# AriAaltoGit/deeplearning4j

Hardware: AMD Instinct MI355X
Metric: images/sec (whole node) ResNet-50 training at 1/2/4/8 MI355X (higher is better)
Workload: dtype bf16; 1 GPU; model=ResNet-50 (DL4J zoo ResNet50 graph), variant=dl4j, global_batch=1024, per_gpu_batch=1024, image_size=224, parallelism=dp1, comm=torch, updater=RmsProp(0.1,0.96,1e-3) + l1 1e-7 + l2 5e-5 (fused HIP updater), hip_graph=False, kernel_db=deeplearning4j_amd/ops/tunedb/gfx950.json

## Files before the change

### csrc/batchnorm.hip

```cpp
#include "common.h"
#include <cstdlib>

template <typename T>
__global__ __launch_bounds__(256) void bn_stats_partial(const T* __restrict__ x, long long M, int C,
                                                        long long rows_per_blk, float* __restrict__ part_s1,
                                                        float* __restrict__ part_s2) {
  const int T8 = C >> 3;
  const int R = 256 / T8;
  const int cg = threadIdx.x % T8, r0 = threadIdx.x / T8;
  float s1[8], s2[8], sh[8];
  Vec8<T>::load(x + cg * 8, sh);
#pragma unroll
  for (int i = 0; i < 8; ++i) { s1[i] = 0.f; s2[i] = 0.f; }
  const long long rbeg = (long long)blockIdx.x * rows_per_blk;
  long long rend = rbeg + rows_per_blk;
  if (rend > M) rend = M;
  if (r0 < R) {
    long long r = rbeg + r0;
    for (; r + 3 * R < rend; r += 4 * R) {
      float v[4][8];
#pragma unroll
      for (int u = 0; u < 4; ++u) Vec8<T>::load(x + (r + u * R) * C + cg * 8, v[u]);
#pragma unroll
      for (int u = 0; u < 4; ++u)
#pragma unroll
        for (int i = 0; i < 8; ++i) { const float d = v[u][i] - sh[i]; s1[i] += d; s2[i] += d * d; }
    }
    for (; r < rend; r += R) {
      float v[8];
      Vec8<T>::load(x + r * C + cg * 8, v);
#pragma unroll
      for (int i = 0; i < 8; ++i) { const float d = v[i] - sh[i]; s1[i] += d; s2[i] += d * d; }
    }
  }
  __shared__ float red1[256 * 9];
  __shared__ float red2[256 * 9];
#pragma unroll
  for (int i = 0; i < 8; ++i) {
    red1[threadIdx.x * 9 + i] = (r0 < R) ? s1[i] : 0.f;
    red2[threadIdx.x * 9 + i] = (r0 < R) ? s2[i] : 0.f;
  }
  __syncthreads();
  for (int c = threadIdx.x; c < C; c += 256) {
    const int g = c >> 3, k = c & 7;
    float a = 0.f, b = 0.f;
    for (int rr = 0; rr < R; ++rr) { a += red1[(rr * T8 + g) * 9 + k]; b += red2[(rr * T8 + g) * 9 + k]; }
    part_s1[(long long)blockIdx.x * C + c] = a;
    part_s2[(long long)blockIdx.x * C + c] = b;
  }
}

__global__ __launch_bounds__(256) void bn_reduce_rows(const float* __restrict__ p1, const float* __restrict__ p2,
                                                      int nblk, int C, float* __restrict__ q1, float* __restrict__ q2) {
  const int c = blockIdx.x * 64 + (threadIdx.x & 63);
  const int grp = threadIdx.x >> 6;
  const int r0 = blockIdx.y * 32 + grp * 8;
  float a[8], b[8];
#pragma unroll
  for (int u = 0; u < 8; ++u) {
    const int r = r0 + u;
    const bool ok = c < C && r < nblk;
    a[u] = ok ? p1[(long long)r * C + c] : 0.f;
    b[u] = ok ? p2[(long long)r * C + c] : 0.f;
  }
  float sa = 0.f, sb = 0.f;
#pragma unroll
  for (int u = 0; u < 8; ++u) { sa += a[u]; sb += b[u]; }
  __shared__ float ra[256], rb[256];
  ra[threadIdx.x] = sa; rb[threadIdx.x] = sb;
  __syncthreads();
  if (grp == 0 && c < C) {
    q1[(long long)blockIdx.y * C + c] = ra[threadIdx.x] + ra[threadIdx.x + 64] + ra[threadIdx.x + 128] + ra[threadIdx.x + 192];
    q2[(long long)blockIdx.y * C + c] = rb[threadIdx.x] + rb[threadIdx.x + 64] + rb[threadIdx.x + 128] + rb[threadIdx.x + 192];
  }
}

template <typename T>
__global__ __launch_bounds__(256) void bn_tiles_reduce(const float* __restrict__ ts, long long P, int C, long long M,
                                                       const T* __restrict__ x, float* __restrict__ q1,
                                                       float* __restrict__ q2, int rpp) {
  const int c = blockIdx.x * 64 + (threadIdx.x & 63);
  const int grp = threadIdx.x >> 6;
  const long long p0 = (long long)blockIdx.y * 32 + grp * 8;
  float sa = 0.f, sb = 0.f;
  if (c < C) {
    const float x0 = ld1<T>(x + c);
#pragma unroll
    for (int u = 0; u < 8; ++u) {
      const long long p = p0 + u;
      if (p >= P) break;
      const long long nrow = M - (long long)rpp * p;
      const float n = (float)(nrow < rpp ? (nrow < 0 ? 0 : nrow) : rpp);
      const float s1 = ts[p * C + c], s2 = ts[(P + p) * C + c], d = ts[(2 * P + p) * C + c] - x0;
      sa += s1 + n * d;
      sb += s2 + 2.f * d * s1 + n * d * d;
    }
  }
  __shared__ float ra[256], rb[256];
  ra[threadIdx.x] = sa;
  rb[threadIdx.x] = sb;
  __syncthreads();
  if (grp == 0 && c < C) {
    q1[(long long)blockIdx.y * C + c] = ra[threadIdx.x] + ra[threadIdx.x + 64] + ra[threadIdx.x + 128] + ra[threadIdx.x + 192];
    q2[(long long)blockIdx.y * C + c] = rb[threadIdx.x] + rb[threadIdx.x + 64] + rb[threadIdx.x + 128] + rb[threadIdx.x + 192];
  }
}

__device__ __forceinline__ void reduce_partials(const float* __restrict__ p1, const float* __restrict__ p2, int nblk,
                                                int C, int c, double& a, double& b) {
  const int grp = threadIdx.x >> 6;
  a = 0.0; b = 0.0;
  if (c < C)
    for (int i = grp; i < nblk; i += 4) { a += p1[(long long)i * C + c]; b += p2[(long long)i * C + c]; }
  __shared__ double ra[256], rb[256];
  ra[threadIdx.x] = a; rb[threadIdx.x] = b;
  __syncthreads();
  if (grp == 0) {
    a = ra[threadIdx.x] + ra[threadIdx.x + 64] + ra[threadIdx.x + 128] + ra[threadIdx.x + 192];
    b = rb[threadIdx.x] + rb[threadIdx.x + 64] + rb[threadIdx.x + 128] + rb[threadIdx.x + 192];
  }
}

template <typename T>
__global__ __launch_bounds__(256) void bn_finalize(const float* __restrict__ part_s1, const float* __restrict__ part_s2,
                                                   int nblk, int C, long long M, const T* __restrict__ x,
                                                   const float* __restrict__ gamma, const float* __restrict__ beta,
                                                   float gconst, float bconst, float* __restrict__ run_mean,
                                                   float* __restrict__ run_var, float decay, float eps, int training,
                                                   float* __restrict__ ctx) {
  const int c = blockIdx.x * 64 + (threadIdx.x & 63);
  double a = 0.0, b = 0.0;
  if (training) reduce_partials(part_s1, part_s2, nblk, C, c, a, b);
  if ((threadIdx.x >> 6) != 0 || c >= C) return;
  float mean, var;
  if (training) {
    const double m1 = a / (double)M;
    mean = (float)((double)ld1<T>(x + c) + m1);
    double v = b / (double)M - m1 * m1;
    if (v < 0) v = 0;
    var = (float)v + eps;
    run_mean[c] = decay * run_mean[c] + (1.f - decay) * mean;
    run_var[c] = decay * run_var[c] + (1.f - decay) * var;
  } else {
    mean = run_mean[c];
    var = run_var[c];
  }
  const float inv = rsqrtf(var);
  const float g = gamma ? gamma[c] : gconst;
  const float bb = beta ? beta[c] : bconst;
  ctx[c] = mean;
  ctx[C + c] = inv;
  ctx[2 * C + c] = g * inv;
  ctx[3 * C + c] = bb - mean * g * inv;
}

template <typename T, bool RELU, bool RES, bool RBN = false>
__global__ __launch_bounds__(256) void bn_apply(const T* __restrict__ x, const T* __restrict__ res, T* __restrict__ y,
                                                long long M, int C, const float* __restrict__ ctx,
                                                unsigned char* __restrict__ mask, const float* __restrict__ rctx) {
  const long long nvec = M * (C >> 3);
  const int T8 = C >> 3;
  const float* scale = ctx + 2 * C;
  const float* shift = ctx + 3 * C;
  const long long stride = (long long)gridDim.x * blockDim.x;
  const long long v0 = (long long)blockIdx.x * blockDim.x + threadIdx.x;
  if (stride % T8 == 0) {
    const int c0 = idx_mod(v0, T8) * 8;
    float sc[8], sf[8], rsc[8], rsf[8];
#pragma unroll
    for (int i = 0; i < 8; ++i) {
      sc[i] = scale[c0 + i]; sf[i] = shift[c0 + i];
      rsc[i] = RBN ? rctx[2 * C + c0 + i] : 1.f;
      rsf[i] = RBN ? rctx[3 * C + c0 + i] : 0.f;
    }
    long long v = v0;
    for (; v + stride < nvec; v += 2 * stride) {
      float a[2][8], r[2][8];
#pragma unroll
      for (int u = 0; u < 2; ++u) {
        Vec8<T>::load(x + (v + u * stride) * 8, a[u]);
        if (RES) Vec8<T>::load(res + (v + u * stride) * 8, r[u]);
      }
#pragma unroll
      for (int u = 0; u < 2; ++u) {
        unsigned bits = 0;
#pragma unroll
        for (int i = 0; i < 8; ++i) {
          float t = a[u][i] * sc[i] + sf[i];
          if (RES) t += RBN ? fmaf(r[u][i], rsc[i], rsf[i]) : r[u][i];
          bits |= (t > 0.f ? 1u : 0u) << i;
          a[u][i] = RELU ? fmaxf(t, 0.f) : t;
        }
        Vec8<T>::store(y + (v + u * stride) * 8, a[u]);
        if (RES && mask) mask[v + u * stride] = (unsigned char)bits;
      }
    }
    if (v < nvec) {
      float a[8], r[8];
      Vec8<T>::load(x + v * 8, a);
      if (RES) Vec8<T>::load(res + v * 8, r);
      unsigned bits = 0;
#pragma unroll
      for (int i = 0; i < 8; ++i) {
        float t = a[i] * sc[i] + sf[i];
        if (RES) t += RBN ? fmaf(r[i], rsc[i], rsf[i]) : r[i];
        bits |= (t > 0.f ? 1u : 0u) << i;
        a[i] = RELU ? fmaxf(t, 0.f) : t;
      }
      Vec8<T>::store(y + v * 8, a);
      if (RES && mask) mask[v] = (unsigned char)bits;
    }
    return;
  }
  for (long long v = v0; v < nvec; v += stride) {
    const int c0 = idx_mod(v, T8) * 8;
    float a[8], r[8];
    Vec8<T>::load(x + v * 8, a);
    if (RES) Vec8<T>::load(res + v * 8, r);
    unsigned bits = 0;
#pragma unroll
    for (int i = 0; i < 8; ++i) {
      float t = a[i] * scale[c0 + i] + shift[c0 + i];
      if (RES) t += RBN ? fmaf(r[i], rctx[2 * C + c0 + i], rctx[3 * C + c0 + i]) : r[i];
      bits |= (t > 0.f ? 1u : 0u) << i;
      a[i] = RELU ? fmaxf(t, 0.f) : t;
    }
    Vec8<T>::store(y + v * 8, a);
    if (RES && mask) mask[v] = (unsigned char)bits;
  }
}

template <typename T, bool RELU, bool RES, bool RBN = false>
__global__ __launch_bounds__(256) void bn_bwd_partial(const T* __restrict__ x, const T* __restrict__ res,
                                                      const T* __restrict__ dy, long long M, int C,
                                                      long long rows_per_blk, const float* __restrict__ ctx,
                                                      float* __restrict__ part_db, float* __restrict__ part_dg,
                                                      const unsigned char* __restrict__ mask,
                                                      const float* __restrict__ rctx, float* __restrict__ part_dg2) {
  const int T8 = C >> 3;
  const int R = 256 / T8;
  const int cg = threadIdx.x % T8, r0 = threadIdx.x / T8;
  float db[8], dg[8], mu[8], is[8], sc[8], sf[8], dg2[8], mu2[8], is2[8];
#pragma unroll
  for (int i = 0; i < 8; ++i) {
    db[i] = 0.f; dg[i] = 0.f; dg2[i] = 0.f;
    mu[i] = ctx[cg * 8 + i]; is[i] = ctx[C + cg * 8 + i];
    sc[i] = ctx[2 * C + cg * 8 + i]; sf[i] = ctx[3 * C + cg * 8 + i];
    mu2[i] = RBN ? rctx[cg * 8 + i] : 0.f;
    is2[i] = RBN ? rctx[C + cg * 8 + i] : 0.f;
  }
  const long long rbeg = (long long)blockIdx.x * rows_per_blk;
  long long rend = rbeg + rows_per_blk;
  if (rend > M) rend = M;
  if (r0 < R) {
    constexpr int U = 4;
    struct Batch { RawVec8<T> xv[U], gv[U], rv[RES ? U : 1]; unsigned mb[U]; };
    auto load = [&](long long r, Batch& b) {
#pragma unroll
      for (int u = 0; u < U; ++u) {
        const long long ru = r + u * R;
        const long long rr = ru < rend ? ru : rbeg + r0;
        const long long o = rr * C + cg * 8;
        b.xv[u].load(x + o);
        b.gv[u].load(dy + o);
        if (RES) {
          if (mask) b.mb[u] = mask[rr * T8 + cg];
          if (!mask || RBN) b.rv[RES ? u : 0].load(res + o);
        }
      }
    };
    auto consume = [&](long long r, const Batch& b) {
#pragma unroll
      for (int u = 0; u < U; ++u) {
        if (r + u * R >= rend) continue;
#pragma unroll
        for (int i = 0; i < 8; ++i) {
          const float xf = b.xv[u].get(i);
          float d = b.gv[u].get(i);
          if (RES && mask) {
            d = (b.mb[u] >> i) & 1u ? d : 0.f;
          } else if (RELU) {
            float t = xf * sc[i] + sf[i];
            if (RES) t += RBN ? fmaf(b.rv[RES ? u : 0].get(i), rctx[2 * C + cg * 8 + i], rctx[3 * C + cg * 8 + i])
                              : b.rv[RES ? u : 0].get(i);
            d = t > 0.f ? d : 0.f;
          }
          db[i] += d;
          dg[i] += d * (xf - mu[i]) * is[i];
          if (RBN) dg2[i] += d * (b.rv[RES ? u : 0].get(i) - mu2[i]) * is2[i];
        }
      }
    };
    long long r = rbeg + r0;
    Batch b0, b1;
    if (r < rend) load(r, b0);
    while (r < rend) {
      const long long r1 = r + U * R;
      if (r1 < rend) load(r1, b1);
      consume(r, b0);
      if (r1 >= rend) break;
      const long long r2 = r1 + U * R;
      if (r2 < rend) load(r2, b0);
      consume(r1, b1);
// ... 566 lines not shown
  float* cdb2 = cdg + C;
  float* cdg2 = cdb2 + C;
  hipLaunchKernelGGL((bn_bwd_partial<T, true, true, true>), dim3(nblk), dim3(256), 0, s, x, res, dy, M, C, rpb, ctx, p1,
                     p2, mask, rctx, p3);
  BnFin f{M, nullptr, nullptr, nullptr, 0.f, 0.f, nullptr, nullptr, 0.f, 0.f, nullptr, dbeta, dgamma, cdb, cdg,
          nullptr, 0};
  int rc = bn_fold_launch<T, 0, 1>(p1, p2, nblk, C, q, f, s);
  if (rc) return rc;
  BnFin f2{M, nullptr, nullptr, nullptr, 0.f, 0.f, nullptr, nullptr, 0.f, 0.f, nullptr, dbeta2, dgamma2, cdb2, cdg2,
           nullptr, 0};
  rc = bn_fold_launch<T, 0, 1>(p1, p3, nblk, C, q2, f2, s);
  if (rc) return rc;
  hipLaunchKernelGGL((bn_bwd_apply<T, true, true, true>), dim3(apply_grid(M, C)), dim3(256), 0, s, x, res, dy, dx, dres,
                     M, C, ctx, cdb, cdg, mask, rctx, cdg2);
  return (int)hipGetLastError();
}

DL4J_API int dl4j_bn_bwd_rbn(int dtype, const void* x, const void* res, const void* dy, void* dx, void* dres,
                             long long M, int C, const float* ctx, float* dgamma, float* dbeta, const float* rctx,
                             float* dgamma2, float* dbeta2, float* ws, const unsigned char* mask, hipStream_t s) {
  if (C % 8 != 0 || C / 8 > 256 || !res || !dres || !rctx || (dtype != 1 && dtype != 2)) return -1;
  if (dtype == 2)
    return bn_bwd_rbn_impl<f16>((const f16*)x, (const f16*)res, (const f16*)dy, (f16*)dx, (f16*)dres, M, C, ctx, dgamma,
                                dbeta, rctx, dgamma2, dbeta2, ws, mask, s);
  return bn_bwd_rbn_impl<bf16>((const bf16*)x, (const bf16*)res, (const bf16*)dy, (bf16*)dx, (bf16*)dres, M, C, ctx,
                               dgamma, dbeta, rctx, dgamma2, dbeta2, ws, mask, s);
}

DL4J_API int dl4j_bn_fwd_rbn(int dtype, const void* x, const void* res, const float* rctx, void* y, long long M, int C,
                             const float* gamma, const float* beta, float gconst, float bconst, float* run_mean,
                             float* run_var, float decay, float eps, float* ws, float* ctx_out, unsigned char* mask,
                             const float* tstats, long long P, int rpp, hipStream_t s) {
  if (C % 8 != 0 || C / 8 > 256 || !res || !rctx || !y || (dtype != 1 && dtype != 2)) return -1;
  if (tstats) {
    if (rpp < 1) return -1;
    if (dtype == 2)
      return bn_fwd_tiles_impl<f16>((const f16*)x, (const f16*)res, (f16*)y, M, C, tstats, P, rpp, gamma, beta,
                                    gconst, bconst, run_mean, run_var, decay, eps, 1, ws, ctx_out, mask, s, rctx);
    return bn_fwd_tiles_impl<bf16>((const bf16*)x, (const bf16*)res, (bf16*)y, M, C, tstats, P, rpp, gamma, beta,
                                   gconst, bconst, run_mean, run_var, decay, eps, 1, ws, ctx_out, mask, s, rctx);
  }
  if (dtype == 2)
    return bn_fwd_impl<f16>((const f16*)x, (const f16*)res, (f16*)y, M, C, gamma, beta, gconst, bconst, run_mean,
                            run_var, decay, eps, 1, 1, ws, ctx_out, mask, s, rctx);
  return bn_fwd_impl<bf16>((const bf16*)x, (const bf16*)res, (bf16*)y, M, C, gamma, beta, gconst, bconst, run_mean,
                           run_var, decay, eps, 1, 1, ws, ctx_out, mask, s, rctx);
}

DL4J_API int dl4j_bn_bwd(int dtype, const void* x, const void* res, const void* dy, void* dx, void* dres, long long M,
                         int C, const float* ctx, float* dgamma, float* dbeta, int relu, float* ws,
                         const unsigned char* mask, hipStream_t s) {
  if (C % 8 != 0 || C / 8 > 256) return -1;
  if (res) relu = 1;
  else mask = nullptr;
#define BNB(T) return bn_bwd_impl<T>((const T*)x, (const T*)res, (const T*)dy, (T*)dx, (T*)dres, M, C, ctx, dgamma, \
                                     dbeta, relu, ws, mask, s)
  if (dtype == 1) BNB(bf16);
  if (dtype == 2) BNB(f16);
  BNB(float);
#undef BNB
}

DL4J_API long long dl4j_bn_bwd_planes_workspace_floats(long long P, int C) {
  return 2 * ((P + 31) / 32) * (long long)C + 4LL * C;
}

template <typename T>
static int bn_bwd_planes_impl(const T* x, const T* dy, T* dx, T* dres, const unsigned char* mask, long long M, int C,
                              const float* ctx, float* dgamma, float* dbeta, int relu, const float* planes,
                              long long P, float* ws, hipStream_t s) {
  float* q = ws;
  float* cdb = q + 2 * ((P + 31) / 32) * (long long)C;
  float* cdg = cdb + C;
  BnFin f{M, nullptr, nullptr, nullptr, 0.f, 0.f, nullptr, nullptr, 0.f, 0.f, nullptr, dbeta, dgamma, cdb, cdg,
          nullptr, 0};
  const int rc = bn_fold_launch<T, 0, 1>(planes, planes + P * C, P, C, q, f, s);
  if (rc) return rc;
  if (dres)
    hipLaunchKernelGGL((bn_bwd_apply<T, true, true>), dim3(apply_grid(M, C)), dim3(256), 0, s, x, nullptr, dy, dx,
                       dres, M, C, ctx, cdb, cdg, mask, nullptr, nullptr);
  else if (relu)
    hipLaunchKernelGGL((bn_bwd_apply<T, true, false>), dim3(apply_grid(M, C)), dim3(256), 0, s, x, nullptr, dy, dx,
                       nullptr, M, C, ctx, cdb, cdg, nullptr, nullptr, nullptr);
  else
    hipLaunchKernelGGL((bn_bwd_apply<T, false, false>), dim3(apply_grid(M, C)), dim3(256), 0, s, x, nullptr, dy, dx,
                       nullptr, M, C, ctx, cdb, cdg, nullptr, nullptr, nullptr);
  return (int)hipGetLastError();
}

DL4J_API int dl4j_bn_bwd_planes(int dtype, const void* x, const void* dy, void* dx, void* dres,
                                const unsigned char* mask, long long M, int C, const float* ctx, float* dgamma,
                                float* dbeta, int relu, const float* planes, long long P, float* ws, hipStream_t s) {
  if (C % 8 != 0 || C / 8 > 256 || P < 1 || P != (M + 63) / 64 || ((dres == nullptr) != (mask == nullptr))) return -1;
  if (dtype == 1)
    return bn_bwd_planes_impl<bf16>((const bf16*)x, (const bf16*)dy, (bf16*)dx, (bf16*)dres, mask, M, C, ctx, dgamma,
                                    dbeta, relu, planes, P, ws, s);
  if (dtype == 2)
    return bn_bwd_planes_impl<f16>((const f16*)x, (const f16*)dy, (f16*)dx, (f16*)dres, mask, M, C, ctx, dgamma,
                                   dbeta, relu, planes, P, ws, s);
  return -1;
}

template <typename T>
__global__ __launch_bounds__(256) void bnpool_fwd(const T* __restrict__ x, T* __restrict__ y,
                                                  unsigned char* __restrict__ am, T* __restrict__ xh,
                                                  const float* __restrict__ ctx, int N, int H, int W, int C, int OH,
                                                  int OW, int kh, int kw, int sh, int sw, int pt, int pl) {
  const int CG = C >> 3;
  const long long total = (long long)N * OH * OW * CG;
  for (long long t = (long long)blockIdx.x * blockDim.x + threadIdx.x; t < total;
       t += (long long)gridDim.x * blockDim.x) {
    int cg, ow, oh, n;
    idx_decomp4(t, CG, OW, OH, cg, ow, oh, n);
    float sc[8], sf[8], best[8], bx[8];
    unsigned char idx[8];
#pragma unroll
    for (int i = 0; i < 8; ++i) {
      sc[i] = ctx[2 * C + cg * 8 + i];
      sf[i] = ctx[3 * C + cg * 8 + i];
      best[i] = -INFINITY;
      bx[i] = 0.f;
      idx[i] = 0;
    }
    for (int i = 0; i < kh; ++i) {
      const int ih = oh * sh - pt + i;
      if (ih < 0 || ih >= H) continue;
      for (int j = 0; j < kw; ++j) {
        const int iw = ow * sw - pl + j;
        if (iw < 0 || iw >= W) continue;
        float v[8];
        Vec8<T>::load(x + (((long long)n * H + ih) * W + iw) * C + cg * 8, v);
#pragma unroll
        for (int c = 0; c < 8; ++c) {
          const float a = fmaxf(v[c] * sc[c] + sf[c], 0.f);
          if (a > best[c]) {
            best[c] = a;
            bx[c] = v[c];
            idx[c] = (unsigned char)(i * kw + j);
          }
        }
      }
    }
    Vec8<T>::store(y + t * 8, best);
    if (am) {
      unsigned long long pk = 0;
#pragma unroll
      for (int c = 0; c < 8; ++c)
        pk |= ((unsigned long long)(idx[c] | (best[c] > 0.f ? 0x80 : 0))) << (8 * c);
      *reinterpret_cast<unsigned long long*>(am + t * 8) = pk;
    }
    if (xh) {
#pragma unroll
      for (int c = 0; c < 8; ++c) bx[c] = (bx[c] - ctx[cg * 8 + c]) * ctx[C + cg * 8 + c];
      Vec8<T>::store(xh + t * 8, bx);
    }
  }
}

template <typename T, int KH, int KW>
__global__ __launch_bounds__(256) void bnpool_fwd_k(const T* __restrict__ x, T* __restrict__ y,
                                                    unsigned char* __restrict__ am, T* __restrict__ xh,
                                                    const float* __restrict__ ctx, int N, int H, int W, int C, int OH,
                                                    int OW, int sh, int sw, int pt, int pl) {
  const int CG = C >> 3;
  const long long total = (long long)N * OH * OW * CG;
  for (long long t = (long long)blockIdx.x * blockDim.x + threadIdx.x; t < total;
       t += (long long)gridDim.x * blockDim.x) {
    int cg, ow, oh, n;
    idx_decomp4(t, CG, OW, OH, cg, ow, oh, n);
    float v[KH * KW][8];
    bool ok[KH * KW];
#pragma unroll
    for (int i = 0; i < KH; ++i)
#pragma unroll
      for (int j = 0; j < KW; ++j) {
        const int ih = oh * sh - pt + i, iw = ow * sw - pl + j;
        ok[i * KW + j] = ih >= 0 && ih < H && iw >= 0 && iw < W;
        const int ihc = min(max(ih, 0), H - 1), iwc = min(max(iw, 0), W - 1);
        Vec8<T>::load(x + (((long long)n * H + ihc) * W + iwc) * C + cg * 8, v[i * KW + j]);
      }
    float sc[8], sf[8], best[8], bx[8];
    unsigned char idx[8];
#pragma unroll
    for (int c = 0; c < 8; ++c) {
      sc[c] = ctx[2 * C + cg * 8 + c];
      sf[c] = ctx[3 * C + cg * 8 + c];
      best[c] = -INFINITY;
      bx[c] = 0.f;
      idx[c] = 0;
    }
#pragma unroll
    for (int q = 0; q < KH * KW; ++q) {
      if (!ok[q]) continue;
#pragma unroll
      for (int c = 0; c < 8; ++c) {
        const float a = fmaxf(v[q][c] * sc[c] + sf[c], 0.f);
        if (a > best[c]) {
          best[c] = a;
          bx[c] = v[q][c];
          idx[c] = (unsigned char)q;
        }
      }
    }
    Vec8<T>::store(y + t * 8, best);
    if (am) {
      unsigned long long pk = 0;
#pragma unroll
      for (int c = 0; c < 8; ++c)
        pk |= ((unsigned long long)(idx[c] | (best[c] > 0.f ? 0x80 : 0))) << (8 * c);
      *reinterpret_cast<unsigned long long*>(am + t * 8) = pk;
    }
    if (xh) {
#pragma unroll
      for (int c = 0; c < 8; ++c) bx[c] = (bx[c] - ctx[cg * 8 + c]) * ctx[C + cg * 8 + c];
      Vec8<T>::store(xh + t * 8, bx);
    }
  }
}

template <typename T>
__global__ __launch_bounds__(256) void bnpool_bwd_dx2(const T* __restrict__ x, const T* __restrict__ dy,
                                                      const unsigned char* __restrict__ am, T* __restrict__ dx,
                                                      const float* __restrict__ ctx, const float* __restrict__ cdb,
                                                      const float* __restrict__ cdg, int N, int H, int W, int C,
                                                      int OH, int OW, int kh, int kw, int sh, int sw, int pt, int pl) {
  const int CG = C >> 3;
  const long long total = (long long)N * H * W * CG;
  for (long long t = (long long)blockIdx.x * blockDim.x + threadIdx.x; t < total;
       t += (long long)gridDim.x * blockDim.x) {
    int cg, iw, ih, n;
    idx_decomp4(t, CG, W, H, cg, iw, ih, n);
    const int hp = ih + pt, wp = iw + pl;
    int oh0 = hp - kh + 1;
    oh0 = oh0 <= 0 ? 0 : (oh0 + sh - 1) / sh;
    int ow0 = wp - kw + 1;
    ow0 = ow0 <= 0 ? 0 : (ow0 + sw - 1) / sw;
    const int oh1 = min(hp / sh, OH - 1), ow1 = min(wp / sw, OW - 1);
    float g[4][8], xv[8];
    unsigned long long pk[4];
    unsigned me[4];
#pragma unroll
    for (int a = 0; a < 2; ++a)
#pragma unroll
      for (int b = 0; b < 2; ++b) {
        const int oh = oh0 + a, ow = ow0 + b, q = a * 2 + b;
        const bool ok = oh <= oh1 && ow <= ow1;
        const long long o = (((long long)n * OH + min(oh, OH - 1)) * OW + min(ow, OW - 1)) * C + cg * 8;
        Vec8<T>::load(dy + o, g[q]);
        pk[q] = *reinterpret_cast<const unsigned long long*>(am + o);
        me[q] = ok ? (0x80u | (unsigned)((hp - oh * sh) * kw + (wp - ow * sw))) : 0x100u;
      }
    Vec8<T>::load(x + t * 8, xv);
#pragma unroll
    for (int i = 0; i < 8; ++i) {
      float acc = 0.f;
#pragma unroll
      for (int q = 0; q < 4; ++q)
        if (((pk[q] >> (8 * i)) & 0xff) == me[q]) acc += g[q][i];
      const int c = cg * 8 + i;
      const float xhat = (xv[i] - ctx[c]) * ctx[C + c];
      xv[i] = ctx[2 * C + c] * (acc - cdb[c] - xhat * cdg[c]);
    }
    Vec8<T>::store(dx + t * 8, xv);
  }
}

template <typename T>
__global__ __launch_bounds__(256) void bnpool_bwd_dx_lds(const T* __restrict__ x, const T* __restrict__ dy,
                                                         const unsigned char* __restrict__ am, T* __restrict__ dx,
                                                         const float* __restrict__ ctx, const float* __restrict__ cdb,
                                                         const float* __restrict__ cdg, int N, int H, int W, int C,
                                                         int OH, int OW, int kh, int kw, int sh, int sw, int pt,
                                                         int pl, int maxrows) {
  extern __shared__ __attribute__((aligned(16))) unsigned char smem[];
  const int CG = C >> 3, RB = 2;
  const int rows_per_img = (H + RB - 1) / RB;
  const int n = blockIdx.x / rows_per_img, ih0 = (blockIdx.x - n * rows_per_img) * RB;
  int oh_lo = ih0 + pt - kh + 1;
  oh_lo = oh_lo <= 0 ? 0 : (oh_lo + sh - 1) / sh;
  const int oh_hi = min((min(ih0 + RB, H) - 1 + pt) / sh, OH - 1);
  const int nrows = oh_hi - oh_lo + 1;
  T* sdy = reinterpret_cast<T*>(smem);
  unsigned char* sam = smem + (size_t)maxrows * OW * C * sizeof(T);
  const int row_elems = OW * C;
  if (nrows > 0) {
    const long long g0 = ((long long)n * OH + oh_lo) * row_elems;
    const int nv = nrows * row_elems / 8;
    for (int i = threadIdx.x; i < nv; i += 256) {
      if (sizeof(T) == 2)
        reinterpret_cast<uint4*>(sdy)[i] = reinterpret_cast<const uint4*>(dy + g0)[i];
      else {
        reinterpret_cast<uint4*>(sdy)[2 * i] = reinterpret_cast<const uint4*>(dy + g0)[2 * i];
        reinterpret_cast<uint4*>(sdy)[2 * i + 1] = reinterpret_cast<const uint4*>(dy + g0)[2 * i + 1];
      }
      reinterpret_cast<uint2*>(sam)[i] = reinterpret_cast<const uint2*>(am + g0)[i];
    }
  }
  __syncthreads();
  const int items = min(RB, H - ih0) * W * CG;
  const bool fixed = (256 % CG) == 0;
  float A[8], B[8], Cq[8];
  if (fixed) {
#pragma unroll
    for (int i = 0; i < 8; ++i) {
      const int c = (threadIdx.x % CG) * 8 + i;
      A[i] = ctx[2 * C + c];
      B[i] = ctx[2 * C + c] * ctx[C + c] * cdg[c];
      Cq[i] = ctx[2 * C + c] * (cdb[c] - ctx[c] * ctx[C + c] * cdg[c]);
    }
  }
  for (int it = threadIdx.x; it < items; it += 256) {
    const int cg = it % CG, q1 = it / CG, iw = q1 % W, ih = ih0 + q1 / W;
    const int hp = ih + pt, wp = iw + pl;
    int oh0 = hp - kh + 1;
    oh0 = oh0 <= 0 ? 0 : (oh0 + sh - 1) / sh;
    int ow0 = wp - kw + 1;
    ow0 = ow0 <= 0 ? 0 : (ow0 + sw - 1) / sw;
    const int oh1 = min(hp / sh, OH - 1), ow1 = min(wp / sw, OW - 1);
    const long long t = (((long long)n * H + ih) * W + iw) * CG + cg;
    float xv[8], acc[8];
    Vec8<T>::load(x + t * 8, xv);
#pragma unroll
    for (int i = 0; i < 8; ++i) acc[i] = 0.f;
#pragma unroll
    for (int a = 0; a < 2; ++a)
#pragma unroll
      for (int b = 0; b < 2; ++b) {
        const int oh = oh0 + a, ow = ow0 + b;
        if (oh > oh1 || ow > ow1) continue;
        const int o = ((oh - oh_lo) * OW + ow) * C + cg * 8;
        float g[8];
        Vec8<T>::load(sdy + o, g);
        const unsigned long long pk = *reinterpret_cast<const unsigned long long*>(sam + o);
        const unsigned me = 0x80u | (unsigned)((hp - oh * sh) * kw + (wp - ow * sw));
#pragma unroll
        for (int i = 0; i < 8; ++i)
          if (((pk >> (8 * i)) & 0xff) == me) acc[i] += g[i];
      }
    if (fixed) {
#pragma unroll
      for (int i = 0; i < 8; ++i) xv[i] = A[i] * acc[i] - B[i] * xv[i] - Cq[i];
    } else {
#pragma unroll
      for (int i = 0; i < 8; ++i) {
        const int c = cg * 8 + i;
        const float xhat = (xv[i] - ctx[c]) * ctx[C + c];
        xv[i] = ctx[2 * C + c] * (acc[i] - cdb[c] - xhat * cdg[c]);
      }
    }
    Vec8<T>::store(dx + t * 8, xv);
  }
}

template <typename T>
__global__ __launch_bounds__(256) void bnpool_bwd_partial(const T* __restrict__ dy, const unsigned char* __restrict__ am,
                                                          const T* __restrict__ xh, long long M, int C,
                                                          long long rows_per_blk, float* __restrict__ part_db,
                                                          float* __restrict__ part_dg) {
  const int T8 = C >> 3;
  const int R = 256 / T8;
  const int cg = threadIdx.x % T8, r0 = threadIdx.x / T8;
  float db[8], dg[8];
#pragma unroll
  for (int i = 0; i < 8; ++i) {
    db[i] = 0.f;
    dg[i] = 0.f;
  }
  const long long rbeg = (long long)blockIdx.x * rows_per_blk;
  long long rend = rbeg + rows_per_blk;
  if (rend > M) rend = M;
  if (r0 < R) {
    for (long long r = rbeg + r0; r < rend; r += R) {
      const long long o = r * C + cg * 8;
      float gv[8], hv[8];
      Vec8<T>::load(dy + o, gv);
      Vec8<T>::load(xh + o, hv);
      const unsigned long long pk = *reinterpret_cast<const unsigned long long*>(am + o);
#pragma unroll
      for (int i = 0; i < 8; ++i) {
        const float d = ((pk >> (8 * i)) & 0x80) ? gv[i] : 0.f;
        db[i] += d;
        dg[i] += d * hv[i];
      }
    }
  }
  __shared__ float red1[256 * 9];
  __shared__ float red2[256 * 9];
#pragma unroll
  for (int i = 0; i < 8; ++i) {
    red1[threadIdx.x * 9 + i] = (r0 < R) ? db[i] : 0.f;
    red2[threadIdx.x * 9 + i] = (r0 < R) ? dg[i] : 0.f;
  }
  __syncthreads();
  for (int c = threadIdx.x; c < C; c += 256) {
    const int g = c >> 3, k = c & 7;
    float a = 0.f, b = 0.f;
    for (int rr = 0; rr < R; ++rr) {
      a += red1[(rr * T8 + g) * 9 + k];
      b += red2[(rr * T8 + g) * 9 + k];
    }
    part_db[(long long)blockIdx.x * C + c] = a;
    part_dg[(long long)blockIdx.x * C + c] = b;
  }
}

template <typename T>
__global__ __launch_bounds__(256) void bnpool_bwd_dx(const T* __restrict__ x, const T* __restrict__ dy,
                                                     const unsigned char* __restrict__ am, T* __restrict__ dx,
                                                     const float* __restrict__ ctx, const float* __restrict__ cdb,
                                                     const float* __restrict__ cdg, int N, int H, int W, int C, int OH,
                                                     int OW, int kh, int kw, int sh, int sw, int pt, int pl) {
  const int CG = C >> 3;
  const long long total = (long long)N * H * W * CG;
  for (long long t = (long long)blockIdx.x * blockDim.x + threadIdx.x; t < total;
       t += (long long)gridDim.x * blockDim.x) {
    int cg, iw, ih, n;
    idx_decomp4(t, CG, W, H, cg, iw, ih, n);
    float acc[8];
#pragma unroll
    for (int c = 0; c < 8; ++c) acc[c] = 0.f;
    const int hp = ih + pt, wp = iw + pl;
    int oh0 = hp - kh + 1;
    oh0 = oh0 <= 0 ? 0 : (oh0 + sh - 1) / sh;
    int ow0 = wp - kw + 1;
    ow0 = ow0 <= 0 ? 0 : (ow0 + sw - 1) / sw;
    const int oh1 = min(hp / sh, OH - 1), ow1 = min(wp / sw, OW - 1);
    for (int oh = oh0; oh <= oh1; ++oh) {
      for (int ow = ow0; ow <= ow1; ++ow) {
        const long long o = (((long long)n * OH + oh) * OW + ow) * C + cg * 8;
        float g[8];
        Vec8<T>::load(dy + o, g);
        const unsigned long long pk = *reinterpret_cast<const unsigned long long*>(am + o);
        const unsigned me = 0x80u | (unsigned)((hp - oh * sh) * kw + (wp - ow * sw));
#pragma unroll
        for (int c = 0; c < 8; ++c)
          if (((pk >> (8 * c)) & 0xff) == me) acc[c] += g[c];
      }
    }
    float xv[8];
    Vec8<T>::load(x + t * 8, xv);
#pragma unroll
    for (int i = 0; i < 8; ++i) {
      const int c = cg * 8 + i;
      const float xhat = (xv[i] - ctx[c]) * ctx[C + c];
      xv[i] = ctx[2 * C + c] * (acc[i] - cdb[c] - xhat * cdg[c]);
    }
    Vec8<T>::store(dx + t * 8, xv);
  }
}

static inline int ew_grid(long long total) {
  long long g = (total + 255) / 256;
  if (g > 256 * 32) g = 256 * 32;
  return (int)(g < 1 ? 1 : g);
}

template <typename T>
static void bnpool_fwd_launch(const T* x, T* y, unsigned char* am, T* xh, const float* ctx, int N, int H, int W, int C,
                              int OH, int OW, int kh, int kw, int sh, int sw, int pt, int pl, int pg, hipStream_t s) {
  if (kh == 3 && kw == 3)
    hipLaunchKernelGGL((bnpool_fwd_k<T, 3, 3>), dim3(pg), dim3(256), 0, s, x, y, am, xh, ctx, N, H, W, C, OH, OW, sh,
                       sw, pt, pl);
  else if (kh == 2 && kw == 2)
    hipLaunchKernelGGL((bnpool_fwd_k<T, 2, 2>), dim3(pg), dim3(256), 0, s, x, y, am, xh, ctx, N, H, W, C, OH, OW, sh,
                       sw, pt, pl);
  else
    hipLaunchKernelGGL(bnpool_fwd<T>, dim3(pg), dim3(256), 0, s, x, y, am, xh, ctx, N, H, W, C, OH, OW, kh, kw, sh, sw,
                       pt, pl);
}

template <typename T>
static int bn_pool_fwd_impl(const T* xb, T* y, unsigned char* am, T* xh, int N, int H, int W, int C, int OH, int OW,
                            int kh, int kw, int sh, int sw, int pt, int pl, const float* gamma, const float* beta,
                            float gconst, float bconst, float* run_mean, float* run_var, float decay, float eps,
                            int training, const float* tstats, long long P, int rpp, float* ws, float* ctx_out,
                            hipStream_t s) {
  const long long M = (long long)N * H * W;
  int nblk;
  long long rpb;
  bn_grid(M, C, &nblk, &rpb);
  float* p1 = ws;
  float* p2 = ws + (long long)nblk * C;
  float* q = p2 + (long long)nblk * C;
  const dim3 fg((C + 63) / 64);
  const int pg = ew_grid((long long)N * OH * OW * (C / 8));
  if (training && tstats && sizeof(T) == 2) {
    nblk = (int)((P + 31) / 32);
    p2 = ws + (long long)nblk * C;
    q = p2 + (long long)nblk * C;
    hipLaunchKernelGGL(bn_tiles_reduce<T>, dim3((C + 63) / 64, nblk), dim3(256), 0, s, tstats, P, C, M, xb, p1, p2,
                       rpp);
    bn_reduce_stage(p1, p2, nblk, C, q, s);
    hipLaunchKernelGGL(bn_finalize<T>, fg, dim3(256), 0, s, p1, p2, nblk, C, M, xb, gamma, beta, gconst, bconst,
                       run_mean, run_var, decay, eps, 1, ctx_out);
  } else {
    if (training) hipLaunchKernelGGL(bn_stats_partial<T>, dim3(nblk), dim3(256), 0, s, xb, M, C, rpb, p1, p2);
    if (training) bn_reduce_stage(p1, p2, nblk, C, q, s);
    hipLaunchKernelGGL(bn_finalize<T>, fg, dim3(256), 0, s, p1, p2, nblk, C, M, xb, gamma, beta, gconst, bconst,
                       run_mean, run_var, decay, eps, training, ctx_out);
  }
  bnpool_fwd_launch<T>(xb, y, am, xh, ctx_out, N, H, W, C, OH, OW, kh, kw, sh, sw, pt, pl, pg, s);
  return (int)hipGetLastError();
}

DL4J_API int dl4j_bn_pool_fwd(int dtype, const void* x, void* y, unsigned char* am, void* xh, int N, int H, int W,
                              int C, int OH, int OW, int kh, int kw, int sh, int sw, int pt, int pl,
                              const float* gamma, const float* beta, float gconst, float bconst, float* run_mean,
                              float* run_var, float decay, float eps, int training, const float* tstats,
                              long long P, int rpp, float* ws, float* ctx_out, hipStream_t s) {
  if (C % 8 != 0 || C / 8 > 256 || kh * kw > 127 || kh < 1 || kw < 1) return -1;
#define BPF(T) return bn_pool_fwd_impl<T>((const T*)x, (T*)y, am, (T*)xh, N, H, W, C, OH, OW, kh, kw, sh, sw, pt, pl, \
                                          gamma, beta, gconst, bconst, run_mean, run_var, decay, eps, training,    \
                                          tstats, P, rpp, ws, ctx_out, s)
  if (dtype == 1) BPF(bf16);
  if (dtype == 2) BPF(f16);
  BPF(float);
#undef BPF
}

template <typename T>
static int bn_pool_bwd_impl(const T* x, const T* dy, const unsigned char* am, const T* xh, T* dx, int N, int H, int W,
                            int C, int OH, int OW, int kh, int kw, int sh, int sw, int pt, int pl, const float* ctx,
                            float* dgamma, float* dbeta, float* ws, hipStream_t s) {
  const long long Mp = (long long)N * OH * OW, M = (long long)N * H * W;
  int nblk;
  long long rpb;
  bn_grid(Mp, C, &nblk, &rpb);
  float* p1 = ws;
  float* p2 = ws + (long long)nblk * C;
  float* q = p2 + (long long)nblk * C;
  float* cdb = q + 2LL * ((nblk + 31) / 32) * C;
  float* cdg = cdb + C;
  const int g = ew_grid(M * (C / 8));
  hipLaunchKernelGGL(bnpool_bwd_partial<T>, dim3(nblk), dim3(256), 0, s, dy, am, xh, Mp, C, rpb, p1, p2);
  bn_reduce_stage(p1, p2, nblk, C, q, s);
  hipLaunchKernelGGL(bn_bwd_finalize, dim3((C + 63) / 64), dim3(256), 0, s, p1, p2, nblk, C, M, dbeta, dgamma, cdb,
                     cdg);
  const bool two = kh <= 2 * sh && kw <= 2 * sw;
  const int maxrows = (2 - 1 + kh - 1) / sh + 1;
  const size_t lds = (size_t)maxrows * OW * C * (sizeof(T) + 1);
  if (two && lds <= 64 * 1024) {
    const int nb = N * ((H + 1) / 2);
    hipLaunchKernelGGL(bnpool_bwd_dx_lds<T>, dim3(nb), dim3(256), lds, s, x, dy, am, dx, ctx, cdb, cdg, N, H, W, C, OH,
                       OW, kh, kw, sh, sw, pt, pl, maxrows);
    return (int)hipGetLastError();
  }
  if (two)
    hipLaunchKernelGGL(bnpool_bwd_dx2<T>, dim3(g), dim3(256), 0, s, x, dy, am, dx, ctx, cdb, cdg, N, H, W, C, OH, OW,
                       kh, kw, sh, sw, pt, pl);
  else
    hipLaunchKernelGGL(bnpool_bwd_dx<T>, dim3(g), dim3(256), 0, s, x, dy, am, dx, ctx, cdb, cdg, N, H, W, C, OH, OW,
                       kh, kw, sh, sw, pt, pl);
  return (int)hipGetLastError();
}

DL4J_API int dl4j_bn_pool_bwd(int dtype, const void* x, const void* dy, const unsigned char* am, const void* xh,
                              void* dx, int N, int H, int W, int C, int OH, int OW, int kh, int kw, int sh, int sw,
                              int pt, int pl, const float* ctx, float* dgamma, float* dbeta, float* ws, hipStream_t s) {
  if (C % 8 != 0 || C / 8 > 256 || kh * kw > 127) return -1;
#define BPB(T) return bn_pool_bwd_impl<T>((const T*)x, (const T*)dy, am, (const T*)xh, (T*)dx, N, H, W, C, OH, OW, kh, \
                                          kw, sh, sw, pt, pl, ctx, dgamma, dbeta, ws, s)
  if (dtype == 1) BPB(bf16);
  if (dtype == 2) BPB(f16);
  BPB(float);
#undef BPB
}
```

### csrc/conv_stem.hip

```cpp
#include "common.h"

typedef __attribute__((ext_vector_type(4))) float f4s_t;
typedef __attribute__((ext_vector_type(8))) __bf16 bf16x8s_t;

namespace {
constexpr int KS = 6;
constexpr int ROWS_PER_WG = 4;
constexpr int IN_ROWS = 2 * ROWS_PER_WG + 6;
constexpr int OUT_LD = 64 + 8;
constexpr int STAGE_SLOTS = 12;
}

__global__ void __launch_bounds__(256, 2) stem_conv_fwd(const u16* __restrict__ x, const bf16x8s_t* __restrict__ wpk,
                                                     u16* __restrict__ y, float* __restrict__ tstats, int N, int H,
                                                     int W, int OH, int OW, int RS, long long P) {
  extern __shared__ __attribute__((aligned(16))) unsigned char smem[];
  u16* xin = reinterpret_cast<u16*>(smem);
  u16* ot = xin + 2 * IN_ROWS * RS;
  const int lane = threadIdx.x & 63, wave = threadIdx.x >> 6, col = lane & 15, hg = lane >> 4;
  const int blocks_per_img = OH / ROWS_PER_WG, nblocks = N * blocks_per_img;
  bf16x8s_t b[4][KS];
#pragma unroll
  for (int nt = 0; nt < 4; ++nt)
#pragma unroll
    for (int ks = 0; ks < KS; ++ks) b[nt][ks] = wpk[(nt * KS + ks) * 64 + lane];
  const int row_elems = 3 * W, row_u2 = row_elems / 4;
  const int nchunks = (IN_ROWS - 1) * row_u2;
  {
    const int tail = RS - 12 - row_elems, per_row = 6 + tail / 2;
    for (int i = threadIdx.x; i < 2 * IN_ROWS * per_row; i += 256) {
      const int rb = i / per_row, j = i - rb * per_row;
      const int e = j < 6 ? 2 * j : 12 + row_elems + 2 * (j - 6);
      *reinterpret_cast<unsigned*>(xin + rb * RS + e) = 0u;
    }
    for (int i = threadIdx.x; i < 2 * row_u2; i += 256) {
      const int b2 = i / row_u2, j = i - b2 * row_u2;
      *reinterpret_cast<uint2*>(xin + (b2 * IN_ROWS + IN_ROWS - 1) * RS + 12 + 4 * j) = make_uint2(0u, 0u);
    }
  }
  uint2 pre[STAGE_SLOTS];
  int buf = 0;
  for (int blk = blockIdx.x; blk < nblocks; blk += gridDim.x, buf ^= 1) {
    const int n = blk / blocks_per_img, oh0 = (blk - n * blocks_per_img) * ROWS_PER_WG;
    u16* xb = xin + buf * IN_ROWS * RS;
#pragma unroll
    for (int q = 0; q < STAGE_SLOTS; ++q) {
      const int i = threadIdx.x + q * 256;
      const int rr = i / row_u2, j = i - rr * row_u2;
      const int ih = 2 * oh0 - 3 + rr;
      pre[q] = make_uint2(0u, 0u);
      if (i < nchunks && ih >= 0 && ih < H)
        pre[q] = *reinterpret_cast<const uint2*>(x + ((long long)n * H + ih) * row_elems + 4 * j);
    }
#pragma unroll
    for (int q = 0; q < STAGE_SLOTS; ++q) {
      const int i = threadIdx.x + q * 256;
      const int rr = i / row_u2, j = i - rr * row_u2;
      if (i < nchunks) *reinterpret_cast<uint2*>(xb + rr * RS + 12 + 4 * j) = pre[q];
    }
    __syncthreads();
    const int oh = oh0 + wave;
    const long long mrow = ((long long)n * OH + oh) * OW;
    u16* otw = ot + wave * 16 * OUT_LD;
    float s1[4], s2[4], shv[4];
#pragma unroll
    for (int nt = 0; nt < 4; ++nt) s1[nt] = s2[nt] = 0.f;
    for (int mt = 0; mt < OW / 16; ++mt) {
      const int ow = mt * 16 + col;
      const unsigned* abase = reinterpret_cast<const unsigned*>(xb + (2 * wave) * RS + 6 * ow + 2);
      f4s_t acc[4];
#pragma unroll
      for (int nt = 0; nt < 4; ++nt) acc[nt] = f4s_t{0.f, 0.f, 0.f, 0.f};
#pragma unroll
      for (int ks = 0; ks < KS; ++ks) {
        const int k0 = ks * 32 + hg * 8, r = k0 / 24, q0 = k0 - r * 24;
        const unsigned* ap = abase + (r * RS + q0) / 2;
        unsigned d[5];
#pragma unroll
        for (int jj = 0; jj < 5; ++jj) d[jj] = ap[jj];
        union {
          unsigned u[4];
          bf16x8s_t v;
        } a;
#pragma unroll
        for (int jj = 0; jj < 4; ++jj) a.u[jj] = __builtin_amdgcn_alignbit(d[jj + 1], d[jj], 16);
#pragma unroll
        for (int nt = 0; nt < 4; ++nt)
          acc[nt] = __builtin_amdgcn_mfma_f32_16x16x32_bf16(a.v, b[nt][ks], acc[nt], 0, 0, 0);
      }
#pragma unroll
      for (int nt = 0; nt < 4; ++nt) {
        u16 hv[4];
#pragma unroll
        for (int j = 0; j < 4; ++j) hv[j] = f2bf(acc[nt][j]);
        if (mt == 0) shv[nt] = __shfl(bf2f(hv[0]), col, 64);
#pragma unroll
        for (int j = 0; j < 4; ++j) {
          const float dd = bf2f(hv[j]) - shv[nt];
          s1[nt] += dd;
          s2[nt] += dd * dd;
          otw[(hg * 4 + j) * OUT_LD + nt * 16 + col] = hv[j];
        }
      }
#pragma unroll
      for (int j = 0; j < 2; ++j) {
        const int id = lane + 64 * j, row = id >> 3, c8 = id & 7;
        *reinterpret_cast<bf16x8*>(y + (mrow + mt * 16 + row) * 64 + c8 * 8) =
            *reinterpret_cast<const bf16x8*>(otw + row * OUT_LD + c8 * 8);
      }
    }
    if (tstats) {
#pragma unroll
      for (int nt = 0; nt < 4; ++nt) {
        s1[nt] += __shfl_xor(s1[nt], 16, 64);
        s1[nt] += __shfl_xor(s1[nt], 32, 64);
        s2[nt] += __shfl_xor(s2[nt], 16, 64);
        s2[nt] += __shfl_xor(s2[nt], 32, 64);
      }
      if (hg == 0) {
        const long long p = (long long)n * OH + oh;
#pragma unroll
        for (int nt = 0; nt < 4; ++nt) {
          tstats[p * 64 + nt * 16 + col] = s1[nt];
          tstats[(P + p) * 64 + nt * 16 + col] = s2[nt];
          tstats[(2 * P + p) * 64 + nt * 16 + col] = shv[nt];
        }
      }
    }
  }
}

DL4J_API int dl4j_stem_conv_fwd(const void* x, const void* wpk, void* y, float* tstats, int N, int H, int W,
                                      int OH, int OW, hipStream_t s) {
  if (N < 1 || OH % ROWS_PER_WG != 0 || OW % 16 != 0 || OH != (H - 1) / 2 + 1 ||
      OW != (W - 1) / 2 + 1 || (3 * W) % 4 != 0)
    return -1;
  int RS = 12 + 3 * W;
  const int need = 6 * (OW - 1) + 3 + 24 + 2;
  if (RS < need) RS = need;
  RS = (RS + 15) & ~15;
  const size_t lds = (size_t)2 * IN_ROWS * RS * 2 + 64 * OUT_LD * 2;
  if (lds > 64 * 1024 || (IN_ROWS - 1) * (3 * W / 4) > STAGE_SLOTS * 256) return -1;
  const long long P = (long long)N * OH;
  int dev = 0, ncu = 256;
  (void)hipGetDevice(&dev);
  (void)hipDeviceGetAttribute(&ncu, hipDeviceAttributeMultiprocessorCount, dev);
  int per = 1;
  if (hipOccupancyMaxActiveBlocksPerMultiprocessor(&per, stem_conv_fwd, 256, lds) != hipSuccess || per < 1) per = 1;
  const int nblocks = N * (OH / ROWS_PER_WG);
  const int grid = nblocks < per * ncu ? nblocks : per * ncu;
  hipLaunchKernelGGL(stem_conv_fwd, dim3(grid), dim3(256), lds, s, (const u16*)x,
                     (const bf16x8s_t*)wpk, (u16*)y, tstats, N, H, W, OH, OW, RS, P);
  return (int)hipGetLastError();
}

constexpr int kWrwWgPerCu = 3;
__global__ void __launch_bounds__(256, kWrwWgPerCu) stem_conv_wrw(const u16* __restrict__ x, const u16* __restrict__ dy,
                                                        float* __restrict__ part, float* __restrict__ part_db, int N,
                                                        int H, int W, int OH, int OW, int RS) {
  extern __shared__ __attribute__((aligned(16))) unsigned char smem[];
  u16* xin = reinterpret_cast<u16*>(smem);
  u16* dyt = xin + IN_ROWS * RS;
  float* dbs = reinterpret_cast<float*>(dyt + 2 * 64 * OUT_LD);
  const int lane = threadIdx.x & 63, wave = threadIdx.x >> 6, col = lane & 15, hg = lane >> 4;
  const int blocks_per_img = OH / ROWS_PER_WG, nblocks = N * blocks_per_img;
  const int row_elems = 3 * W, row_u2 = row_elems / 4;
  const int nchunks = (IN_ROWS - 1) * row_u2;
  const int rounds = ROWS_PER_WG * OW / 64;
  {
    const int tail = RS - 12 - row_elems, per_row = 6 + tail / 2;
    for (int i = threadIdx.x; i < IN_ROWS * per_row; i += 256) {
      const int rb = i / per_row, j = i - rb * per_row;
      const int e = j < 6 ? 2 * j : 12 + row_elems + 2 * (j - 6);
      *reinterpret_cast<unsigned*>(xin + rb * RS + e) = 0u;
    }
    for (int i = threadIdx.x; i < row_u2; i += 256)
      *reinterpret_cast<uint2*>(xin + (IN_ROWS - 1) * RS + 12 + 4 * i) = make_uint2(0u, 0u);
  }
  int koff[3];
#pragma unroll
  for (int t3 = 0; t3 < 3; ++t3) {
    const int k = (wave * 3 + t3) * 16 + col, r = k / 24, q = k - r * 24;
    koff[t3] = r * RS + q;
  }
  f4s_t acc[4][3];
#pragma unroll
  for (int ct = 0; ct < 4; ++ct)
#pragma unroll
    for (int t3 = 0; t3 < 3; ++t3) acc[ct][t3] = f4s_t{0.f, 0.f, 0.f, 0.f};
  float dbacc[8];
#pragma unroll
  for (int i = 0; i < 8; ++i) dbacc[i] = 0.f;
  uint2 pre[STAGE_SLOTS];
  for (int blk = blockIdx.x; blk < nblocks; blk += gridDim.x) {
    const int n = blk / blocks_per_img, oh0 = (blk - n * blocks_per_img) * ROWS_PER_WG;
    __syncthreads();
#pragma unroll
    for (int q = 0; q < STAGE_SLOTS; ++q) {
      const int i = threadIdx.x + q * 256;
      const int rr = i / row_u2, j = i - rr * row_u2;
      const int ih = 2 * oh0 - 3 + rr;
      pre[q] = make_uint2(0u, 0u);
      if (i < nchunks && ih >= 0 && ih < H)
        pre[q] = *reinterpret_cast<const uint2*>(x + ((long long)n * H + ih) * row_elems + 4 * j);
    }
#pragma unroll
    for (int q = 0; q < STAGE_SLOTS; ++q) {
      const int i = threadIdx.x + q * 256;
      const int rr = i / row_u2, j = i - rr * row_u2;
      if (i < nchunks) *reinterpret_cast<uint2*>(xin + rr * RS + 12 + 4 * j) = pre[q];
    }
    const long long m_base = ((long long)n * OH + oh0) * OW;
    auto load_dy = [&](int rnd, uint4* dst) {
#pragma unroll
      for (int j = 0; j < 2; ++j)
        dst[j] = *reinterpret_cast<const uint4*>(dy + (m_base + rnd * 64 + (threadIdx.x >> 3) + 32 * j) * 64 +
                                                 (threadIdx.x & 7) * 8);
    };
    auto round = [&](int rnd, uint4* gr) {
      u16* dt = dyt + (rnd & 1) * 64 * OUT_LD;
#pragma unroll
      for (int j = 0; j < 2; ++j) {
        const int px = (threadIdx.x >> 3) + 32 * j, c8 = threadIdx.x & 7;
        const u16* hv = reinterpret_cast<const u16*>(&gr[j]);
#pragma unroll
        for (int i = 0; i < 8; ++i) {
          dt[(c8 * 8 + i) * OUT_LD + (((px >> 3) ^ c8) << 3) + (px & 7)] = hv[i];
          dbacc[i] += bf2f(hv[i]);
        }
      }
      if (rnd + 2 < rounds) load_dy(rnd + 2, gr);
      __syncthreads();
#pragma unroll
      for (int ch = 0; ch < 2; ++ch) {
        const int p0 = rnd * 64 + ch * 32 + 8 * hg;
        const int ohl = p0 / OW, ow0 = p0 - ohl * OW;
        const u16* wb = xin + 2 * ohl * RS + (2 * ow0 + 1) * 3;
        bf16x8s_t bfr[3];
#pragma unroll
        for (int t3 = 0; t3 < 3; ++t3) {
          union {
            u16 h[8];
            bf16x8s_t v;
          } bb;
#pragma unroll
          for (int j = 0; j < 8; ++j) bb.h[j] = wb[koff[t3] + 6 * j];
          bfr[t3] = bb.v;
        }
#pragma unroll
        for (int ct = 0; ct < 4; ++ct) {
          const int row = ct * 16 + col;
          const bf16x8s_t a =
              *reinterpret_cast<const bf16x8s_t*>(dt + row * OUT_LD + (((ch * 4 + hg) ^ (row >> 3)) << 3));
#pragma unroll
          for (int t3 = 0; t3 < 3; ++t3)
            acc[ct][t3] = __builtin_amdgcn_mfma_f32_16x16x32_bf16(a, bfr[t3], acc[ct][t3], 0, 0, 0);
        }
      }
    };
    uint4 gA[2], gB[2];
    load_dy(0, gA);
    if (rounds > 1) load_dy(1, gB);
    for (int rnd = 0; rnd < rounds; rnd += 2) {
      round(rnd, gA);
      if (rnd + 1 < rounds) round(rnd + 1, gB);
    }
  }
  float* pw = part + (long long)blockIdx.x * 64 * 192;
#pragma unroll
  for (int ct = 0; ct < 4; ++ct)
#pragma unroll
    for (int t3 = 0; t3 < 3; ++t3)
#pragma unroll
      for (int j = 0; j < 4; ++j) pw[(ct * 16 + 4 * hg + j) * 192 + (3 * wave + t3) * 16 + col] = acc[ct][t3][j];
  __syncthreads();
#pragma unroll
  for (int i = 0; i < 8; ++i) dbs[threadIdx.x * 8 + i] = dbacc[i];
  __syncthreads();
  if (threadIdx.x < 64) {
    const int c8 = threadIdx.x >> 3, i = threadIdx.x & 7;
    float sum = 0.f;
    for (int t = c8; t < 256; t += 8) sum += dbs[t * 8 + i];
    part_db[(long long)blockIdx.x * 64 + c8 * 8 + i] = sum;
  }
}

__global__ void __launch_bounds__(256) stem_wrw_reduce(const float* __restrict__ part, const float* __restrict__ part_db,
                                                       int G, float* __restrict__ dW, float* __restrict__ db) {
  __shared__ float red[16][17];
  const int ol = threadIdx.x & 15, sl = threadIdx.x >> 4;
  const int o = blockIdx.x * 16 + ol;
  float a0 = 0.f, a1 = 0.f, a2 = 0.f, a3 = 0.f;
  if (o < 64 * 147) {
    const int co = o / 147, rem = o - co * 147, c = rem / 49, rs = rem - c * 49, r = rs / 7, s = rs - r * 7;
    const float* src = part + co * 192 + r * 24 + s * 3 + c;
    int g = sl;
    for (; g + 48 < G; g += 64) {
      a0 += src[(long long)g * 12288];
      a1 += src[(long long)(g + 16) * 12288];
      a2 += src[(long long)(g + 32) * 12288];
      a3 += src[(long long)(g + 48) * 12288];
    }
    for (; g < G; g += 16) a0 += src[(long long)g * 12288];
  } else if (db && o < 64 * 147 + 64) {
    const int co = o - 64 * 147;
    for (int g = sl; g < G; g += 16) a0 += part_db[(long long)g * 64 + co];
  }
  red[ol][sl] = (a0 + a1) + (a2 + a3);
  __syncthreads();
  if (sl == 0) {
    float t = 0.f;
#pragma unroll
    for (int i = 0; i < 16; ++i) t += red[ol][i];
    if (o < 64 * 147) dW[o] = t;
    else if (db && o < 64 * 147 + 64) db[o - 64 * 147] = t;
  }
}

DL4J_API long long dl4j_stem_wrw_workspace_floats(int N, int OH) {
  int dev = 0, ncu = 256;
  (void)hipGetDevice(&dev);
  (void)hipDeviceGetAttribute(&ncu, hipDeviceAttributeMultiprocessorCount, dev);
  const long long G = (long long)kWrwWgPerCu * ncu;
  return G * (64 * 192 + 64);
}

DL4J_API int dl4j_stem_conv_wrw(const void* x, const void* dy, float* dW, float* db, float* ws, int N, int H, int W,
                                int OH, int OW, hipStream_t s) {
  if (N < 1 || OH % ROWS_PER_WG != 0 || OW % 16 != 0 || OH != (H - 1) / 2 + 1 || OW != (W - 1) / 2 + 1 ||
      (3 * W) % 4 != 0 || (ROWS_PER_WG * OW) % 64 != 0)
    return -1;
  int RS = 12 + 3 * W;
  const int need = 6 * (OW - 1) + 3 + 24 + 2;
  if (RS < need) RS = need;
  RS = (RS + 15) & ~15;
  const size_t lds = (size_t)IN_ROWS * RS * 2 + 2 * 64 * OUT_LD * 2 + 256 * 8 * 4;
  if (lds > 64 * 1024 || (IN_ROWS - 1) * (3 * W / 4) > STAGE_SLOTS * 256) return -1;
  int dev = 0, ncu = 256;
  (void)hipGetDevice(&dev);
  (void)hipDeviceGetAttribute(&ncu, hipDeviceAttributeMultiprocessorCount, dev);
  const int nblocks = N * (OH / ROWS_PER_WG);
  const int G = nblocks < kWrwWgPerCu * ncu ? nblocks : kWrwWgPerCu * ncu;
  float* part = ws;
  float* part_db = ws + (long long)G * 64 * 192;
  hipLaunchKernelGGL(stem_conv_wrw, dim3(G), dim3(256), lds, s, (const u16*)x, (const u16*)dy, part, part_db, N, H, W,
                     OH, OW, RS);
  hipLaunchKernelGGL(stem_wrw_reduce, dim3((64 * 147 + 64 + 15) / 16), dim3(256), 0, s, part, part_db, G, dW, db);
  return (int)hipGetLastError();
}

__global__ __launch_bounds__(256) void stem_pack_weights(const u16* __restrict__ w, u16* __restrict__ pk,
                                                         long long sk, long long sc, long long sr, long long ss) {
  const int e = blockIdx.x * blockDim.x + threadIdx.x;
  if (e >= 4 * 6 * 64 * 8) return;
  const int n = e & 7, m = (e >> 3) & 63, j = (e >> 9) % 6, i = e / (6 * 512);
  const int row = j * 32 + (m >> 4) * 8 + n, k = i * 16 + (m & 15);
  const int r = row / 24, rem = row - r * 24;
  u16 v = 0;
  if (r < 7 && rem < 21) {
    const int s_ = rem / 3, c = rem - s_ * 3;
    v = w[k * sk + c * sc + r * sr + s_ * ss];
  }
  pk[e] = v;
}

DL4J_API int dl4j_stem_pack_weights(const void* w, void* pk, long long sk, long long sc, long long sr, long long ss,
                                    hipStream_t s) {
  hipLaunchKernelGGL(stem_pack_weights, dim3((4 * 6 * 64 * 8 + 255) / 256), dim3(256), 0, s, (const u16*)w, (u16*)pk,
                     sk, sc, sr, ss);
  return (int)hipGetLastError();
}
```

### csrc/include/dl4j_amd.h

```cpp
#ifndef DL4J_AMD_H
#define DL4J_AMD_H

#include <stddef.h>
#include <stdint.h>

#ifdef __cplusplus
extern "C" {
#endif

#define DL4J_AMD_ABI_VERSION 1

typedef struct ihipStream_t* hipStream_t;

enum dl4j_dtype { DL4J_F32 = 0, DL4J_BF16 = 1, DL4J_F16 = 2, DL4J_I32 = 3 };

enum dl4j_status {
  DL4J_OK = 0,
  DL4J_ERR_ARG = 1001,
  DL4J_ERR_SHAPE = 1002,
  DL4J_ERR_DTYPE = 1003,
  DL4J_ERR_LAYOUT = 1004,
  DL4J_ERR_LAUNCH = 1005,
  DL4J_ERR_COMM = 1006,
  DL4J_ERR_ABI = 1007
};

enum dl4j_updater {
  DL4J_UPD_NOOP = 0, DL4J_UPD_SGD = 1, DL4J_UPD_NESTEROVS = 2, DL4J_UPD_ADAM = 3, DL4J_UPD_ADAMAX = 4,
  DL4J_UPD_NADAM = 5, DL4J_UPD_ADAGRAD = 6, DL4J_UPD_ADADELTA = 7, DL4J_UPD_RMSPROP = 8
};

enum dl4j_reduce_op { DL4J_SUM = 0, DL4J_AVG = 1, DL4J_MAX = 2 };

typedef struct dl4j_tensor {
  void* data;
  int dtype;
  int ndim;
  long long shape[8];
  long long strides[8];
  int device;
} dl4j_tensor_t;

typedef struct dl4j_comm_s* dl4j_comm_t;

typedef struct Dl4jDevProps {
  char name[128];
  char arch[64];
  int cus, xcds, warp, max_threads, lds_per_block, clock_khz, mem_clock_khz, bus_width, pci_bus;
  long long total_mem, l2_bytes, lds_per_cu;
} Dl4jDevProps;

int dl4j_abi_version(void);
int dl4j_matmul(const dl4j_tensor_t* A, const dl4j_tensor_t* B, dl4j_tensor_t* C, float alpha, float beta, hipStream_t s);
int dl4j_update_flat(int op, float* params, float* grad, float* state, long long n, const float* hp, float l1, float l2, float inv_batch, int write_update, hipStream_t s);
int dl4j_comm_unique_id(void* id_out);
int dl4j_comm_id_bytes(void);
int dl4j_comm_init_rank(dl4j_comm_t* comm, int nranks, const void* id, int rank);
int dl4j_comm_init_all(dl4j_comm_t* comms, int ndev, const int* devices);
int dl4j_comm_all_reduce(dl4j_comm_t comm, const void* send, void* recv, long long count, int dtype, int op, hipStream_t s);
int dl4j_comm_broadcast(dl4j_comm_t comm, const void* send, void* recv, long long count, int dtype, int root, hipStream_t s);
int dl4j_comm_all_gather(dl4j_comm_t comm, const void* send, void* recv, long long count_per_rank, int dtype, hipStream_t s);
int dl4j_comm_reduce_scatter(dl4j_comm_t comm, const void* send, void* recv, long long count_per_rank, int dtype, int op, hipStream_t s);
int dl4j_comm_group_start(void);
int dl4j_comm_group_end(void);
int dl4j_comm_abort(dl4j_comm_t comm);
int dl4j_comm_destroy(dl4j_comm_t comm);

int dl4j_gelu(int dtype, const void* z, const void* dy, void* out, long long n, hipStream_t s);

int dl4j_attn_fwd_dt(int dt, const void* qkv, const float* mask, void* out, float* lse, int B, int T, int H, int D, float scale, int causal, hipStream_t s);
int dl4j_attn_bwd_dt(int dt, const void* qkv, const void* out, const void* dout, const float* mask, const float* lse, float* dq_dot, void* dqkv, int B, int T, int H, int D, float scale, int causal, hipStream_t s);
int dl4j_attn_fwd_drop_dt(int dt, const void* qkv, const float* mask, void* out, float* lse, int B, int T, int H, int D, float scale, int causal, float drop, unsigned long long seed, const long long* offset, hipStream_t s);
int dl4j_attn_bwd_drop_dt(int dt, const void* qkv, const void* out, const void* dout, const float* mask, const float* lse, float* dq_dot, void* dqkv, int B, int T, int H, int D, float scale, int causal, float drop, unsigned long long seed, const long long* offset, hipStream_t s);
int dl4j_attn_drop_mask(unsigned char* keep, int BH, int T, float drop, unsigned long long seed, const long long* offset, hipStream_t s);
int dl4j_attn_fwd(const void* qkv, const float* mask, void* out, float* lse, int B, int T, int H, int D, float scale, int causal, hipStream_t s);
int dl4j_attn_bwd(const void* qkv, const void* out, const void* dout, const float* mask, const float* lse, float* dq_dot, void* dqkv, int B, int T, int H, int D, float scale, int causal, hipStream_t s);

int dl4j_bn_workspace_floats(long long M, int C);
int dl4j_bn_fwd(int dtype, const void* x, const void* res, void* y, long long M, int C, const float* gamma, const float* beta, float gconst, float bconst, float* run_mean, float* run_var, float decay, float eps, int training, int relu, float* ws, float* ctx_out, unsigned char* mask, hipStream_t s);
long long dl4j_bn_tiles_workspace_floats(long long P, int C);
int dl4j_bn_fwd_tiles(int dtype, const void* x, const void* res, void* y, long long M, int C, const float* tstats, long long P, int rpp, const float* gamma, const float* beta, float gconst, float bconst, float* run_mean, float* run_var, float decay, float eps, int relu, float* ws, float* ctx_out, unsigned char* mask, hipStream_t s);
long long dl4j_bn_bwd_rbn_workspace_floats(long long M, int C);
int dl4j_bn_bwd_rbn(int dtype, const void* x, const void* res, const void* dy, void* dx, void* dres, long long M, int C, const float* ctx, float* dgamma, float* dbeta, const float* rctx, float* dgamma2, float* dbeta2, float* ws, const unsigned char* mask, hipStream_t s);
int dl4j_bn_fwd_rbn(int dtype, const void* x, const void* res, const float* rctx, void* y, long long M, int C, const float* gamma, const float* beta, float gconst, float bconst, float* run_mean, float* run_var, float decay, float eps, float* ws, float* ctx_out, unsigned char* mask, const float* tstats, long long P, int rpp, hipStream_t s);
int dl4j_bn_bwd(int dtype, const void* x, const void* res, const void* dy, void* dx, void* dres, long long M, int C, const float* ctx, float* dgamma, float* dbeta, int relu, float* ws, const unsigned char* mask, hipStream_t s);
long long dl4j_bn_bwd_planes_workspace_floats(long long P, int C);
int dl4j_bn_bwd_planes(int dtype, const void* x, const void* dy, void* dx, void* dres, const unsigned char* mask, long long M, int C, const float* ctx, float* dgamma, float* dbeta, int relu, const float* planes, long long P, float* ws, hipStream_t s);
int dl4j_bn_pool_fwd(int dtype, const void* x, void* y, unsigned char* am, void* xh, int N, int H, int W, int C, int OH, int OW, int kh, int kw, int sh, int sw, int pt, int pl, const float* gamma, const float* beta, float gconst, float bconst, float* run_mean, float* run_var, float decay, float eps, int training, const float* tstats, long long P, int rpp, float* ws, float* ctx_out, hipStream_t s);
int dl4j_bn_pool_bwd(int dtype, const void* x, const void* dy, const unsigned char* am, const void* xh, void* dx, int N, int H, int W, int C, int OH, int OW, int kh, int kw, int sh, int sw, int pt, int pl, const float* ctx, float* dgamma, float* dbeta, float* ws, hipStream_t s);

int dl4j_nonfinite_count(const void* segs, int nseg, void* seg_dev, unsigned long long* counts, long long max_n, hipStream_t s);

int dl4j_conv_v3_num_variants(void);
int dl4j_conv_v3_default_variant(long long M, int Nout);
int dl4j_conv_fwd_v3(int dt, const void* X, const void* Wkrsc, const float* bias, void* Y, int N, int H, int W, int C, int K, int R, int S, int sh, int sw, int ph, int pw, int dh, int dw, int OH, int OW, float beta, float* tstats, int variant, hipStream_t s);
int dl4j_conv_wrw_v3_num_variants(void);
long long dl4j_conv_wrw_v3_ws_floats(int N, int C, int K, int R, int S, int OH, int OW, int variant, int splits, int* splits_out);
int dl4j_conv_wrw_v3(int dt, const void* X, const void* dY, float* dW, float* db, float* ws, int N, int H, int W, int C, int K, int R, int S, int sh, int sw, int ph, int pw, int dh, int dw, int OH, int OW, int variant, int splits, hipStream_t s);

long long dl4j_conv_halo_plan(int N, int H, int W, int C, int K, int R, int S, int sh, int sw, int ph, int pw, int dh, int dw, int OH, int OW, int* pixels_per_chunk);
int dl4j_conv_halo(int dt, const void* X, const void* Wkrsc, const float* bias, void* Y, int N, int H, int W, int C, int K, int R, int S, int sh, int sw, int ph, int pw, int dh, int dw, int OH, int OW, float beta, float* tstats, hipStream_t s);

void dl4j_conv_set_variant(int v);
void dl4j_conv_set_wrw_variant(int v);
void dl4j_conv_set_wrw_remap(int v);
int dl4j_conv_w_relayout_batched(const void* jobs, int njobs, long long total_blocks, hipStream_t s);
int dl4j_conv_relayout_job_bytes(void);
int dl4j_conv_relayout_per_block(void);
int dl4j_conv_w_relayout_tiled(const void* jobs, int njobs, long long total_blocks, hipStream_t s);
int dl4j_conv_relayout_tile_job_bytes(void);
int dl4j_conv_relayout_tile_max_rs(void);
int dl4j_conv_w_relayout(const void* W, void* krsc, void* flip, int K, int C, int R, int S, hipStream_t s);
int dl4j_conv_fwd(const void* X, const void* Wkrsc, const float* bias, void* Y, int N, int H, int W, int C, int K, int R, int S, int sh, int sw, int ph, int pw, int dh, int dw, int OH, int OW, float* tstats, hipStream_t s);
int dl4j_conv_bwd_data_s1(const void* dY, const void* Wflip, void* dX, int N, int H, int W, int C, int K, int R, int S, int ph, int pw, int OH, int OW, int accum, hipStream_t s);
int dl4j_conv_bwd_data_1x1(const void* dY, const void* Wflip, void* dX, int N, int H, int W, int C, int K, int stride, int OH, int OW, int accum, hipStream_t s);
int dl4j_conv_wrw_permute(float* ws, float* dW, int K, int C, int R, int S, int rezero, hipStream_t s);
int dl4j_conv_wrw(const void* X, const void* dY, float* dW, float* db, int N, int H, int W, int C, int K, int R, int S, int sh, int sw, int ph, int pw, int dh, int dw, int OH, int OW, int splits, hipStream_t s);
long long dl4j_conv_wrw_det_floats(int N, int C, int K, int R, int S, int OH, int OW, int splits);
int dl4j_conv_wrw_det(const void* X, const void* dY, float* dW, float* db, float* part, int N, int H, int W, int C, int K, int R, int S, int sh, int sw, int ph, int pw, int dh, int dw, int OH, int OW, int splits, hipStream_t s);

int dl4j_stem_conv_fwd(const void* x, const void* wpk, void* y, float* tstats, int N, int H, int W, int OH, int OW, hipStream_t s);
long long dl4j_stem_wrw_workspace_floats(int N, int OH);
int dl4j_stem_conv_wrw(const void* x, const void* dy, float* dW, float* db, float* ws, int N, int H, int W, int OH, int OW, hipStream_t s);
int dl4j_stem_pack_weights(const void* w, void* pk, long long sk, long long sc, long long sr, long long ss, hipStream_t s);

int dl4j_conv_wrw_set_tree(int fan);
long long dl4j_conv_wrw_halo_ws_floats(int N, int H, int W, int C, int K, int R, int S, int sh, int sw, int ph, int pw, int dh, int dw, int OH, int OW, int variant, int splits, int* splits_out);
int dl4j_conv_wrw_halo(int dt, const void* X, const void* dY, float* dW, float* db, float* ws, int N, int H, int W, int C, int K, int R, int S, int sh, int sw, int ph, int pw, int dh, int dw, int OH, int OW, int variant, int splits, hipStream_t s);

int dl4j_w2v_sg(const int32_t* item_in, const int32_t* item_tgt, const float* alpha, long long n, float* syn0, float* syn1, float* syn1neg, int D, const uint8_t* codes, const int32_t* points, const int32_t* codelen, int maxc, const int32_t* table, long long tsize, int negative, int flags, unsigned long long seed, long long item_base, float* loss_out, int max_blocks, hipStream_t stream);
int dl4j_w2v_cbow(const int32_t* item_tgt, const float* alpha, const int32_t* ctx_off, const int32_t* ctx, long long n, float* syn0, float* syn1, float* syn1neg, int D, const uint8_t* codes, const int32_t* points, const int32_t* codelen, int maxc, const int32_t* table, long long tsize, int negative, int flags, unsigned long long seed, long long item_base, const float* extra_in, int n_extra, float* extra_grad, float* loss_out, int max_blocks, hipStream_t stream);
int dl4j_glove(const int32_t* ei, const int32_t* ej, const float* ex, long long n, float* W, float* b, float* hW, float* hb, int D, float lr, float xmax, float alpha, float* cost_out, int max_blocks, hipStream_t stream);

int dl4j_rt_device_count(void);
int dl4j_rt_device_props(int dev, Dl4jDevProps* p);
int dl4j_rt_set_device(int dev);
int dl4j_rt_get_device(void);
int dl4j_rt_device_sync(int dev);
int dl4j_rt_mem_info(int dev, long long* free_b, long long* total_b);
int dl4j_rt_stream_create(int dev, int high_priority, void** out);
int dl4j_rt_stream_create_cumask(int dev, int ncu, void** out);
int dl4j_rt_stream_cu_count(void* s);
int dl4j_rt_stream_destroy(void* s);
int dl4j_rt_stream_sync(void* s);
int dl4j_rt_stream_query(void* s);
int dl4j_rt_stream_wait_event(void* s, void* ev);
int dl4j_rt_event_create(int timing, void** out);
int dl4j_rt_event_destroy(void* e);
int dl4j_rt_event_record(void* e, void* s);
int dl4j_rt_event_sync(void* e);
int dl4j_rt_event_query(void* e);
int dl4j_rt_event_elapsed(void* a, void* b, float* ms);
int dl4j_rt_capture_begin(void* s, int dev, int mode);
int dl4j_rt_capture_end(void* s, int dev, void** out);
int dl4j_rt_graph_launch(void* h, void* s);
long long dl4j_rt_graph_node_count(void* h);
int dl4j_rt_free_pool(int dev, int pool);
int dl4j_rt_graph_destroy(void* hp);
int dl4j_rt_malloc(int dev, long long nbytes, void* stream, void** out);
int dl4j_rt_record_stream(int dev, void* ptr, void* s);
int dl4j_rt_free(int dev, void* ptr);
int dl4j_rt_free_pool(int dev, int pool);
long long dl4j_rt_empty_cache(int dev);
int dl4j_rt_alloc_stats(int dev, long long* stats);
int dl4j_rt_reset_peak(int dev);
void* dl4j_rt_dlpack_empty(int dev, int ndim, const long long* shape, int code, int bits, void* stream, int* err);
int dl4j_rt_op_count(void);
int dl4j_rt_op_info(int i, const char** name, const char** sig, const char** what, void** fn);

int dl4j_gemm_stream(int in_dt, const void* A, long long lda, const void* B, long long ldb, void* C, long long ldc, int M, int N, int K, float alpha, const float* bias, int bias_mode, int act, int out_dt, float* tstats, int stats_P, int store_nt, hipStream_t s);
int dl4j_gemm_set_splitk_fixup(int on);
long long dl4j_gemm_plan(int M, int N, int K, int batch, int* cfg, int* splits);
void dl4j_bnb_arm(const void* x, const float* ctx, const unsigned char* mask, int mode);
int dl4j_gemm(int in_dt, int out_dt, int M, int N, int K, int batch, const void* A, long long lda, int akc, long long sA, const void* B, long long ldb, int bkc, long long sB, void* C, long long ldc, long long sC, float alpha, float beta, const float* bias, int bias_mode, int act, void* Z, int cfg, int splits, float* ws, float* tstats, int stats_P, hipStream_t s);
long long dl4j_gemm_f32_plan(int M, int N, int K, int batch, int* tile, int* splits);
int dl4j_gemm_f32(int in_dt, int out_dt, int M, int N, int K, int batch, const void* A, long long sam, long long sak, long long sA, const void* B, long long sbk, long long sbn, long long sB, void* C, long long ldc, long long sC, float alpha, float beta, const float* bias, int bias_mode, int act, void* Z, int tile, int splits, float* ws, hipStream_t s);
int dl4j_gemm_simple(int in_dt, int out_dt, int M, int N, int K, int batch, const void* A, long long sam, long long sak, long long sA, const void* B, long long sbk, long long sbn, long long sB, void* C, long long ldc, long long sC, float alpha, float beta, const float* bias, int bias_mode, int act, void* Z, hipStream_t s);

int dl4j_conv_stream(int dt, const void* X, const void* Wkrsc, const float* bias, void* Y, int N, int H, int W, int C, int K, int R, int S, int sh, int sw, int ph, int pw, int dh, int dw, int OH, int OW, float beta, float* tstats, hipStream_t s);

void dl4j_ln_set_config(int block_cap, int fold);
long long dl4j_ln_partial_rows(long long M);
int dl4j_ln_fwd(int dtype, const void* x, const void* r, const float* gamma, const float* beta, void* y, float* mean, float* rstd, long long M, int N, float eps, hipStream_t s);
int dl4j_ln_fwd_drop(int dtype, void* x, const void* r, const float* gamma, const float* beta, void* y, float* mean, float* rstd, long long M, int N, float eps, float keep, unsigned long long seed, const long long* offset, hipStream_t s);
int dl4j_ln_bwd(int dtype, const void* dy, const void* x, const void* r, const float* gamma, const float* mean, const float* rstd, void* dx, float* part, float* dgamma, float* dbeta, float* dsum, long long M, int N, hipStream_t s);

int dl4j_lstm_fwd(int dtype, const void* zx, const void* rwt, const float* peep, const float* h0, const float* c0, const float* mask, float* out, void* out16, float* gates, float* call, float* hT, float* cT, int Tn, int mb, int H, hipStream_t s);
int dl4j_lstm_bwd(int dtype, const void* eps, int eps_dt, const float* gates, const float* call, const float* c0, const void* rw, const float* peep, const float* mask, const float* dh_last, const float* dc_last, float* dz, float* dh0, float* dc0, int Tn, int mb, int H, int t_end, hipStream_t s);

void dl4j_lstm_coop_launch_mode(int mode);
unsigned* dl4j_lstm_step_guard(void);
int dl4j_lstm_step_guard_reset(hipStream_t s);
long long dl4j_lstm_coop_bwd_exch_bytes(int mb, int H);
int dl4j_lstm_bwd_coop(const void* eps, int eps_dt, const float* gates, const float* call, const float* c0, const void* rw, const float* peep, const float* mask, const float* dh_last, const float* dc_last, float* dz, float* dh0, float* dc0, unsigned long long* exch, unsigned* err, int Tn, int mb, int H, int t_end, unsigned tag_base, int reset, hipStream_t s);
long long dl4j_lstm_coop_exch_bytes(int mb, int H);
int dl4j_lstm_fwd_coop(const void* zx, const void* rwt, const float* peep, const float* h0, const float* c0, const float* mask, float* out, void* out16, float* gates, float* call, float* hT, float* cT, unsigned long long* exch, unsigned* err, int Tn, int mb, int H, unsigned tag_base, int reset, hipStream_t s);
long long dl4j_lstm_stack2_exch_bytes(int mb, int H, int Tn, int bwd);
int dl4j_lstm_stack2_max_t(void);
int dl4j_lstm_fwd_stack2(const void* p, int H, int reset, hipStream_t s);
int dl4j_lstm_bwd_stack2(const void* p, int H, int reset, hipStream_t s);
int dl4j_lstm_stack2_struct_bytes(int bwd);

int dl4j_lstm_bwd_prep(int dt, const float* dz, const float* out, const float* h0, const float* call, const float* c0, void* dzb, void* hpb, float* db, float* dpeep, int R, int mb, int H, int peephole, hipStream_t s);
int dl4j_lstm_pack_rw(int dt, const void* rw, long long s0, long long s1, int H, void* fwd, void* bwd, float* peep, hipStream_t s);

int dl4j_transform(int dt, int op, const void* x, void* y, long long n, float a0, float a1, hipStream_t s);
int dl4j_transform_bp(int dt, int op, const void* z, const void* eps, void* out, long long n, float a0, hipStream_t s);
int dl4j_binary(int dt, int op, const void* a, const void* b, void* out, int rank, const long long* shape, const long long* sa, const long long* sb, int flat, hipStream_t s);
int dl4j_reduce_segments(long long O, long long R, long long I);
long long dl4j_reduce_ws_bytes(long long O, long long R, long long I);
int dl4j_reduce(int dt, int op, const void* x, float* out, long long* iout, long long O, long long R, long long I, int bias_corrected, void* ws, hipStream_t s);
int dl4j_strided_copy2(int sdt, int ddt, const void* x, void* y, int rank, const long long* shape, const long long* st, const long long* off, const long long* lim, long long base, hipStream_t s);
int dl4j_strided_copy(int dt, const void* x, void* y, int rank, const long long* shape, const long long* st, const long long* off, const long long* lim, long long base, hipStream_t s);
int dl4j_strided_copy2(int sdt, int ddt, const void* x, void* y, int rank, const long long* shape, const long long* st, const long long* off, const long long* lim, long long base, hipStream_t s);
int dl4j_mergemax(int dt, const void* const* inputs, int nin, void* y, unsigned char* am, long long n, hipStream_t s);
int dl4j_mergemax_bp(int dt, const void* eps, const unsigned char* am, void* const* outs, int nout, long long n, hipStream_t s);
int dl4j_col2im(int dt, const void* cols, void* x, int N, int C, int Hp, int Wp, int R, int S, int sh, int sw, int dh, int dw, int OH, int OW, hipStream_t s);
int dl4j_im2col_rows(int dt, const void* x, void* cols, int N, int C, const long long* st, const int* g, hipStream_t s);
int dl4j_col2im_rows(int dt, const void* cols, void* dx, int N, int C, const int* g, hipStream_t s);
int dl4j_fill(void* out, long long nbytes, unsigned pattern, hipStream_t s);
int dl4j_axpy(int dt, const void* x, float* y, long long n, float alpha, hipStream_t s);

int dl4j_lrn_fwd(int dt, const void* x, void* y, float* unit, long long total, int C, int P, long long sn, long long sc, long long sp, int half, float k, float alpha, float beta, int cfast, hipStream_t s);
int dl4j_lrn_bwd(int dt, const void* x, const void* g, const float* unit, void* dx, long long total, int C, int P, long long sn, long long sc, long long sp, int half, float alpha, float beta, int cfast, hipStream_t s);
int dl4j_dropout(int dt, const void* x, void* y, long long n, unsigned long long seed, const long long* offset, int mode, int bwd, float p, float a, float b, float alpha_p, float sd, hipStream_t s);
int dl4j_emb_gather(int dt, const void* W, const long long* idx, void* out, int rows, int D, long long swr, long long swc, int V, hipStream_t s);
int dl4j_emb_scatter_add(int dt, const void* g, const long long* idx, float* dW, int rows, int D, long long sdr, long long sdc, int V, hipStream_t s);
int dl4j_bert_embed_fwd(int dt, const void* Ww, const void* Wp, const void* Wt, const long long* idx, void* out, int rows, int Tn, int E, long long sw, long long sp, int V, hipStream_t s);
int dl4j_bert_embed_bwd_pt(int dt, const void* de, float* gpos, float* gtype, int B, int Tn, int Tmax, int E, long long sgr, long long sgc, int ntype, long long str, long long stc, hipStream_t s);
int dl4j_dwconv_fwd(int dt, const void* x, const float* wr, const float* bias, void* y, const int* gi, hipStream_t s);
int dl4j_dwconv_bwd_data(int dt, const void* dy, const float* wr, void* dx, const int* gi, hipStream_t s);
int dl4j_dwconv_bwd_weight(int dt, const void* x, const void* dy, float* dwr, const int* gi, hipStream_t s);

int dl4j_pool_fwd(int dtype, int mode, const void* x, void* y, unsigned char* argmax, int N, int H, int W, int C, int OH, int OW, int kh, int kw, int sh, int sw, int pt, int pl, hipStream_t s);
int dl4j_pool_bwd(int dtype, int mode, const void* dy, const unsigned char* argmax, void* dx, int N, int H, int W, int C, int OH, int OW, int kh, int kw, int sh, int sw, int pt, int pl, hipStream_t s);

int dl4j_softmax_xent_strided(int dtype, const void* z, int ldz, const float* y, long long ys_b, long long ys_t, long long ys_j, int mb, int B, int V, void* grad, int ldg, float* score, float clip_eps, hipStream_t s);
int dl4j_softmax_xent(int dtype, const void* z, const float* y, int B, int V, void* grad, float* score, float* prob, float clip_eps, hipStream_t s);
int dl4j_softmax_xent_masked(int dtype, const void* z, const float* y, int B, int V, void* grad, float* score, const float* rmask, float clip_eps, hipStream_t s);
int dl4j_score_reduce(const float* s, long long n, float add, float scale, const float* reg, float reg_scale, float* out, hipStream_t st);

int dl4j_segment_stats(int dtype, const void* x, const long long* off, int nseg, long long maxlen, float* ws, float* out, int bins, unsigned* hist, hipStream_t stream);
long long dl4j_channel_sum_ws_floats(long long M, int C);
int dl4j_channel_sum(int dtype, const void* x, long long M, int C, float* out, float* ws, hipStream_t stream);

long long dl4j_threshold_ws_ints(long long n);
int dl4j_threshold_encode(float* residual, long long n, float thr, int* out, int capacity, int* ws, hipStream_t s);
int dl4j_threshold_count(const float* residual, long long n, float thr, int* ws, int* hdr4, hipStream_t s);
int dl4j_threshold_decode(const int* enc, float* target, int max_count, float scale, hipStream_t s);
int dl4j_bitmap_encode(float* residual, long long n, float thr, int* out, int* counter, hipStream_t s);
int dl4j_decode_any(const int* enc, long long n, int max_payload, float* target, float scale, hipStream_t s);
int dl4j_bitmap_decode(const int* enc, long long n, float* target, float scale, hipStream_t s);

int dl4j_fused_update(const void* segs, const void* btab, int nblocks, float* p, float* g, float* st, void* shadow, int shadow_kind, float inv_div, int write_update, float* reg_out, float* gn_partial, hipStream_t stream);
int dl4j_fused_update_regpart(const void* segs, const void* btab, int nblocks, float* p, float* g, float* st, void* shadow, int shadow_kind, float inv_div, int write_update, float* reg_part, float* gn_partial, hipStream_t stream);
int dl4j_update_chunk(void);
int dl4j_segdesc_size(void);


void* rt_cooc_new(const char* dir, int64_t max_entries);
int rt_cooc_add(void* h, const int32_t* tokens, const int64_t* offs, int64_t nseq, int window, int symmetric);
int64_t rt_cooc_spills(void* h);
int64_t rt_cooc_finish(void* h, const char* out_path);
void rt_cooc_free(void* h);

int64_t rt_w2v_batch(const int32_t* tokens, const int64_t* offs, int64_t nseq, const int32_t* labels, const int64_t* label_offs, const float* keep_prob, int window, int mode, uint64_t* seed_io, float alpha0, float alpha_min, int64_t words_before, int64_t total_words, int32_t* item_in, int32_t* item_tgt, float* item_alpha, int32_t* ctx_off, int32_t* ctx, int64_t cap_items, int64_t cap_ctx, int64_t* words_out);
double rt_w2v_sg_apply(const int32_t* item_in, const int32_t* item_tgt, const float* item_alpha, int64_t n, float* syn0, float* syn1, float* syn1neg, int D, const uint8_t* codes, const int32_t* points, const int32_t* codelen, int maxc, const int32_t* table, int64_t tsize, int negative, int flags, uint64_t seed, int64_t item_base, int nthreads);
double rt_w2v_cbow_apply(const int32_t* item_tgt, const float* item_alpha, const int32_t* ctx_off, const int32_t* ctx, int64_t n, float* syn0, float* syn1, float* syn1neg, int D, const uint8_t* codes, const int32_t* points, const int32_t* codelen, int maxc, const int32_t* table, int64_t tsize, int negative, int flags, uint64_t seed, int64_t item_base, int nthreads, const float* extra_in, int n_extra, float* extra_grad);
void* rt_glove_cooccur_new(const int32_t* tokens, const int64_t* offs, int64_t nseq, int window, int symmetric);
int64_t rt_glove_cooccur_size(void* h);
int64_t rt_glove_cooccur_fetch(void* h, int32_t* out_i, int32_t* out_j, float* out_x, int64_t cap);
void rt_glove_cooccur_free(void* h);
double rt_glove_apply(const int32_t* ei, const int32_t* ej, const float* ex, int64_t n, float* W, float* b, float* hW, float* hb, int D, float lr, float xmax, float alpha, int nthreads);

int64_t rt_random_walks(const int64_t* offs, const int32_t* nbr, const float* weight, const int32_t* starts, int64_t nstarts, int walk_length, uint64_t seed, int no_edge, int32_t* out, int nthreads);

long long rt_threshold_count(const float* r, long long n, float thr);
int rt_threshold_encode(float* r, long long n, float thr, int32_t* out, int capacity);
void rt_threshold_decode(const int32_t* enc, float* target, float scale);
int rt_bitmap_encode(float* r, long long n, float thr, int32_t* out);
void rt_bitmap_decode(const int32_t* enc, float* target, float scale);

void* rt_vptree_build(const float* data, int n, int d, int metric_id, int invert, uint64_t seed);
void rt_vptree_free(void* h);
void rt_vptree_knn(void* h, const float* queries, int nq, int k, int32_t* out_idx, float* out_dist, int nthreads);
void* rt_sptree_build(const double* Y, int n, int D);
void rt_sptree_free(void* h);
int rt_sptree_depth(void* h);
int rt_sptree_cum(void* h);
void rt_sptree_com(void* h, double* out);
double rt_sptree_nonedge(void* h, int i, double theta, double* negF);
double rt_bhtsne_gradient(const double* Y, int n, int D, const int64_t* rowP, const int32_t* colP, const double* valP, double theta, double* dY, int nthreads);
void rt_tsne_row_probs(const float* dist, int n, int K, double perplexity, double tol, float* out, int nthreads);

long long rt_ws_create(long long initial_bytes, long long max_bytes, long long alignment, double overalloc, int learning, int reset_policy, int cycles_before_init);
void rt_ws_destroy(long long h);
int rt_ws_alloc(long long h, long long bytes, long long* off, long long* generation);
long long rt_ws_cycle_end(long long h);
int rt_ws_set_capacity(long long h, long long bytes);
long long rt_ws_generation(long long h);
int rt_ws_stats(long long h, long long* out);

#ifdef __cplusplus
}
#endif

#endif
```

### deeplearning4j_amd/nn/graph/computation_graph.py

```python
import os

import torch

from ...datasets.dataset import DataSet, MultiDataSet
from ..conf.enums import BackpropType
from ..conf.graph import LayerVertex
from ..conf.layers import ActivationLayer, BatchNormalization
from ..conf.validation import check_layer_input, validate_network_conf
from ...exceptions import DL4JInvalidInputException
from ..layers.output import BaseOutputLayerImpl
from ..network_base import BaseNetwork
from ... import profiling as _prof


def _shares_storage(a, b):
    if a is None or b is None or not torch.is_tensor(a) or not torch.is_tensor(b) or a.device != b.device:
        return False
    if a.numel() == 0 or b.numel() == 0:
        return False

    def span(t):
        n = 1 + sum((s - 1) * abs(st) for s, st in zip(t.shape, t.stride()))
        return t.data_ptr(), t.data_ptr() + n * t.element_size()
    a0, a1 = span(a)
    b0, b1 = span(b)
    return a0 < b1 and b0 < a1



def _out_dtype(t):
    return t.float() if t.dtype in (torch.bfloat16, torch.float16) else t

class ComputationGraph(BaseNetwork):
    _key_by_name = True

    def __init__(self, conf, params=None):
        super().__init__(conf)
        self._init_params = params
        self.inputs = None
        self.labels = None
        self.inputMaskArrays = None
        self.labelMaskArrays = None

    def init(self, parameters=None, cloneParametersArray=False, device=None):
        if self.initCalled and parameters is None:
            return
        parameters = parameters if parameters is not None else self._init_params
        conf = self.conf
        if conf.inputTypes is not None and not hasattr(conf, "_types"):
            conf.addPreProcessorsAndInferNIn()
        self.topo = [n for n in conf.topologicalOrder() if n not in conf.networkInputs]
        validate_network_conf({n: conf.vertices[n].layerConf for n in self.topo
                               if isinstance(conf.vertices[n], LayerVertex)})
        self.vertex_inputs = conf.vertexInputs
        self.consumers = {n: [] for n in list(conf.networkInputs) + self.topo}
        for v in self.topo:
            for i in self.vertex_inputs[v]:
                self.consumers[i].append(v)
        self.layers_by_name = {}
        layer_list = []
        for idx, name in enumerate(self.topo):
            v = conf.vertices[name]
            if isinstance(v, LayerVertex):
                impl = v.layerConf.instantiate(index=idx, net=self)
                self.layers_by_name[name] = impl
                layer_list.append((idx, name, impl))
        self._setup_flat(layer_list, parameters, cloneParametersArray, device)
        self.outputs = list(conf.networkOutputs)
        self._plan_fusions()
        for l in self.layers_by_name.values():
            if hasattr(l, "bind"):
                l.bind()

    def _plan_fusions(self):
        from ..conf.activations import ActivationReLU
        from ..conf.graph import ElementWiseVertex
        self._passthrough = {}
        self._residual_of = {}
        pos = {n: i for i, n in enumerate(self.topo)}
        for n in self.conf.networkInputs:
            pos[n] = -1

        def is_relu_layer(n):
            vv = self.conf.vertices.get(n)
            return isinstance(vv, LayerVertex) and isinstance(vv.layerConf, ActivationLayer) and \
                isinstance(vv.layerConf.activation, ActivationReLU) and vv.preProcessor is None and \
                vv.layerConf.idropout is None and len(self.vertex_inputs[n]) == 1

        def is_max_pool(n):
            from ..conf.layers import SubsamplingLayer
            vv = self.conf.vertices.get(n)
            if not (isinstance(vv, LayerVertex) and type(vv.layerConf) is SubsamplingLayer) or \
                    vv.preProcessor is not None or vv.layerConf.idropout is not None or \
                    len(self.vertex_inputs[n]) != 1:
                return False
            lc = vv.layerConf
            return lc.poolingType.value == "MAX" and tuple(lc.dilation) == (1, 1)

        for name in self.topo:
            v = self.conf.vertices[name]
            if not (isinstance(v, LayerVertex) and isinstance(v.layerConf, BatchNormalization)):
                continue
            if v.layerConf.idropout is not None:
                continue
            cons = self.consumers[name]
            if len(cons) != 1 or name in self.outputs:
                continue
            nxt_name = cons[0]
            nxt = self.conf.vertices[nxt_name]
            if isinstance(nxt, ElementWiseVertex) and nxt.op == "Add" and len(self.vertex_inputs[nxt_name]) == 2 \
                    and nxt_name not in self.outputs and len(self.consumers[nxt_name]) == 1 \
                    and is_relu_layer(self.consumers[nxt_name][0]) and os.environ.get("DL4J_AMD_FUSE_RES", "1") == "1":
                ins = self.vertex_inputs[nxt_name]
                other = ins[1] if ins[0] == name else ins[0]
                relu_name = self.consumers[nxt_name][0]
                if other != name and pos[other] < pos[name] and relu_name not in self.outputs:
                    self.layers_by_name[name].fuse_relu = True
                    self._residual_of[name] = other
                    self._passthrough[nxt_name] = name
                    self._passthrough[relu_name] = nxt_name
                    ov = self.conf.vertices.get(other)
                    if isinstance(ov, LayerVertex) and isinstance(ov.layerConf, BatchNormalization) and \
                            ov.layerConf.idropout is None and ov.preProcessor is None and \
                            self.consumers.get(other) == [nxt_name] and other not in self.outputs and \
                            not getattr(ov.layerConf, "useLogStd", False) and \
                            os.environ.get("DL4J_AMD_FUSE_RES_BN", "1") == "1":
                        self.layers_by_name[name].residual_bn = self.layers_by_name[other]
                        self.layers_by_name[other].defer_apply = True
                    continue
            if is_relu_layer(nxt_name) and nxt_name not in self.outputs:
                self.layers_by_name[name].fuse_relu = True
                self._passthrough[nxt_name] = name
                pc = self.consumers[nxt_name]
                if len(pc) == 1 and pc[0] not in self.outputs and is_max_pool(pc[0]) and \
                        os.environ.get("DL4J_AMD_FUSE_POOL", "1") == "1":
                    self.layers_by_name[name].fuse_pool = self.layers_by_name[pc[0]]
                    self._passthrough[pc[0]] = nxt_name
        from ..conf.layers import ConvolutionLayer, ZeroPaddingLayer
        from ..conf.enums import ConvolutionMode
        for name in self.topo:
            v = self.conf.vertices[name]
            if not (isinstance(v, LayerVertex) and isinstance(v.layerConf, ZeroPaddingLayer)) or \
                    name in self.outputs or len(self.consumers[name]) != 1 or \
                    os.environ.get("DL4J_AMD_FOLD_PAD", "1") != "1":
                continue
            cn = self.consumers[name][0]
            cv = self.conf.vertices[cn]
            if not (isinstance(cv, LayerVertex) and type(cv.layerConf) is ConvolutionLayer) or \
                    cv.preProcessor is not None or cv.layerConf.convolutionMode != ConvolutionMode.Truncate or \
                    len(self.vertex_inputs[cn]) != 1 or len(self.vertex_inputs[name]) != 1:
                continue
            p = list(v.layerConf.padding)
            self.layers_by_name[cn].extra_pad4 = (p[0], p[1], p[2], p[3])
            self._passthrough[name] = self.vertex_inputs[name][0]
        for name in self.topo:
            v = self.conf.vertices[name]
            if not (isinstance(v, LayerVertex) and type(v.layerConf) is ConvolutionLayer) or name in self.outputs \
                    or len(self.consumers[name]) != 1 or os.environ.get("DL4J_AMD_DEFER_BIAS", "1") != "1":
                continue
            impl = self.layers_by_name[name]
            if "b" not in impl.params or type(v.layerConf.activation).__name__ != "ActivationIdentity":
                continue
            if v.layerConf.nIn % 8 == 0 and v.layerConf.nOut % 4 == 0 and \
                    os.environ.get("DL4J_AMD_DEFER_BIAS", "1") != "all":
                continue
            bn_name = self.consumers[name][0]
            bv = self.conf.vertices[bn_name]
            if not (isinstance(bv, LayerVertex) and isinstance(bv.layerConf, BatchNormalization)) or \
                    bv.preProcessor is not None or len(self.vertex_inputs[bn_name]) != 1:
                continue
            impl.defer_bias = True
            self.layers_by_name[bn_name].deferred_bias = impl
        for name in self.topo:
            v = self.conf.vertices[name]
            if not (isinstance(v, LayerVertex) and type(v.layerConf) is ConvolutionLayer) or name in self.outputs \
                    or len(self.consumers[name]) != 1 or os.environ.get("DL4J_AMD_CONV_BN_STATS", "1") != "1":
                continue
            if type(v.layerConf.activation).__name__ != "ActivationIdentity" or v.layerConf.idropout is not None:
                continue
            bv = self.conf.vertices[self.consumers[name][0]]
            if isinstance(bv, LayerVertex) and isinstance(bv.layerConf, BatchNormalization) and \
                    bv.preProcessor is None and bv.layerConf.idropout is None and \
                    not getattr(bv.layerConf, "useLogStd", False):
                self.layers_by_name[name].emit_bn_stats = True
        flows = {n: False for n in self.conf.networkInputs}
        self._need_input_grad = {}
        for name in self.topo:
            ins = self.vertex_inputs[name]
            need = any(flows.get(i, False) for i in ins)
            self._need_input_grad[name] = need
            layer = self.layers_by_name.get(name)
            own = layer is not None and layer.conf.numParams() > 0
            flows[name] = need or own
        for name, layer in self.layers_by_name.items():
            layer.need_input_grad = self._need_input_grad[name]

    def getLayers(self):
        return list(self.layers_by_name.values())

    def getLayer(self, name):
        if isinstance(name, int):
            return self.getLayers()[name]
        return self.layers_by_name[name]

    def getVertex(self, name):
        return _RuntimeVertex(self, name)

    def getVertices(self):
        return [_RuntimeVertex(self, n) for n in list(self.conf.networkInputs) + list(self.conf.vertices)]

    def _replace_impl(self, idx, name, old, new):
        self.layers_by_name[name] = new

    def _summary_types(self, inputTypes):
        import copy
        c = copy.deepcopy(self.conf)
        c.inputTypes = list(inputTypes)
        types = c.addPreProcessorsAndInferNIn()
        out = {}
        for name in self.layers_by_name:
            ins = [types[i] for i in c.vertexInputs[name]]
            out[name] = (ins[0] if len(ins) == 1 else ins, types[name])
        return out

    def getNumLayers(self):
        return len(self.layers_by_name)

    def getOutputLayer(self, i):
        return self.layers_by_name[self.outputs[i]]

    def getConfiguration(self):
        return self.conf

    def _prep_inputs(self, inputs):
        if torch.is_tensor(inputs) or not isinstance(inputs, (list, tuple)):
            inputs = [inputs]
        out = []
        for x in inputs:
            if not torch.is_tensor(x):
                import numpy as np
                x = torch.from_numpy(np.asarray(x))
            x = x.toTensor() if hasattr(x, "toTensor") else x
            out.append(self._to_dev(x, self._feat_dtype()) if x.is_floating_point() else self._to_dev(x))
        return out

    def feedForward(self, inputs=None, train=False, masks=None, stored_state=False, store_last_for_tbptt=False,
                    layerTillIndex=None):
        if isinstance(inputs, bool):
            inputs, train = None, inputs
        inputs = self._prep_inputs(self.inputs if inputs is None else inputs)
        if len(inputs) != len(self.conf.networkInputs):
            raise DL4JInvalidInputException(f"ComputationGraph has {len(self.conf.networkInputs)} inputs "
                                            f"{list(self.conf.networkInputs)}, got {len(inputs)} arrays")
        chk = self._input_check(inputs)
        idx = self._index_checked()
        if masks is None:
            masks = self.inputMaskArrays
        acts = {}
        amask = {}
        active = {}
        mb = inputs[0].shape[0]
        self._prep_mb = mb
        for i, n in enumerate(self.conf.networkInputs):
            acts[n] = inputs[i]
            amask[n] = masks[i] if masks is not None and i < len(masks) else None
            active[n] = True
        self._ctx = {}
        for name in self.topo:
            v = self.conf.vertices[name]
            ins = [acts[i] for i in self.vertex_inputs[name]]
            ms = [amask.get(i) for i in self.vertex_inputs[name]]
            active[name] = any(active.get(i, True) for i in self.vertex_inputs[name])
            if isinstance(v, LayerVertex):
                x = ins[0] if len(ins) == 1 else torch.cat(ins, dim=1)
                if len(ins) > 1:
                    self._ctx[name] = ("merge", [t.shape[1] for t in ins])
                mask = ms[0] if ms else None
                if v.preProcessor is not None:
                    x = v.preProcessor.preProcess(x, mb, train)
                    if mask is not None:
                        mask, _ = v.preProcessor.feedForwardMaskArray(mask, None, mb)
                if chk is not None or name in idx:
                    check_layer_input(v.layerConf, x, name)
                if name in self._passthrough:
                    acts[name] = acts[self._passthrough[name]]
                    amask[name] = mask
                    continue
                layer = self.layers_by_name[name]
                layer.iteration, layer.epoch = self.conf.iterationCount, self.conf.epochCount
                if name in self._residual_of:
                    layer.residual = acts[self._residual_of[name]]
                tok = _prof.layer_begin("fwd", name, layer) if _prof.ACTIVE else None
                if not active[name] and hasattr(layer, "setLabels"):
                    mask = None
                if stored_state and hasattr(layer, "tBpttStateMap"):
                    out = layer.activate(x, train, mask, stored_state=True, store_last_for_tbptt=store_last_for_tbptt)
                else:
                    out = layer.activate(x, train, mask)
                if tok is not None:
                    _prof.layer_end(tok, "fwd", name, layer, out)
                acts[name] = out
                amask[name], _ = layer.feedForwardMaskArray(mask, None, mb)
                if getattr(layer, "MASK_PASSTHROUGH", False):
                    active[name] = False
            elif name in self._passthrough:
                acts[name] = acts[self._passthrough[name]]
                amask[name] = ms[0] if ms else None
            else:
                from ..conf.graph import DuplicateToTimeSeriesVertex
                if isinstance(v, DuplicateToTimeSeriesVertex):
                    v._T = acts[v.inputName].shape[2]
                out, ctx = v.forward(ins, train, ms)
                self._ctx[name] = ("vertex", ctx)
                acts[name] = out
                amask[name] = v.feedForwardMask(ms)
        if chk is not None:
            self._validated = chk
        self._acts_masks = amask
        return acts

    def setLayerMaskArrays(self, featureMaskArrays, labelMaskArrays):
        self.inputMaskArrays = list(featureMaskArrays) if featureMaskArrays is not None else None
        self.labelMaskArrays = list(labelMaskArrays) if labelMaskArrays is not None else None

    def clearLayerMaskArrays(self):
        self.inputMaskArrays = self.labelMaskArrays = None

    def output(self, *inputs, train=False, masks=None):
        if inputs and isinstance(inputs[0], bool):
            train, inputs = inputs[0], inputs[1:]
        if len(inputs) == 1 and isinstance(inputs[0], (list, tuple)):
            inputs = inputs[0]
        with torch.no_grad():
            acts = self.feedForward(list(inputs), train, masks)
        outs = [_out_dtype(acts[o]) for o in self.outputs]
        lm = self.labelMaskArrays
        if lm is not None:
            from ..network_base import _apply_output_mask
            outs = [_apply_output_mask(t, lm[i]) if i < len(lm) and hasattr(self.layers_by_name.get(o), "setLabels")
                    else t for i, (o, t) in enumerate(zip(self.outputs, outs))]
        return outs

    def outputSingle(self, *inputs, train=False):
        if inputs and isinstance(inputs[0], bool):
            train, inputs = inputs[0], inputs[1:]
        return self.output(*inputs, train=train)[0]

    def _backprop(self, tbptt_back=None):
        eps_acc = {}

        def add(name, e):
            if e is None:
                return
            if name in eps_acc:
                if eps_acc[name] is e:
                    return
                eps_acc[name] = eps_acc[name] + e
            else:
                eps_acc[name] = e

        self._begin_backward()
        for name in reversed(self.topo):
            v = self.conf.vertices[name]
            if name in self._passthrough:
                add(self._passthrough[name], eps_acc.pop(name, None))
                continue
            if isinstance(v, LayerVertex):
                layer = self.layers_by_name.get(name)
                if name in self.outputs and (isinstance(layer, BaseOutputLayerImpl) or hasattr(layer, "computeScore")):
                    tok = _prof.layer_begin("bwd", name, layer) if _prof.ACTIVE else None
                    _, e = layer.backpropGradient(None)
                    if tok is not None:
                        _prof.layer_end(tok, "bwd", name, layer, e)
                    self._grad_ready(name)
                else:
                    e_in = eps_acc.pop(name, None)
                    if e_in is None:
                        continue
                    if not self._need_input_grad[name] and layer.conf.numParams() == 0:
                        continue
                    tok = _prof.layer_begin("bwd", name, layer) if _prof.ACTIVE else None
                    ins0 = self.vertex_inputs[name]
                    if len(ins0) == 1 and v.preProcessor is None and ins0[0] in eps_acc and \
                            hasattr(layer, "dx_accum") and \
                            not any(_shares_storage(eps_acc[ins0[0]], t) for t in
                                    [e_in] + [t for k, t in eps_acc.items() if k != ins0[0]]):
                        layer.dx_accum = eps_acc[ins0[0]]
                    if tbptt_back is not None and hasattr(layer, "tBpttStateMap"):
                        _, e = layer.backpropGradient(e_in, tbptt_back=tbptt_back)
                    else:
                        _, e = layer.backpropGradient(e_in)
                    if tok is not None:
                        _prof.layer_end(tok, "bwd", name, layer, e)
                    self._grad_ready(name)
                    if name in self._residual_of:
                        add(self._residual_of[name], layer.dresidual)
                        layer.dresidual = None
                if e is None or not self._need_input_grad[name]:
                    continue
                if v.preProcessor is not None:
                    e = v.preProcessor.backprop(e, self._mb)
                ins = self.vertex_inputs[name]
                if len(ins) > 1:
                    parts = torch.split(e, self._ctx[name][1], dim=1)
                    for i, p in zip(ins, parts):
                        add(i, p)
                else:
                    add(ins[0], e)
            else:
                e_in = eps_acc.pop(name, None)
                if e_in is None or not self._need_input_grad[name]:
                    continue
                es = v.backward(e_in, self._ctx[name][1])
                for i, ei in zip(self.vertex_inputs[name], es):
                    add(i, ei)
        self._end_backward()
        for l in self.listeners:
            if hasattr(l, "onBackwardPass"):
                l.onBackwardPass(self)
        self._input_eps = [eps_acc.get(n) for n in self.conf.networkInputs]
        return self._input_eps

    def computeGradientAndScore(self, inputs=None, labels=None, fmasks=None, lmasks=None, stored_state=False,
                                store_last_for_tbptt=False, tbptt_back=None, defer_reg=False):
        if inputs is None:
            fmasks = getattr(self, "inputMaskArrays", None) if fmasks is None else fmasks
            lmasks = getattr(self, "labelMaskArrays", None) if lmasks is None else lmasks
        inputs = self._prep_inputs(self.inputs if inputs is None else inputs)
        labels = self.labels if labels is None else labels
        if torch.is_tensor(labels):
            labels = [labels]
        self._mb = inputs[0].shape[0]
        self._prepare_conv_weights()
        fm = [self._to_dev(m) for m in fmasks] if fmasks else None
        skip = not any(hasattr(l, "onForwardPass") for l in self.listeners)
        outs = [self.layers_by_name.get(o) for o in self.outputs]
        for o, l in zip(self.outputs, outs):
            if l is not None and skip and not self.consumers.get(o):
                l._skip_train_output = True
        try:
            acts = self.feedForward(inputs, True, fm, stored_state, store_last_for_tbptt)
        finally:
            for l in outs:
                if l is not None:
                    l._skip_train_output = False
        for l in self.listeners:
            if hasattr(l, "onForwardPass"):
                l.onForwardPass(self, acts)
        mb_in = self._prep_mb if getattr(self, "_prep_mb", None) else None
        for i, o in enumerate(self.outputs):
            layer = self.layers_by_name.get(o)
            if layer is None or not hasattr(layer, "setLabels"):
                from ...exceptions import DL4JException
                kind = type(layer.conf).__name__ if layer is not None else type(self.conf.vertices[o]).__name__
                raise DL4JException(f"Cannot calculate gradient and score: network output \"{o}\" is not an output "
                                    f"layer ({kind}); end the graph in an OutputLayer / RnnOutputLayer / LossLayer")
            layer.setLabels(self._to_dev(labels[i], self.master_dtype))
            layer.inputMiniBatchSize = mb_in
            lm = lmasks[i] if lmasks is not None and i < len(lmasks) else None
            if lm is not None:
                layer.maskArray = self._to_dev(lm)
        self._backprop(tbptt_back)
        l1, l2 = (0.0, 0.0) if defer_reg else self._regularization_terms()
        score = None
        for i, o in enumerate(self.outputs):
            layer = self.layers_by_name[o]
            s = layer.computeScore(l1 if i == 0 else 0.0, l2 if i == 0 else 0.0, True)
            score = s if score is None else score + s
        self._loss_part = score
        self._score_t = score
        self._score_val = None
        return score

    def _fit_batch_sgd(self, inputs, labels, fmasks=None, lmasks=None):
        x0 = inputs[0] if isinstance(inputs, (list, tuple)) else inputs
        if self.conf.backpropType == BackpropType.TruncatedBPTT and x0.dim() == 3:
            return self._fit_tbptt(inputs, labels, fmasks, lmasks)
        self.computeGradientAndScore(inputs, labels, fmasks, lmasks, defer_reg=True)
        self._apply_update(x0.shape[0])
        self._iteration_done()

    def _fit_tbptt(self, inputs, labels, fmasks, lmasks):
        inputs = inputs if isinstance(inputs, (list, tuple)) else [inputs]
        labels = labels if isinstance(labels, (list, tuple)) else [labels]
        T = inputs[0].shape[2]
        fwd, back = self.conf.tbpttFwdLength, self.conf.tbpttBackLength
        self.rnnClearPreviousState()
        for s in range((T + fwd - 1) // fwd):
            t0, t1 = s * fwd, min(T, (s + 1) * fwd)
            xs = [x[:, :, t0:t1] if x.dim() == 3 else x for x in inputs]
            ys = [y[:, :, t0:t1] if y.dim() == 3 else y for y in labels]
            fm = [m[:, t0:t1] if m is not None else None for m in fmasks] if fmasks else None
            lm = [m[:, t0:t1] if m is not None else None for m in lmasks] if lmasks else None
            if self._try_graph_step(xs, ys, fm, lm, tbptt_back=back):
                continue
            from ...memory.arena import tbptt_scope
            with tbptt_scope(self):
                self.computeGradientAndScore(xs, ys, fm, lm, stored_state=True, store_last_for_tbptt=True,
                                             tbptt_back=back, defer_reg=True)
                self._apply_update(inputs[0].shape[0])
            self._iteration_done()
        self.rnnClearPreviousState()

    def fit(self, data, labels=None, numEpochs=None, featureMaskArrays=None, labelMaskArrays=None):
        if not self.initCalled:
            self.init()
        if labels is not None and not isinstance(labels, int):
            self._fit_batch(data, labels, featureMaskArrays, labelMaskArrays)
            return self
        if isinstance(labels, int):
            numEpochs = labels
        if numEpochs is not None:
            for _ in range(numEpochs):
                self.fit(data)
            return self
        if isinstance(data, DataSet):
            self._fit_batch([data.features], [data.labels],
                            None if data.featuresMask is None else [data.featuresMask],
                            None if data.labelsMask is None else [data.labelsMask])
            return self
        if isinstance(data, MultiDataSet):
            self._fit_batch(data.features, data.labels, data.featuresMasks, data.labelsMasks)
            return self
        self._fit_iterator(data)
        return self

    def _fit_iterator(self, it):
        from ...datasets.iterators import AsyncDataSetIterator
        wrap = it
        if getattr(it, "asyncSupported", lambda: False)() and not isinstance(it, AsyncDataSetIterator) and \
                type(it).__name__ not in ("BenchmarkDataSetIterator", "BenchmarkMultiDataSetIterator",
                                          "ListDataSetIterator"):
            wrap = AsyncDataSetIterator(it, 2, self.device)
        for l in self.listeners:
            if hasattr(l, "onEpochStart"):
                l.onEpochStart(self)
        wrap.reset()
        t0 = self._timer()
        while wrap.hasNext():
            ds = wrap.next()
            self.lastEtlTime = (self._timer() - t0) * 1000.0
            if isinstance(ds, MultiDataSet):
                self._fit_batch(ds.features, ds.labels, ds.featuresMasks, ds.labelsMasks)
            else:
                self._fit_batch([ds.features], [ds.labels], None if ds.featuresMask is None else [ds.featuresMask],
                                None if ds.labelsMask is None else [ds.labelsMask])
            t0 = self._timer()
        if wrap is not it and hasattr(wrap, "shutdown"):
            wrap.shutdown()
        for l in self.listeners:
            if hasattr(l, "onEpochEnd"):
                l.onEpochEnd(self)
        self.incrementEpochCount()

    def _score_dataset(self, ds, training=False):
        if isinstance(ds, DataSet):
            ds = MultiDataSet.fromDataSet(ds)
        with torch.no_grad():
            self._mb = ds.features[0].shape[0]
            self.feedForward(ds.features, training)
            l1, l2 = self._regularization_terms()
            score = 0.0
            for i, o in enumerate(self.outputs):
                layer = self.layers_by_name[o]
                layer.setLabels(self._to_dev(ds.labels[i], self.master_dtype))
                layer.inputMiniBatchSize = self._mb
                score += float(layer.computeScore(l1 if i == 0 else 0.0, l2 if i == 0 else 0.0, training))
            return score

    def scoreExamples(self, data, addRegularizationTerms=True):
        ds = data if isinstance(data, (DataSet, MultiDataSet)) else data.next()
        if isinstance(ds, DataSet):
            ds = MultiDataSet.fromDataSet(ds)
        with torch.no_grad():
            self.feedForward(ds.features, False, ds.featuresMasks)
            l1, l2 = self._regularization_terms() if addRegularizationTerms else (0.0, 0.0)
            total = None
            for i, o in enumerate(self.outputs):
                layer = self.layers_by_name[o]
                layer.setLabels(self._to_dev(ds.labels[i], self.master_dtype))
                if ds.labelsMasks and i < len(ds.labelsMasks) and ds.labelsMasks[i] is not None:
                    layer.maskArray = self._to_dev(ds.labelsMasks[i])
                s = layer.computeScoreForExamples(l1 if i == 0 else 0.0, l2 if i == 0 else 0.0)
                total = s if total is None else total + s
            return total

    def evaluate(self, it, labelsList=None, topN=1):
        from ...eval.evaluation import Evaluation
        return self.doEvaluation(it, Evaluation(labelsList, topN=topN))[0]

    def evaluateRegression(self, it):
        from ...eval.regression import RegressionEvaluation
        return self.doEvaluation(it, RegressionEvaluation())[0]

    def evaluateROC(self, it, steps=0):
        from ...eval.roc import ROC
        return self.doEvaluation(it, ROC(steps))[0]

    def doEvaluation(self, it, *evals):
        items = [it] if isinstance(it, (DataSet, MultiDataSet)) else it
        if not isinstance(it, (DataSet, MultiDataSet)):
            it.reset()
        for ds in items:
            if isinstance(ds, MultiDataSet):
                out = self.output(ds.features)[0]
                lab = ds.labels[0]
                lm = ds.labelsMasks[0] if ds.labelsMasks else None
            else:
                out = self.output(ds.features)[0]
                lab, lm = ds.labels, ds.labelsMask
            for e in evals:
                e.eval(lab, out, lm)
        return list(evals)

    def rnnTimeStep(self, *inputs):
        inputs = self._prep_inputs(list(inputs))
        mb = inputs[0].shape[0]
        acts = {n: inputs[i] for i, n in enumerate(self.conf.networkInputs)}
        with torch.no_grad():
            for name in self.topo:
                v = self.conf.vertices[name]
                if name in self._passthrough:
                    acts[name] = acts[self._passthrough[name]]
                    continue
                ins = [acts[i] for i in self.vertex_inputs[name]]
                if isinstance(v, LayerVertex):
                    x = ins[0] if len(ins) == 1 else torch.cat(ins, 1)
                    if v.preProcessor is not None:
                        x = v.preProcessor.preProcess(x, mb, False)
                    layer = self.layers_by_name[name]
                    if name in self._residual_of:
                        layer.residual = acts[self._residual_of[name]]
                    if hasattr(layer, "rnnTimeStep"):
                        acts[name] = layer.rnnTimeStep(x)
                    else:
                        acts[name] = layer.activate(x, False)
                else:
                    acts[name], _ = v.forward(ins, False, None)
        return [_out_dtype(acts[o]) for o in self.outputs]

    def rnnClearPreviousState(self):
        for l in self.layers_by_name.values():
            if hasattr(l, "rnnClearPreviousState"):
                l.rnnClearPreviousState()

    def rnnGetPreviousState(self, layerName):
        layer = self.layers_by_name[layerName] if isinstance(layerName, str) else self.getLayers()[layerName]
        return layer.rnnGetPreviousState() if hasattr(layer, "rnnGetPreviousState") else None

    def rnnSetPreviousState(self, layerName, state):
        layer = self.layers_by_name[layerName] if isinstance(layerName, str) else self.getLayers()[layerName]
        if not hasattr(layer, "rnnSetPreviousState"):
            raise ValueError(f"layer {layerName} is not a recurrent layer")
        layer.rnnSetPreviousState(state)

    def rnnGetPreviousStates(self):
        return {n: l.rnnGetPreviousState() for n, l in self.layers_by_name.items() if hasattr(l, "rnnGetPreviousState")}

    def rnnSetPreviousStates(self, states):
        for n, st in states.items():
            self.rnnSetPreviousState(n, st)

    def pretrainLayer(self, layerName, data, numEpochs=1):
        if not self.initCalled:
# ... 128 lines not shown
```

### deeplearning4j_amd/nn/layers/convolution.py

```python
import torch
import torch.nn.functional as F

from ... import ops
from ..conf.enums import ConvolutionMode
from ..conf.layers import conv_out_size, same_padding
from .base import LayerImpl, copy_grad_
from deeplearning4j_amd.nn.util.dtypes import acc as _acc


def _cl(x):
    if x.is_cuda and x.dim() == 4:
        if x.is_contiguous(memory_format=torch.channels_last):
            return x
        from ...ops import nd4j_kernels as NK
        y = NK.channels_last_copy(x)
        return y if y is not None else x.contiguous(memory_format=torch.channels_last)
    return x


def compute_pad4(conf, h, w, kernel=None, stride=None, dilation=None):
    kernel = kernel or conf.kernelSize
    stride = stride or conf.stride
    dilation = dilation or getattr(conf, "dilation", [1, 1]) or [1, 1]
    if conf.convolutionMode == ConvolutionMode.Same:
        oh = conv_out_size(h, kernel[0], stride[0], 0, dilation[0], ConvolutionMode.Same)
        ow = conv_out_size(w, kernel[1], stride[1], 0, dilation[1], ConvolutionMode.Same)
        pt, pb = same_padding(h, oh, kernel[0], stride[0], dilation[0])
        pl, pr = same_padding(w, ow, kernel[1], stride[1], dilation[1])
        return (pt, pb, pl, pr)
    p = conf.padding
    conv_out_size(h, kernel[0], stride[0], p[0], dilation[0], conf.convolutionMode)
    conv_out_size(w, kernel[1], stride[1], p[1], dilation[1], conf.convolutionMode)
    return (p[0], p[0], p[1], p[1])


def _truncate_input(conf, x, kernel, stride, pad4, dilation):
    if conf.convolutionMode == ConvolutionMode.Same:
        return x
    h, w = x.shape[2], x.shape[3]
    oh = conv_out_size(h, kernel[0], stride[0], pad4[0], dilation[0], ConvolutionMode.Truncate)
    ow = conv_out_size(w, kernel[1], stride[1], pad4[2], dilation[1], ConvolutionMode.Truncate)
    need_h = (oh - 1) * stride[0] + (kernel[0] - 1) * dilation[0] + 1 - 2 * pad4[0]
    need_w = (ow - 1) * stride[1] + (kernel[1] - 1) * dilation[1] + 1 - 2 * pad4[2]
    if need_h < h or need_w < w:
        return x[:, :, :max(need_h, 0) if need_h < h else h, :max(need_w, 0) if need_w < w else w]
    return x


class ConvolutionLayerImpl(LayerImpl):
    def type(self):
        return "CONVOLUTIONAL"

    extra_pad4 = None
    defer_bias = False
    dx_accum = None
    emit_bn_stats = False

    def _geom(self, x):
        c = self.conf
        pad4 = compute_pad4(c, x.shape[2], x.shape[3])
        if self.extra_pad4 is not None:
            pad4 = tuple(a + b for a, b in zip(pad4, self.extra_pad4))
        return list(c.kernelSize), list(c.stride), pad4, list(c.dilation)

    def preOutput(self, x, training=False):
        k, s, pad4, d = self._geom(x)
        W = self.W("W")
        b = self.params["b"].reshape(-1) if "b" in self.params else None
        if self.defer_bias and training:
            b = None
        xt = x
        self._xt = xt
        self._geom_cache = (s, pad4, d)
        return ops.conv2d_forward(_cl(xt.to(W.dtype)), W, b, s, pad4, d,
                                  want_stats=bool(training and self.emit_bn_stats))

    def activate(self, x, training=False, mask=None):
        if x.dim() != 4:
            raise ValueError(f"Got rank {x.dim()} array as input to ConvolutionLayer {self.layerId()}; "
                             "expected rank 4 [minibatch, channels, height, width]")
        if x.shape[1] != self.conf.nIn:
            raise ValueError(f"Cannot do forward pass in Convolution layer {self.layerId()}: input depth "
                             f"{x.shape[1]} does not match nIn {self.conf.nIn}")
        self.training = training
        x = self.applyDropOutIfNecessary(x, training)
        self.input = x
        z = self.preOutput(x, training)
        self._z = z
        return self.conf.activation.getActivation(z, training)

    def backpropGradient(self, eps):
        delta = self.conf.activation.backprop(self._z, eps.to(self._z.dtype))
        s, pad4, d = self._geom_cache
        W = self.W("W")
        xt = _cl(self._xt.to(W.dtype))
        need_dx = getattr(self, "need_input_grad", True)
        acc = getattr(self, "dx_accum", None)
        self.dx_accum = None
        dx, dW, db = ops.conv2d_backward(xt, W, _cl(delta.to(W.dtype)), s, pad4, d, need_dx, True,
                                         "b" in self.grads, gW=self.grads["W"], gb=self.grads.get("b"),
                                         grads_zeroed=getattr(self.net, "_grads_zeroed", False),
                                         dx_accum=acc if need_dx and self.conf.idropout is None else None)
        if dW is not None:
            copy_grad_(self.grads["W"], dW)
        if "b" in self.grads and db is not None:
            copy_grad_(self.grads["b"], db)
        if not need_dx:
            return self.make_gradient(), None
        if dx.shape[2:] != self.input.shape[2:]:
            full = torch.zeros(self.input.shape, dtype=dx.dtype, device=dx.device)
            full[:, :, :dx.shape[2], :dx.shape[3]] = dx
            dx = full
        return self.make_gradient(), self.backpropDropOut(dx)


class Convolution1DLayerImpl(ConvolutionLayerImpl):

    def activate(self, x, training=False, mask=None):
        self._was3d = x.dim() == 3
        x4 = x.unsqueeze(3) if x.dim() == 3 else x
        out = super().activate(x4, training, None)
        out = out.squeeze(3)
        if mask is not None:
            out = out * mask.unsqueeze(1).to(out.dtype)[:, :, :out.shape[2]]
        return out

    def backpropGradient(self, eps):
        g, dx = super().backpropGradient(eps.unsqueeze(3))
        return g, (dx.squeeze(3) if dx is not None else None)


class Deconvolution2DImpl(ConvolutionLayerImpl):

    def _pad(self):
        c = self.conf
        return [0, 0] if c.convolutionMode == ConvolutionMode.Same else list(c.padding)

    def preOutput(self, x, training=False):
        from ...ops.nn_misc import deconv_forward
        c = self.conf
        W = self.W("W")
        b = self.W("b").reshape(-1) if "b" in self.params else None
        self._xt = x
        out = deconv_forward(_cl(x.to(W.dtype)), W, b, list(c.stride), self._pad(), list(c.dilation))
        self._full_hw = out.shape[2:]
        if c.convolutionMode == ConvolutionMode.Same:
            out = out[:, :, :x.shape[2] * c.stride[0], :x.shape[3] * c.stride[1]]
        return out

    def backpropGradient(self, eps):
        from ...ops.nn_misc import deconv_backward
        c = self.conf
        delta = self.conf.activation.backprop(self._z, eps.to(self._z.dtype))
        W = self.W("W")
        if tuple(delta.shape[2:]) != tuple(self._full_hw):
            full = torch.zeros(delta.shape[:2] + tuple(self._full_hw), dtype=delta.dtype, device=delta.device)
            full[:, :, :delta.shape[2], :delta.shape[3]] = delta
            delta = full
        gW = self.grads["W"] if self.grads["W"].dtype == torch.float32 and self.grads["W"].is_contiguous() else None
        dx, dW, db = deconv_backward(self._xt.to(W.dtype), W, delta.to(W.dtype), list(c.stride), self._pad(),
                                     list(c.dilation), "b" in self.grads, gW=gW,
                                     gb=self.grads["b"].reshape(-1) if "b" in self.grads else None)
        if dW is not None and dW is not gW:
            copy_grad_(self.grads["W"], _acc(dW))
        if "b" in self.grads and db is not None:
            copy_grad_(self.grads["b"], _acc(db))
        return self.make_gradient(), self.backpropDropOut(dx)


class DepthwiseConvolution2DImpl(ConvolutionLayerImpl):

    def preOutput(self, x, training=False):
        from ...ops.nn_misc import depthwise_forward
        c = self.conf
        W = self.W("W")
        pad4 = compute_pad4(c, x.shape[2], x.shape[3])
        self._xt = _cl(x.to(W.dtype))
        self._geom_cache = (list(c.stride), pad4, list(c.dilation))
        b = self.params["b"].reshape(-1) if "b" in self.params else None
        return depthwise_forward(self._xt, W, b, *self._geom_cache)

    def backpropGradient(self, eps):
        from ...ops.nn_misc import depthwise_backward
        delta = self.conf.activation.backprop(self._z, eps.to(self._z.dtype))
        W = self.W("W")
        dx, dW, db = depthwise_backward(self._xt, W, _cl(delta.to(W.dtype)), *self._geom_cache,
                                        need_db="b" in self.grads)
        copy_grad_(self.grads["W"], dW)
        if "b" in self.grads:
            copy_grad_(self.grads["b"], db)
        return self.make_gradient(), self.backpropDropOut(dx)


class SeparableConvolution2DImpl(DepthwiseConvolution2DImpl):

    def preOutput(self, x, training=False):
        from ...ops.nn_misc import depthwise_forward
        c = self.conf
        W = self.W("W")
        pad4 = compute_pad4(c, x.shape[2], x.shape[3])
        self._xt = _cl(x.to(W.dtype))
        self._geom_cache = (list(c.stride), pad4, list(c.dilation))
        self._y1 = _cl(depthwise_forward(self._xt, W, None, *self._geom_cache))
        b = self.params["b"].reshape(-1) if "b" in self.params else None
        return ops.conv2d_forward(self._y1, self.W("pW"), b, (1, 1), (0, 0, 0, 0), (1, 1))

    def backpropGradient(self, eps):
        from ...ops.nn_misc import depthwise_backward
        delta = self.conf.activation.backprop(self._z, eps.to(self._z.dtype))
        W, pW = self.W("W"), self.W("pW")
        dy1, dpW, db = ops.conv2d_backward(self._y1, pW, _cl(delta.to(pW.dtype)), (1, 1), (0, 0, 0, 0), (1, 1),
                                           True, True, "b" in self.grads, gW=self.grads["pW"],
                                           gb=self.grads.get("b"))
        if dpW is not None:
            copy_grad_(self.grads["pW"], _acc(dpW))
        if "b" in self.grads and db is not None:
            copy_grad_(self.grads["b"], _acc(db))
        dx, dW, _ = depthwise_backward(self._xt, W, _cl(dy1.to(W.dtype)), *self._geom_cache, need_db=False)
        copy_grad_(self.grads["W"], dW)
        return self.make_gradient(), self.backpropDropOut(dx)


class SubsamplingLayerImpl(LayerImpl):
    def type(self):
        return "SUBSAMPLING"

    def activate(self, x, training=False, mask=None):
        self.training = training
        x = self.applyDropOutIfNecessary(x, training)
        self.input = x
        c = self.conf
        pad4 = compute_pad4(c, x.shape[2], x.shape[3], c.kernelSize, c.stride, c.dilation)
        xt = x
        self._xshape = x.shape
        y, self._ctx = ops.pool2d_forward(_cl(xt), c.poolingType.value, c.kernelSize, c.stride, pad4, c.dilation,
                                          c.pnorm, c.eps)
        return y

    def backpropGradient(self, eps):
        dx = ops.pool2d_backward(_cl(eps), self._ctx)
        if dx.shape[2:] != self._xshape[2:]:
            full = torch.zeros(self._xshape, dtype=dx.dtype, device=dx.device)
            full[:, :, :dx.shape[2], :dx.shape[3]] = dx
            dx = full
        return self.make_gradient(), self.backpropDropOut(dx)


class Subsampling1DLayerImpl(SubsamplingLayerImpl):
    def activate(self, x, training=False, mask=None):
        out = super().activate(x.unsqueeze(3), training, None).squeeze(3)
        if mask is not None:
            from ..util.time_series import reverse_time_series
        return out

    def backpropGradient(self, eps):
        g, dx = super().backpropGradient(eps.unsqueeze(3))
        return g, dx.squeeze(3)


class ZeroPaddingLayerImpl(LayerImpl):
    def activate(self, x, training=False, mask=None):
        t, b, l, r = self.conf.padding
        self._pad = (t, b, l, r)
        return _cl(F.pad(x, (l, r, t, b)))

    def backpropGradient(self, eps):
        t, b, l, r = self._pad
        H, W = eps.shape[2], eps.shape[3]
        return self.make_gradient(), eps[:, :, t:H - b, l:W - r]


class ZeroPadding1DLayerImpl(LayerImpl):
    def activate(self, x, training=False, mask=None):
        l, r = self.conf.padding
        self._pad = (l, r)
        return F.pad(x, (l, r))

    def backpropGradient(self, eps):
        l, r = self._pad
        return self.make_gradient(), eps[:, :, l:eps.shape[2] - r]


class Cropping2DImpl(LayerImpl):
    def activate(self, x, training=False, mask=None):
        t, b, l, r = self.conf.cropping
        self._shape = x.shape
        return x[:, :, t:x.shape[2] - b, l:x.shape[3] - r]

    def backpropGradient(self, eps):
        t, b, l, r = self.conf.cropping
        g = torch.zeros(self._shape, dtype=eps.dtype, device=eps.device)
        g[:, :, t:self._shape[2] - b, l:self._shape[3] - r] = eps
        return self.make_gradient(), g


def _nd4j():
    from ...ops import nd4j_kernels
    return nd4j_kernels


class Upsampling2DImpl(LayerImpl):

    def activate(self, x, training=False, mask=None):
        s = self.conf.size
        if x.is_cuda:
            y = _nd4j().upsample_nearest2d(x, s[0], s[1])
            if y is not None:
                return y
        return x.repeat_interleave(s[0], dim=2).repeat_interleave(s[1], dim=3)

    def backpropGradient(self, eps):
        s = self.conf.size
        n, c, h, w = eps.shape
        if eps.is_cuda:
            g = _nd4j().upsample_nearest2d_bp(eps, s[0], s[1])
            if g is not None:
                return self.make_gradient(), g
        return self.make_gradient(), eps.reshape(n, c, h // s[0], s[0], w // s[1], s[1]).sum(dim=(3, 5))


class Upsampling1DImpl(LayerImpl):
    def activate(self, x, training=False, mask=None):
        return x.repeat_interleave(self.conf.size[0], dim=2)

    def backpropGradient(self, eps):
        s = self.conf.size[0]
        n, c, T = eps.shape
        return self.make_gradient(), eps.reshape(n, c, T // s, s).sum(dim=3)


class SpaceToDepthImpl(LayerImpl):

    def activate(self, x, training=False, mask=None):
        b = self.conf.blockSize
        n, c, H, W = x.shape
        if x.is_cuda:
            y = _nd4j().space_to_depth(x, b)
            if y is not None:
                return y
        y = x.reshape(n, c, H // b, b, W // b, b).permute(0, 3, 5, 1, 2, 4)
        return y.reshape(n, b * b * c, H // b, W // b)

    def backpropGradient(self, eps):
        b = self.conf.blockSize
        if eps.is_cuda:
            g = _nd4j().depth_to_space(eps, b)
            if g is not None:
                return self.make_gradient(), g
        n, cc, h, w = eps.shape
        c = cc // (b * b)
        g = eps.reshape(n, b, b, c, h, w).permute(0, 3, 4, 1, 5, 2)
        return self.make_gradient(), g.reshape(n, c, h * b, w * b)


class SpaceToBatchImpl(LayerImpl):
    def activate(self, x, training=False, mask=None):
        (pt, pb), (pl, pr) = self.conf.padding
        bh, bw = self.conf.blocks
        if x.is_cuda:
            y = _nd4j().space_to_batch(x, (bh, bw), ((pt, pb), (pl, pr)))
            if y is not None:
                self._shape = (x.shape, (x.shape[0], x.shape[1], x.shape[2] + pt + pb, x.shape[3] + pl + pr))
                return y
        xp = F.pad(x, (pl, pr, pt, pb))
        n, c, H, W = xp.shape
        self._shape = (x.shape, xp.shape)
        y = xp.reshape(n, c, H // bh, bh, W // bw, bw).permute(3, 5, 0, 1, 2, 4)
        return y.reshape(bh * bw * n, c, H // bh, W // bw)

    def backpropGradient(self, eps):
        (pt, pb), (pl, pr) = self.conf.padding
        bh, bw = self.conf.blocks
        xs, xps = self._shape
        n, c, H, W = xps
        if eps.is_cuda:
            g = _nd4j().batch_to_space(eps, (bh, bw), ((pt, pb), (pl, pr)))
            if g is not None:
                return self.make_gradient(), g
        g = eps.reshape(bh, bw, n, c, H // bh, W // bw).permute(2, 3, 4, 0, 5, 1).reshape(n, c, H, W)
        return self.make_gradient(), g[:, :, pt:pt + xs[2], pl:pl + xs[3]]
```

### deeplearning4j_amd/nn/layers/normalization.py

```python
import torch

from ... import ops
from .base import LayerImpl, copy_grad_
from deeplearning4j_amd.nn.util.dtypes import acc as _acc


class BatchNormalizationImpl(LayerImpl):
    def __init__(self, conf, index=0, net=None):
        super().__init__(conf, index, net)
        self.fuse_relu = False

    def type(self):
        return "NORMALIZATION"

    def _gb(self):
        c = self.conf
        if c.lockGammaBeta:
            return c.gamma, c.beta
        return self.params["gamma"], self.params["beta"]

    def activate(self, x, training=False, mask=None):
        self.training = training
        x = self.applyDropOutIfNecessary(x, training)
        self.input = x
        if x.dim() not in (2, 4):
            raise ValueError(f"BatchNormalization on activations of rank {x.dim()} not supported {self.layerId()}")
        g, b = self._gb()
        c = self.conf
        pool = getattr(self, "fuse_pool", None)
        if pool is not None and x.dim() == 4:
            from .convolution import compute_pad4
            pc = pool.conf
            pad4 = compute_pad4(pc, x.shape[2], x.shape[3], pc.kernelSize, pc.stride, pc.dilation)
            y, self._ctx = ops.bn_pool_forward(x, g, b, self.params["mean"], self.params["var"], training, c.decay,
                                               c.eps, tuple(pc.kernelSize), tuple(pc.stride), pad4)
            self._pool_fused = True
            self._track_deferred_bias(training)
            return y
        self._pool_fused = False
        self._apply_deferred = False
        if getattr(self, "defer_apply", False) and training:
            r = ops.bn_forward(x, g, b, self.params["mean"], self.params["var"], training, c.decay, c.eps,
                               stats_only=True)
            if r is not None:
                self._apply_deferred = True
                y, self._ctx = r
                self._track_deferred_bias(training)
                return y
        res = getattr(self, "residual", None)
        rbn = getattr(self, "residual_bn", None)
        self._rbn_active = None
        if res is not None and rbn is not None and getattr(rbn, "_apply_deferred", False):
            r = ops.bn_forward(x, g, b, self.params["mean"], self.params["var"], training, c.decay, c.eps,
                               relu=True, residual=res, rctx=rbn._ctx[2])
            if r is None:
                raise RuntimeError(f"{self.layerId()}: fused shortcut BatchNormalization could not run")
            y, self._ctx = r
            self._rbn_active = rbn
        else:
            y, self._ctx = ops.bn_forward(x, g, b, self.params["mean"], self.params["var"], training, c.decay, c.eps,
                                          relu=self.fuse_relu, residual=res)
        self.residual = None
        self._track_deferred_bias(training)
        return y

    def _track_deferred_bias(self, training):
        c = self.conf
        db = getattr(self, "deferred_bias", None)
        if training and db is not None:
            from ...ops.nd4j_kernels import axpy_
            with torch.no_grad():
                axpy_(self.params["mean"], db.params["b"], 1.0 - c.decay)

    def backpropGradient(self, eps):
        gg, gb = self.grads.get("gamma"), self.grads.get("beta")
        if getattr(self, "_apply_deferred", False):
            self._apply_deferred = False
            self._zero_stat_grads()
            return self.make_gradient(), self.backpropDropOut(eps)
        if getattr(self, "_pool_fused", False):
            dx, dgamma, dbeta = ops.bn_pool_backward(eps, self._ctx, gg, gb)
            self.dresidual = None
        elif getattr(self, "_rbn_active", None) is not None:
            rbn = self._rbn_active
            self._rbn_active = None
            dx, dgamma, dbeta, self.dresidual = ops.bn_backward(eps, self._ctx, gg, gb,
                                                                rgrads=(rbn.grads.get("gamma"), rbn.grads.get("beta")))
        else:
            dx, dgamma, dbeta, self.dresidual = ops.bn_backward(eps, self._ctx, gg, gb)
        if gg is not None:
            if dgamma is not gg:
                copy_grad_(gg, dgamma)
            if dbeta is not gb:
                copy_grad_(gb, dbeta)
        self._zero_stat_grads()
        return self.make_gradient(), self.backpropDropOut(dx)

    def _zero_stat_grads(self):
        if not getattr(self, "_stat_grads_zero", False):
            self.grads["mean"].zero_()
            self.grads["var"].zero_()
            self._stat_grads_zero = True


def _is_identity(a):
    from ..conf.activations import ActivationIdentity
    return a is None or isinstance(a, ActivationIdentity)


class LocalResponseNormalizationImpl(LayerImpl):

    def activate(self, x, training=False, mask=None):
        from ...ops.nn_misc import lrn_forward
        self.input = x
        c = self.conf
        y, self._ctx = lrn_forward(x, c.n, c.k, c.alpha, c.beta)
        return y.to(x.dtype)

    def backpropGradient(self, eps):
        from ...ops.nn_misc import lrn_backward
        return self.make_gradient(), lrn_backward(eps, self._ctx).to(eps.dtype)


class LayerNormalizationImpl(LayerImpl):
    def activate(self, x, training=False, mask=None):
        self.input = x
        y, self._ctx = ops.layer_norm_forward(x, self.params["gamma"], self.params["beta"], self.conf.eps)
        self._pre = y
        return self.conf.activation.getActivation(y, training) if not _is_identity(self.conf.activation) else y

    def backpropGradient(self, eps):
        if not _is_identity(self.conf.activation):
            eps = self.conf.activation.backprop(self._pre, eps)
        dx, dg, db = ops.layer_norm_backward(eps, self._ctx)
        copy_grad_(self.grads["gamma"], dg)
        copy_grad_(self.grads["beta"], db)
        return self.make_gradient(), dx
```

### deeplearning4j_amd/ops/conv_stem.py

```python
import torch

from . import native
from .native import _ptr, _stream

_packed = {}


def supported(x, w, b, stride, pad4, dilation):
    if not (x.is_cuda and x.dtype == torch.bfloat16 and w.dtype == torch.bfloat16 and x.dim() == 4):
        return False
    N, C, H, W = x.shape
    if tuple(w.shape) != (64, 3, 7, 7) or C != 3 or b is not None:
        return False
    if tuple(stride) != (2, 2) or tuple(pad4) != (3, 3, 3, 3) or tuple(dilation) != (1, 1):
        return False
    OH, OW = (H - 1) // 2 + 1, (W - 1) // 2 + 1
    return OH % 4 == 0 and (4 * OW) % 64 == 0 and x.is_contiguous(memory_format=torch.channels_last)


def pack_weights(w):
    from .conv_native import WEIGHT_VERSION, is_managed
    key = (w.data_ptr(), str(w.device))
    ent = _packed.get(key)
    if ent is None:
        ent = _packed[key] = {"pk": torch.empty(4, 6, 64, 8, dtype=torch.bfloat16, device=w.device), "v": -1}
    if ent["v"] != WEIGHT_VERSION[0] or not is_managed(w.data_ptr()):
        lib = native.load()
        rc = lib.dl4j_stem_pack_weights(_ptr(w), _ptr(ent["pk"]), *[int(t) for t in w.stride()], _stream())
        native._check(rc, "stem_pack_weights")
        ent["v"] = WEIGHT_VERSION[0]
    return ent["pk"]


def pack_weights_reference(w):
    k = torch.arange(147, device=w.device)
    r, rem = k // 21, k % 21
    full = torch.zeros(192, 64, dtype=w.dtype, device=w.device)
    full.index_copy_(0, r * 24 + rem, w.permute(2, 3, 1, 0).reshape(147, 64))
    return full.view(6, 4, 8, 4, 16).permute(3, 0, 1, 4, 2).reshape(4, 6, 64, 8).contiguous()


def forward(x, w, want_stats=False):
    N, _, H, W = x.shape
    OH, OW = (H - 1) // 2 + 1, (W - 1) // 2 + 1
    lib = native.load()
    y = torch.empty((N, 64, OH, OW), dtype=torch.bfloat16, device=x.device, memory_format=torch.channels_last)
    ts = torch.empty((3, N * OH, 64), dtype=torch.float32, device=x.device) if want_stats else None
    rc = lib.dl4j_stem_conv_fwd(_ptr(x), _ptr(pack_weights(w)), _ptr(y), _ptr(ts), N, H, W, OH, OW,
                                _stream())
    if rc == -1:
        return None
    native._check(rc, "stem_conv_fwd")
    if ts is not None:
        y._bn_tile_stats = (ts, ts.shape[1], OW)
    return y


_ws = {}


def backward_weight(x, dy, gW=None, gb=None, need_db=False):
    N, _, H, W = x.shape
    OH, OW = dy.shape[2], dy.shape[3]
    lib = native.load()
    key = str(x.device)
    nws = lib.dl4j_stem_wrw_workspace_floats(N, OH)
    ws = _ws.get(key)
    if ws is None or ws.numel() < nws:
        ws = _ws[key] = torch.empty(nws, dtype=torch.float32, device=x.device)
    direct = gW is not None and gW.dtype == torch.float32 and gW.is_contiguous() and gW.numel() == 64 * 147
    dW = gW if direct else torch.empty((64, 3, 7, 7), dtype=torch.float32, device=x.device)
    db = None
    if need_db:
        directb = gb is not None and gb.dtype == torch.float32 and gb.is_contiguous() and gb.numel() == 64
        db = gb.reshape(-1) if directb else torch.empty(64, dtype=torch.float32, device=x.device)
    rc = lib.dl4j_stem_conv_wrw(_ptr(x), _ptr(dy), _ptr(dW), _ptr(db), _ptr(ws), N, H, W, OH, OW,
                                _stream())
    if rc == -1:
        return "unsupported"
    native._check(rc, "stem_conv_wrw")
    db_out = None
    if need_db:
        db_out = None if (gb is not None and db.data_ptr() == gb.data_ptr()) else db
    return (None if direct else dW), db_out
```

### deeplearning4j_amd/ops/native.py

```python
import ctypes
import os

import threading

import numpy as np
import torch

from . import abi
from .build import KERNEL_LIB

_lib = None
_load_lock = threading.Lock()
c_void_p, c_int, c_ll, c_float = ctypes.c_void_p, ctypes.c_int, ctypes.c_longlong, ctypes.c_float


def load():
    global _lib
    if _lib is not None:
        return _lib
    with _load_lock:
        if _lib is None:
            if not os.path.exists(KERNEL_LIB):
                if os.environ.get("DL4J_AMD_AUTOBUILD", "1") == "1":
                    from .build import build_kernels
# ... 158 lines not shown
        st = _slot(cache, ("graph", k), len(b), device)
        _write_pinned(st, b)


def refresh_graph_table(plan, slot, iteration, epoch):
    cache = plan.__dict__.get("_native_cache")
    st = cache.slots[("graph", slot)]
    b = seg_table_bytes(plan, iteration, epoch)
    if b != st.bytes:
        _write_pinned(st, b)


def mark_graph_replayed(plan, slot):
    cache = plan.__dict__.get("_native_cache")
    st = cache.slots[("graph", slot)]
    if st.event is None:
        st.event = torch.cuda.Event()
    st.event.record()


def fused_update(plan, params, grad, state, iteration, epoch, div, shadow, write_update, reg_out=None):
    lib = load()
    if lib.dl4j_segdesc_size() != _SEG_DTYPE.itemsize:
        raise RuntimeError("SegDesc layout mismatch between python and HIP")
    segs = plan.segments
    b = seg_table_bytes(plan, iteration, epoch)
    cache = plan.__dict__.setdefault("_native_cache", _SegTableCache())
    gslot = GRAPH_SLOT[0]
    if gslot is None:
        st = _slot(cache, "eager", len(b), params.device)
        if st.bytes != b:
            _write_pinned(st, b)
            st.dev.copy_(st.pinned, non_blocking=True)
            if st.event is None:
                st.event = torch.cuda.Event()
            st.event.record()
    else:
        st = cache.slots.get(("graph", gslot))
        if st is None or st.dev.numel() != len(b):
            raise RuntimeError("graph table slot not prepared before capture (prepare_graph_slots)")
        if st.bytes != b:
            st.pinned.numpy()[:] = np.frombuffer(b, dtype=np.uint8)
            st.bytes = b
        st.dev.copy_(st.pinned, non_blocking=True)
    if cache.btab is None or cache.btab.device != params.device:
        chunk = lib.dl4j_update_chunk()
        rows = [(si, ci) for si, s in enumerate(segs) for ci in range((s.n + chunk - 1) // chunk)]
        cache.btab = torch.tensor(rows if rows else [(0, 0)], dtype=torch.int32).to(params.device)
        cache.nblocks = len(rows)
    sk = 0
    if shadow is not None:
        sk = {torch.bfloat16: 1, torch.float16: 2}.get(shadow.dtype)
        if sk is None:
            return False
    gn_part = None
    if any(getattr(sg, "gn_mode", 0) in (1, 2, 4, 5) for sg in segs):
        gn_part = getattr(cache, "gn_partial", None)
        if gn_part is None or gn_part.numel() < cache.nblocks or gn_part.device != params.device:
            gn_part = cache.gn_partial = torch.empty(max(cache.nblocks, 1), dtype=torch.float32,
                                                     device=params.device)
    reg_part = None
    if reg_out is not None:
        reg_part = getattr(cache, "reg_partial", None)
        if reg_part is None or reg_part.numel() < cache.nblocks or reg_part.device != params.device:
            reg_part = cache.reg_partial = torch.empty(max(cache.nblocks, 1), dtype=torch.float32,
                                                       device=params.device)
        rc = lib.dl4j_fused_update_regpart(_ptr(st.dev), _ptr(cache.btab), cache.nblocks, _ptr(params), _ptr(grad),
                                           _ptr(state), _ptr(shadow), sk, 1.0 / div, 1 if write_update else 0,
                                           _ptr(reg_part), _ptr(gn_part), _stream())
        _check(rc, "fused_update")
        score_reduce(reg_part[:cache.nblocks], 0.0, 1.0, out=reg_out.reshape(-1)[:1])
    else:
        rc = lib.dl4j_fused_update(_ptr(st.dev), _ptr(cache.btab), cache.nblocks, _ptr(params), _ptr(grad),
                                   _ptr(state), _ptr(shadow), sk, 1.0 / div, 1 if write_update else 0, None,
                                   _ptr(gn_part), _stream())
        _check(rc, "fused_update")
    from . import rnn_native
    rnn_native.check_step_guard(params.device)
    return True


def score_reduce(s, add, scale, reg=None, reg_scale=0.0, out=None):
    lib = load()
    if out is None:
        out = torch.empty((), dtype=torch.float32, device=s.device)
    rc = lib.dl4j_score_reduce(_ptr(s), s.numel(), float(add), float(scale), _ptr(reg), float(reg_scale), _ptr(out),
                               _stream())
    _check(rc, "score_reduce")
    return out


def score_reduce_ok(*ts):
    return all(t is None or (torch.is_tensor(t) and t.is_cuda and t.dtype == torch.float32 and t.is_contiguous())
               for t in ts) and load() is not None


def _rows_like(t, ref):
    if t.dim() == 4 and not t.is_contiguous(memory_format=torch.channels_last):
        t = t.contiguous(memory_format=torch.channels_last)
    elif t.dim() == 2 and not t.is_contiguous():
        t = t.contiguous()
    return t.to(ref.dtype)


def bn_fwd(x, gamma, beta, run_mean, run_var, training, decay, eps, relu, residual=None, rctx=None,
           stats_only=False):
    dt = _dt16(x)
    xr = _as_rows_nhwc(x) if dt is not None else None
    if xr is None:
        return None
    M, C = xr.shape
    if C % 8 != 0 or C // 8 > 256 or run_mean.dtype != torch.float32:
        return None
    if (stats_only or rctx is not None) and not (training and dt in (1, 2)):
        return None
    lib = load()
    if rctx is not None:
        return _bn_fwd_rbn(lib, x, xr, dt, M, C, gamma, beta, run_mean, run_var, decay, eps, residual, rctx)
    y = None if stats_only else _like_rows(x)
    ws = _ae((lib.dl4j_bn_workspace_floats(M, C),), torch.float32, x.device)
    ctx = _ae((4 * C,), torch.float32, x.device)
    g = gamma if torch.is_tensor(gamma) else None
    b = beta if torch.is_tensor(beta) else None
    res = _rows_like(residual, x) if residual is not None else None
    mask = _ae((M * C // 8,), torch.uint8, x.device) if res is not None and training else None
    ts = getattr(x, "_bn_tile_stats", None)
    rpp = _tile_rpp(ts, M, C) if training and dt in (1, 2) else None
    if rpp is not None:
        wst = _ae((lib.dl4j_bn_tiles_workspace_floats(ts[1], C),), torch.float32, x.device)
        rc = lib.dl4j_bn_fwd_tiles(dt, _ptr(xr), _ptr(res), _ptr(y), M, C, _ptr(ts[0]), ts[1], rpp, _ptr(g), _ptr(b),
                                   float(gamma) if g is None else 1.0, float(beta) if b is None else 0.0,
                                   _ptr(run_mean), _ptr(run_var), float(decay), float(eps), 1 if relu else 0,
                                   _ptr(wst), _ptr(ctx), _ptr(mask), _stream())
        _check(rc, "bn_fwd_tiles")
        if stats_only:
            return x, ("NATIVE_STATS", x, ctx, False, M, C, None, None)
        _bnb_request(y, xr, ctx, relu, res, mask, training, dt)
        return y, ("NATIVE", x, ctx, relu, M, C, res, mask)
    rc = lib.dl4j_bn_fwd(dt, _ptr(xr), _ptr(res), _ptr(y), M, C, _ptr(g), _ptr(b),
                         float(gamma) if g is None else 1.0, float(beta) if b is None else 0.0, _ptr(run_mean),
                         _ptr(run_var), float(decay), float(eps), 1 if training else 0, 1 if relu else 0, _ptr(ws),
                         _ptr(ctx), _ptr(mask), _stream())
    _check(rc, "bn_fwd")
    if stats_only:
        return x, ("NATIVE_STATS", x, ctx, False, M, C, None, None)
    _bnb_request(y, xr, ctx, relu, res, mask, training, dt)
    return y, ("NATIVE", x, ctx, relu, M, C, res, mask)


def _tile_rpp(ts, M, C):
    if ts is None or ts[0].shape[2] != C:
        return None
    rpp = ts[2] if len(ts) > 2 else 64
    if rpp == 64:
        return 64 if ts[1] == 2 * ((M + 127) // 128) else None
    return rpp if ts[1] == (M + rpp - 1) // rpp else None


def _bn_fwd_rbn(lib, x, xr, dt, M, C, gamma, beta, run_mean, run_var, decay, eps, residual, rctx):
    y = _like_rows(x)
    ctx = _ae((4 * C,), torch.float32, x.device)
    g = gamma if torch.is_tensor(gamma) else None
    b = beta if torch.is_tensor(beta) else None
    res = _rows_like(residual, x)
    mask = _ae((M * C // 8,), torch.uint8, x.device)
    ts = getattr(x, "_bn_tile_stats", None)
    rpp = _tile_rpp(ts, M, C)
    tiles = rpp is not None
    if tiles:
        ws = _ae((lib.dl4j_bn_tiles_workspace_floats(ts[1], C),), torch.float32, x.device)
    else:
        ws = _ae((lib.dl4j_bn_workspace_floats(M, C),), torch.float32, x.device)
    rc = lib.dl4j_bn_fwd_rbn(dt, _ptr(xr), _ptr(res), _ptr(rctx), _ptr(y), M, C, _ptr(g), _ptr(b),
                             float(gamma) if g is None else 1.0, float(beta) if b is None else 0.0, _ptr(run_mean),
                             _ptr(run_var), float(decay), float(eps), _ptr(ws), _ptr(ctx), _ptr(mask),
                             _ptr(ts[0]) if tiles else None, ts[1] if tiles else 0, rpp if tiles else 0, _stream())
    _check(rc, "bn_fwd_rbn")
    return y, ("NATIVE", x, ctx, True, M, C, res, mask, rctx)


BNB_MODE = int(os.environ.get("DL4J_AMD_BN_BWD_EPILOGUE", "0") or 0)
BNB = BNB_MODE > 0


def _bnb_request(y, xr, ctx, relu, res, mask, training, dt):
    if BNB and training and (res is None or (mask is not None and BNB_MODE >= 2)) and dt in (1, 2) and \
            xr.dim() == 2:
        y._bn_bwd_req = (xr, ctx, bool(relu), mask)


class bnb_armed:

    def __init__(self, req):
        self.req = req

    def __enter__(self):
        xr, ctx, relu, mask = self.req
        load().dl4j_bnb_arm(_ptr(xr), _ptr(ctx), _ptr(mask), 3 if mask is not None else (2 if relu else 1))
        return self

    def __exit__(self, *exc):
        load().dl4j_bnb_arm(None, None, None, 0)
        return False


def bnb_tag(dx, planes, req):
    dx._bn_bwd_stats = (planes, req[1], planes.shape[1], dx._version)


def _bnb_planes(dy, c, res, M, C, mask=None):
    st = getattr(dy, "_bn_bwd_stats", None)
    if st is None or (res is not None and mask is None):
        return None
    planes, ctx_t, P, ver = st
    if ctx_t is not c or ver != dy._version or P != (M + 63) // 64 or tuple(planes.shape) != (2, P, C):
        return None
    return planes


def bn_bwd(dy, ctx, dgamma_out=None, dbeta_out=None, rgrads=None):
    _, x, c, relu, M, C, res, mask = ctx[:8]
    rctx = ctx[8] if len(ctx) > 8 else None
    planes = _bnb_planes(dy, c, res, M, C, mask) if rctx is None else None
    dy = _rows_like(dy, x)
    lib = load()
    dx = _like_rows(x)
    dres = _like_rows(x) if res is not None else None
    ok = lambda t: t is not None and t.dtype == torch.float32 and t.is_contiguous() and t.numel() == C
    dgamma = dgamma_out if ok(dgamma_out) else _ae((C,), torch.float32, x.device)
    dbeta = dbeta_out if ok(dbeta_out) else _ae((C,), torch.float32, x.device)
    if rctx is not None:
        rg = rgrads if rgrads is not None else (None, None)
        dg2 = rg[0] if ok(rg[0]) else _ae((C,), torch.float32, x.device)
        db2 = rg[1] if ok(rg[1]) else _ae((C,), torch.float32, x.device)
        ws = _ae((lib.dl4j_bn_bwd_rbn_workspace_floats(M, C),), torch.float32, x.device)
        rc = lib.dl4j_bn_bwd_rbn(_dt16(x), _ptr(x), _ptr(res), _ptr(dy), _ptr(dx), _ptr(dres), M, C, _ptr(c),
                                 _ptr(dgamma), _ptr(dbeta), _ptr(rctx), _ptr(dg2), _ptr(db2), _ptr(ws), _ptr(mask),
                                 _stream())
        _check(rc, "bn_bwd_rbn")
        if rgrads is not None:
            for dst, src in zip(rgrads, (dg2, db2)):
                if dst is not None and dst is not src:
                    dst.copy_(src.reshape(dst.shape))
        return dx, dgamma, dbeta, dres
    if planes is not None:
        P = planes.shape[1]
        ws = _ae((lib.dl4j_bn_bwd_planes_workspace_floats(P, C),), torch.float32, x.device)
        rc = lib.dl4j_bn_bwd_planes(_dt16(x), _ptr(x), _ptr(dy), _ptr(dx), _ptr(dres), _ptr(mask if dres is not None
                                                                                               else None), M, C,
                                    _ptr(c), _ptr(dgamma), _ptr(dbeta), 1 if relu else 0, _ptr(planes), P, _ptr(ws),
                                    _stream())
        _check(rc, "bn_bwd_planes")
        return dx, dgamma, dbeta, dres
    ws = _ae((lib.dl4j_bn_workspace_floats(M, C),), torch.float32, x.device)
    rc = lib.dl4j_bn_bwd(_dt16(x), _ptr(x), _ptr(res), _ptr(dy), _ptr(dx), _ptr(dres), M, C, _ptr(c), _ptr(dgamma),
                         _ptr(dbeta), 1 if relu else 0, _ptr(ws), _ptr(mask), _stream())
    _check(rc, "bn_bwd")
    return dx, dgamma, dbeta, dres


def bn_pool_fwd(x, gamma, beta, run_mean, run_var, training, decay, eps, kernel, stride, pad4):
    dt = _dt16(x)
    if dt is None or x.dim() != 4 or not torch.is_tensor(gamma) or run_mean.dtype != torch.float32:
        return None
    if not x.is_contiguous(memory_format=torch.channels_last):
        return None
    N, C, H, W = x.shape
    if C % 8 != 0 or C // 8 > 256:
        return None
    kh, kw = kernel
    sh, sw = stride
    pt, pb, pl, pr = pad4
    OH = (H + pt + pb - kh) // sh + 1
    OW = (W + pl + pr - kw) // sw + 1
    if OH < 1 or OW < 1 or kh * kw > 127:
        return None
    lib = load()
    y = _ae((N, C, OH, OW), x.dtype, x.device, channels_last=True)
    am = _ae((N * OH * OW * C,), torch.uint8, x.device) if training else None
    xh = _ae((N, C, OH, OW), x.dtype, x.device, channels_last=True) if training else None
    ts = getattr(x, "_bn_tile_stats", None)
    M = N * H * W
    rpp = ts[2] if ts is not None and len(ts) > 2 else 64
    if not (training and ts is not None and dt in (1, 2) and ts[0].shape[2] == C and
            (ts[1] * rpp == M if rpp != 64 else ts[1] == 2 * ((M + 127) // 128))):
        ts = None
    nws = lib.dl4j_bn_workspace_floats(M, C)
    if ts is not None:
        nws = max(nws, lib.dl4j_bn_tiles_workspace_floats(ts[1], C))
    ws = _ae((nws,), torch.float32, x.device)
    ctx = _ae((4 * C,), torch.float32, x.device)
    b = beta if torch.is_tensor(beta) else None
    rc = lib.dl4j_bn_pool_fwd(dt, _ptr(x), _ptr(y), _ptr(am), _ptr(xh), N, H, W, C, OH, OW, kh, kw, sh, sw, pt, pl,
                              _ptr(gamma), _ptr(b), 1.0, float(beta) if b is None else 0.0, _ptr(run_mean),
                              _ptr(run_var), float(decay), float(eps), 1 if training else 0,
                              _ptr(ts[0] if ts is not None else None), int(ts[1]) if ts is not None else 0, int(rpp),
                              _ptr(ws), _ptr(ctx), _stream())
    if rc == -1:
        return None
    _check(rc, "bn_pool_fwd")
    return y, ("NATIVE_POOL", x, ctx, am, xh, (kh, kw, sh, sw, pt, pl), (OH, OW))


def bn_pool_bwd(dy, ctx, dgamma_out=None, dbeta_out=None):
    _, x, c, am, xh, (kh, kw, sh, sw, pt, pl), (OH, OW) = ctx
    N, C, H, W = x.shape
    dy = _rows_like(dy, xh)
    lib = load()
    dx = _ae(x.shape, x.dtype, x.device, channels_last=True)
    ok = lambda t: t is not None and t.dtype == torch.float32 and t.is_contiguous() and t.numel() == C
    dgamma = dgamma_out if ok(dgamma_out) else _ae((C,), torch.float32, x.device)
    dbeta = dbeta_out if ok(dbeta_out) else _ae((C,), torch.float32, x.device)
    ws = _ae((lib.dl4j_bn_workspace_floats(N * OH * OW, C),), torch.float32, x.device)
    rc = lib.dl4j_bn_pool_bwd(_dt16(x), _ptr(x), _ptr(dy), _ptr(am), _ptr(xh), _ptr(dx), N, H, W, C, OH, OW, kh, kw,
                              sh, sw, pt, pl, _ptr(c), _ptr(dgamma), _ptr(dbeta), _ptr(ws), _stream())
    _check(rc, "bn_pool_bwd")
    return dx, dgamma, dbeta


def _dt16(t):
    return {torch.float32: 0, torch.bfloat16: 1, torch.float16: 2}.get(t.dtype)


def softmax_xent(logits, labels, clip_eps, row_mask=None):
    dt = _dt16(logits)
    if dt is None or not logits.is_contiguous():
        return None
    B, V = logits.shape
    lab = labels.contiguous().float()
    grad = _ae(logits.shape, logits.dtype, logits.device)
    score = _ae((B,), torch.float32, logits.device)
    if row_mask is not None:
        m = row_mask.reshape(-1).to(torch.float32).contiguous()
        if m.numel() != B:
            return None
        rc = load().dl4j_softmax_xent_masked(dt, _ptr(logits), _ptr(lab), B, V, _ptr(grad), _ptr(score), _ptr(m),
                                             float(clip_eps or 0.0), _stream())
        _check(rc, "softmax_xent_masked")
        return score, grad, None
    rc = load().dl4j_softmax_xent(dt, _ptr(logits), _ptr(lab), B, V, _ptr(grad), _ptr(score), None,
                                  float(clip_eps or 0.0), _stream())
    _check(rc, "softmax_xent")
    return score, grad, None


def softmax_xent_strided(logits, y, mb, ys, clip_eps):
    dt = _dt16(logits)
    if dt is None or logits.dim() != 2 or logits.stride(1) != 1 or y.dtype != torch.float32 or not y.is_cuda:
        return None
    B, V = logits.shape
    from ..memory import arena
    from .gemm import kz_view
    V8 = (V + 7) // 8 * 8
    buf = arena.empty((B, V8), logits.dtype, logits.device)
    score = arena.empty((B,), torch.float32, logits.device)
    rc = load().dl4j_softmax_xent_strided(dt, _ptr(logits), logits.stride(0) if B > 1 else V, _ptr(y), int(ys[0]),
                                          int(ys[1]), int(ys[2]), int(mb), B, V, _ptr(buf), V8, _ptr(score),
                                          float(clip_eps or 0.0), _stream())
    _check(rc, "softmax_xent_strided")
    return score, (kz_view(buf, V) if V8 != V else buf)


def pool2d_fwd(x, ptype, kernel, stride, pad4):
    dt = _dt16(x)
    if dt is None or x.dim() != 4 or x.shape[1] % 8 != 0:
        return None
    if not x.is_contiguous(memory_format=torch.channels_last):
        x = x.contiguous(memory_format=torch.channels_last)
    N, C, H, W = x.shape
    pt, pb, pl, pr = pad4
    kh, kw = kernel
    sh, sw = stride
    OH = (H + pt + pb - kh) // sh + 1
    OW = (W + pl + pr - kw) // sw + 1
    y = _ae((N, C, OH, OW), x.dtype, x.device, channels_last=True)
    mode = 0 if ptype == "MAX" else 1
    am = _ae((N * OH * OW * C if mode == 0 else 8,), torch.uint8, x.device)
    rc = load().dl4j_pool_fwd(dt, mode, _ptr(x), _ptr(y), _ptr(am), N, H, W, C, OH, OW, kh, kw, sh, sw, pt, pl,
                              _stream())
    _check(rc, "pool_fwd")
    return y, ("NATIVE", mode, am, x.shape, x.dtype, (kh, kw, sh, sw, pt, pl), (OH, OW))


def pool2d_bwd(dy, ctx):
    _, mode, am, xshape, xdt, (kh, kw, sh, sw, pt, pl), (OH, OW) = ctx
    N, C, H, W = xshape
    dy = dy.to(xdt).contiguous(memory_format=torch.channels_last)
    dx = _ae(xshape, xdt, dy.device, channels_last=True)
    rc = load().dl4j_pool_bwd({torch.bfloat16: 1, torch.float16: 2}.get(xdt, 0), mode, _ptr(dy), _ptr(am), _ptr(dx), N, H, W, C, OH,
                              OW, kh, kw, sh, sw, pt, pl, _stream())
    _check(rc, "pool_bwd")
    return dx


def conv2d_fwd(x, w, b, stride, pad4, dilation, want_stats=False):
    from . import conv_native
    return conv_native.conv2d_fwd(x, w, b, stride, pad4, dilation, want_stats)


def conv2d_bwd(x, w, dy, stride, pad4, dilation, need_dx, need_dw, need_db, gW=None, gb=None, grads_zeroed=False,
               dx_accum=None):
    from . import conv_native
    return conv_native.conv2d_bwd(x, w, dy, stride, pad4, dilation, need_dx, need_dw, need_db, gW, gb,
                                  grads_zeroed, dx_accum)


def segment_stats(flat, offsets, bins=0):
    lib = load()
    dt = _dt(flat)
    if dt is None or not flat.is_contiguous():
        raise ValueError("segment_stats needs a contiguous fp32/bf16 tensor")
    nseg = len(offsets) - 1
    if offsets[0] < 0 or offsets[-1] > flat.numel() or any(b < a for a, b in zip(offsets[:-1], offsets[1:])):
        raise IndexError("segment offsets outside the flat array")
    dev = flat.device
    off = torch.tensor(offsets, dtype=torch.int64, device=dev)
    ws = torch.empty(5 * nseg, dtype=torch.float32, device=dev)
    out = torch.empty(nseg, 5, dtype=torch.float32, device=dev)
    hist = torch.empty(nseg, bins, dtype=torch.int32, device=dev) if bins > 0 else None
    maxlen = max(b - a for a, b in zip(offsets[:-1], offsets[1:])) if nseg else 0
    rc = lib.dl4j_segment_stats(dt, _ptr(flat), _ptr(off), nseg, maxlen, _ptr(ws), _ptr(out), bins, _ptr(hist),
                                _stream())
    _check(rc, "segment_stats")
    return out, (hist.to(torch.int64) if hist is not None else None)


def channel_sum(rows, out=None):
    dt = _dt16(rows)
    if dt is None or rows.dim() != 2 or not rows.is_contiguous() or rows.shape[1] == 0:
        return None
    lib = load()
    if out is None or not (out.is_contiguous() and out.dtype == torch.float32 and out.numel() == rows.shape[1]):
        out = torch.empty(rows.shape[1], dtype=torch.float32, device=rows.device)
    ws = _scratch(lib.dl4j_channel_sum_ws_floats(rows.shape[0], rows.shape[1]), rows.device)
    _check(lib.dl4j_channel_sum(dt, _ptr(rows), rows.shape[0], rows.shape[1], _ptr(out), _ptr(ws),
                                _stream()), "channel_sum")
    return out


_scratch_bufs = {}


def _scratch(nfloats, device):
    key = (str(device), torch.cuda.current_stream(device).stream_id if device.type == "cuda" else 0)
    t = _scratch_bufs.get(key)
    if t is None or t.numel() < nfloats:
        t = _scratch_bufs[key] = torch.empty(max(int(nfloats), 1 << 16), dtype=torch.float32, device=device)
    return t
```

### deeplearning4j_amd/ops/norm.py

```python
import torch

from .dispatch import use_native
from deeplearning4j_amd.nn.util.dtypes import acc as _acc


def _dims(x):
    return (0,) if x.dim() == 2 else (0, 2, 3)


def _bshape(x):
    return (1, -1) if x.dim() == 2 else (1, -1, 1, 1)


def bn_forward(x, gamma, beta, run_mean, run_var, training, decay, eps, relu=False, residual=None, rctx=None,
               stats_only=False):
    if residual is not None:
        relu = True
    if stats_only or rctx is not None:
        if not (use_native(x, "bn") and x.dim() in (2, 4) and torch.is_tensor(gamma)):
            return None
        from . import native
        return native.bn_fwd(x, gamma, beta, run_mean, run_var, training, decay, eps, relu, residual, rctx=rctx,
                             stats_only=stats_only)
    if use_native(x, "bn") and x.dim() in (2, 4) and torch.is_tensor(gamma):
        from . import native
        r = native.bn_fwd(x, gamma, beta, run_mean, run_var, training, decay, eps, relu, residual)
        if r is not None:
            return r
    from .fallback import note
    note(x, "bn", f"torch path ({x.dtype}, dim {x.dim()})")
    xf = _acc(x)
    dims = _dims(x)
    bs = _bshape(x)
    if training:
        mean = xf.mean(dim=dims)
        var = xf.var(dim=dims, unbiased=False) + eps
        with torch.no_grad():
            run_mean.mul_(decay).add_(mean.reshape(run_mean.shape).to(run_mean.dtype) * (1 - decay))
            run_var.mul_(decay).add_(var.reshape(run_var.shape).to(run_var.dtype) * (1 - decay))
    else:
        mean = _acc(run_mean.reshape(-1))
        var = _acc(run_var.reshape(-1))
    invstd = torch.rsqrt(var)
    g = _acc(gamma.reshape(-1)) if torch.is_tensor(gamma) else torch.full_like(mean, float(gamma))
    b = _acc(beta.reshape(-1)) if torch.is_tensor(beta) else torch.full_like(mean, float(beta))
    xhat = (xf - mean.reshape(bs)) * invstd.reshape(bs)
    y = xhat * g.reshape(bs) + b.reshape(bs)
    if residual is not None:
        y = y + _acc(residual)
    if relu:
        y = torch.relu(y)
    y = y.to(x.dtype)
    if x.dim() == 4 and x.is_cuda:
        y = y.contiguous(memory_format=torch.channels_last)
    return y, ("REF", x, mean, invstd, g, b, relu, y if relu else None, residual is not None)


def bn_backward(dy, ctx, dgamma_out=None, dbeta_out=None, rgrads=None):
    if ctx[0] == "NATIVE":
        from . import native
        return native.bn_bwd(dy, ctx, dgamma_out, dbeta_out, rgrads=rgrads)
    _, x, mean, invstd, g, b, relu, y, has_res = ctx
    dims = _dims(x)
    bs = _bshape(x)
    dyf = _acc(dy)
    if relu:
        dyf = dyf * (y > 0).to(dyf.dtype)
    xhat = (_acc(x) - mean.reshape(bs)) * invstd.reshape(bs)
    m = x.numel() // x.shape[1]
    dbeta = dyf.sum(dim=dims)
    dgamma = (dyf * xhat).sum(dim=dims)
    dx = (g * invstd).reshape(bs) * (dyf - dbeta.reshape(bs) / m - xhat * (dgamma.reshape(bs) / m))
    dx = dx.to(dy.dtype)
    if x.dim() == 4 and x.is_cuda:
        dx = dx.contiguous(memory_format=torch.channels_last)
    dres = dyf.to(dy.dtype) if has_res else None
    return dx, dgamma, dbeta, dres


def bn_pool_forward(x, gamma, beta, run_mean, run_var, training, decay, eps, kernel, stride, pad4):
    if use_native(x, "bn") and x.dim() == 4 and torch.is_tensor(gamma):
        from . import native
        r = native.bn_pool_fwd(x, gamma, beta, run_mean, run_var, training, decay, eps, kernel, stride, pad4)
        if r is not None:
            return r
    from .pool import pool2d_forward
    y_bn, bctx = bn_forward(x, gamma, beta, run_mean, run_var, training, decay, eps, relu=True)
    y, pctx = pool2d_forward(y_bn, "MAX", kernel, stride, pad4)
    return y, ("COMPOSED", bctx, pctx, tuple(x.shape))


def bn_pool_backward(dy, ctx, dgamma_out=None, dbeta_out=None):
    if ctx[0] == "NATIVE_POOL":
        from . import native
        return native.bn_pool_bwd(dy, ctx, dgamma_out, dbeta_out)
    from .pool import pool2d_backward
    _, bctx, pctx, xshape = ctx
    d = pool2d_backward(dy, pctx)
    if tuple(d.shape[2:]) != tuple(xshape[2:]):
        full = torch.zeros(xshape, dtype=d.dtype, device=d.device)
        full[:, :, :d.shape[2], :d.shape[3]] = d
        d = full
    dx, dgamma, dbeta, _ = bn_backward(d, bctx, dgamma_out, dbeta_out)
    return dx, dgamma, dbeta


def bn_forward_inference_only(x, gamma, beta, run_mean, run_var, relu=False):
    y, _ = bn_forward(x, gamma, beta, run_mean, run_var, False, 0.0, 0.0, relu)
    return y


def layer_norm_forward(x, gamma, beta, eps):
    xf = _acc(x)
    if x.dim() == 3:
        xf = xf.transpose(1, 2)
    mean = xf.mean(dim=-1, keepdim=True)
    var = xf.var(dim=-1, unbiased=False, keepdim=True)
    invstd = torch.rsqrt(var + eps)
    xhat = (xf - mean) * invstd
    y = xhat * _acc(gamma.reshape(-1)) + _acc(beta.reshape(-1))
    if x.dim() == 3:
        y = y.transpose(1, 2)
    return y.to(x.dtype), (xhat, invstd, _acc(gamma.reshape(-1)), x.dim())


def layer_norm_backward(dy, ctx):
    xhat, invstd, g, nd = ctx
    d = _acc(dy)
    if nd == 3:
        d = d.transpose(1, 2)
    n = xhat.shape[-1]
    red = tuple(range(d.dim() - 1))
    dgamma = (d * xhat).sum(dim=red)
    dbeta = d.sum(dim=red)
    dxhat = d * g
    dx = invstd * (dxhat - dxhat.mean(dim=-1, keepdim=True) - xhat * (dxhat * xhat).mean(dim=-1, keepdim=True))
    if nd == 3:
        dx = dx.transpose(1, 2)
    _ = n
    return dx.to(dy.dtype), dgamma, dbeta
```

Before: 41580 images/sec.

## Fuse stem BN+maxpool backward dx into stem conv weight-gradient kernel

```diff
diff --git a/csrc/batchnorm.hip b/csrc/batchnorm.hip
--- a/csrc/batchnorm.hip
+++ b/csrc/batchnorm.hip
@@ -1,4 +1,5 @@
 #include "common.h"
+#include "bnpool_dx.h"
 #include <cstdlib>
 
 template <typename T>
@@ -1171,12 +1172,8 @@
   float A[8], B[8], Cq[8];
   if (fixed) {
 #pragma unroll
-    for (int i = 0; i < 8; ++i) {
-      const int c = (threadIdx.x % CG) * 8 + i;
-      A[i] = ctx[2 * C + c];
-      B[i] = ctx[2 * C + c] * ctx[C + c] * cdg[c];
-      Cq[i] = ctx[2 * C + c] * (cdb[c] - ctx[c] * ctx[C + c] * cdg[c]);
-    }
+    for (int i = 0; i < 8; ++i)
+      bnpool_dx_factors(ctx, cdb, cdg, C, (threadIdx.x % CG) * 8 + i, A[i], B[i], Cq[i]);
   }
   for (int it = threadIdx.x; it < items; it += 256) {
     const int cg = it % CG, q1 = it / CG, iw = q1 % W, ih = ih0 + q1 / W;
@@ -1208,7 +1205,7 @@
       }
     if (fixed) {
 #pragma unroll
-      for (int i = 0; i < 8; ++i) xv[i] = A[i] * acc[i] - B[i] * xv[i] - Cq[i];
+      for (int i = 0; i < 8; ++i) xv[i] = bnpool_dx_elem(A[i], B[i], Cq[i], acc[i], xv[i]);
     } else {
 #pragma unroll
       for (int i = 0; i < 8; ++i) {
@@ -1388,6 +1385,21 @@
 }
 
 template <typename T>
+static void bn_pool_bwd_stats_impl(const T* dy, const unsigned char* am, const T* xh, long long Mp, long long M, int C,
+                                   float* dgamma, float* dbeta, float* cdb, float* cdg, float* ws, hipStream_t s) {
+  int nblk;
+  long long rpb;
+  bn_grid(Mp, C, &nblk, &rpb);
+  float* p1 = ws;
+  float* p2 = ws + (long long)nblk * C;
+  float* q = p2 + (long long)nblk * C;
+  hipLaunchKernelGGL(bnpool_bwd_partial<T>, dim3(nblk), dim3(256), 0, s, dy, am, xh, Mp, C, rpb, p1, p2);
+  bn_reduce_stage(p1, p2, nblk, C, q, s);
+  hipLaunchKernelGGL(bn_bwd_finalize, dim3((C + 63) / 64), dim3(256), 0, s, p1, p2, nblk, C, M, dbeta, dgamma, cdb,
+                     cdg);
+}
+
+template <typename T>
 static int bn_pool_bwd_impl(const T* x, const T* dy, const unsigned char* am, const T* xh, T* dx, int N, int H, int W,
                             int C, int OH, int OW, int kh, int kw, int sh, int sw, int pt, int pl, const float* ctx,
                             float* dgamma, float* dbeta, float* ws, hipStream_t s) {
@@ -1395,16 +1407,10 @@
   int nblk;
   long long rpb;
   bn_grid(Mp, C, &nblk, &rpb);
-  float* p1 = ws;
-  float* p2 = ws + (long long)nblk * C;
-  float* q = p2 + (long long)nblk * C;
-  float* cdb = q + 2LL * ((nblk + 31) / 32) * C;
+  float* cdb = ws + 2LL * nblk * C + 2LL * ((nblk + 31) / 32) * C;
   float* cdg = cdb + C;
   const int g = ew_grid(M * (C / 8));
-  hipLaunchKernelGGL(bnpool_bwd_partial<T>, dim3(nblk), dim3(256), 0, s, dy, am, xh, Mp, C, rpb, p1, p2);
-  bn_reduce_stage(p1, p2, nblk, C, q, s);
-  hipLaunchKernelGGL(bn_bwd_finalize, dim3((C + 63) / 64), dim3(256), 0, s, p1, p2, nblk, C, M, dbeta, dgamma, cdb,
-                     cdg);
+  bn_pool_bwd_stats_impl<T>(dy, am, xh, Mp, M, C, dgamma, dbeta, cdb, cdg, ws, s);
   const bool two = kh <= 2 * sh && kw <= 2 * sw;
   const int maxrows = (2 - 1 + kh - 1) / sh + 1;
   const size_t lds = (size_t)maxrows * OW * C * (sizeof(T) + 1);
@@ -1434,3 +1440,16 @@
   BPB(float);
 #undef BPB
 }
+
+DL4J_API int dl4j_bn_pool_bwd_stats(int dtype, const void* dy, const unsigned char* am, const void* xh, int N, int H,
+                                    int W, int C, int OH, int OW, float* dgamma, float* dbeta, float* cdbg, float* ws,
+                                    hipStream_t s) {
+  if (C % 8 != 0 || C / 8 > 256 || !cdbg) return -1;
+  const long long Mp = (long long)N * OH * OW, M = (long long)N * H * W;
+#define BPS(T) bn_pool_bwd_stats_impl<T>((const T*)dy, am, (const T*)xh, Mp, M, C, dgamma, dbeta, cdbg, cdbg + C, ws, s)
+  if (dtype == 1) BPS(bf16);
+  else if (dtype == 2) BPS(f16);
+  else BPS(float);
+#undef BPS
+  return (int)hipGetLastError();
+}
diff --git a/csrc/bnpool_dx.h b/csrc/bnpool_dx.h
--- /dev/null
+++ b/csrc/bnpool_dx.h
@@ -0,0 +1,19 @@
+#pragma once
+#include "common.h"
+
+__device__ __forceinline__ void bnpool_dx_factors(const float* __restrict__ ctx, const float* __restrict__ cdb,
+                                                  const float* __restrict__ cdg, int C, int c, float& A, float& B,
+                                                  float& Cq) {
+  A = ctx[2 * C + c];
+  B = ctx[2 * C + c] * ctx[C + c] * cdg[c];
+  Cq = ctx[2 * C + c] * (cdb[c] - ctx[c] * ctx[C + c] * cdg[c]);
+}
+
+__device__ __forceinline__ float bnpool_dx_elem(float A, float B, float Cq, float g, float x) {
+  return A * g - B * x - Cq;
+}
+
+__device__ __forceinline__ int bnpool_first_window(int p, int k, int s) {
+  const int o = p - k + 1;
+  return o <= 0 ? 0 : (o + s - 1) / s;
+}
diff --git a/csrc/conv_stem.hip b/csrc/conv_stem.hip
--- a/csrc/conv_stem.hip
+++ b/csrc/conv_stem.hip
@@ -1,4 +1,6 @@
 #include "common.h"
+#include "bnpool_dx.h"
+#include <cstdlib>
 
 typedef __attribute__((ext_vector_type(4))) float f4s_t;
 typedef __attribute__((ext_vector_type(8))) __bf16 bf16x8s_t;
@@ -155,13 +157,31 @@
 }
 
 constexpr int kWrwWgPerCu = 3;
-__global__ void __launch_bounds__(256, kWrwWgPerCu) stem_conv_wrw(const u16* __restrict__ x, const u16* __restrict__ dy,
-                                                        float* __restrict__ part, float* __restrict__ part_db, int N,
-                                                        int H, int W, int OH, int OW, int RS) {
+constexpr int kWrwFusedWgPerCu = 2;
+constexpr int kWrwFusedGridPerCu = 8;
+constexpr int kWrwMaxGridPerCu = 8;
+constexpr int POOL_SLOTS = 6;
+struct StemBnPool {
+  const u16* dyp;
+  const unsigned char* am;
+  const float* ctx;
+  const float* cdbg;
+  int PH, PW, kh, kw, sh, sw, pt, pl, maxrows;
+};
+
+__device__ __forceinline__ int small_div(int a, float inv) { return (int)(((float)a + 0.5f) * inv); }
+
+template <bool FUSE>
+__global__ void __launch_bounds__(256, FUSE ? kWrwFusedWgPerCu : kWrwWgPerCu)
+stem_conv_wrw(const u16* __restrict__ x, const u16* __restrict__ dy, float* __restrict__ part,
+              float* __restrict__ part_db, int N, int H, int W, int OH, int OW, int RS, StemBnPool bp) {
+  constexpr int LA = FUSE ? 3 : 2;
   extern __shared__ __attribute__((aligned(16))) unsigned char smem[];
   u16* xin = reinterpret_cast<u16*>(smem);
   u16* dyt = xin + IN_ROWS * RS;
   float* dbs = reinterpret_cast<float*>(dyt + 2 * 64 * OUT_LD);
+  u16* sdy = reinterpret_cast<u16*>(dbs + 256 * 8);
+  unsigned char* sam = reinterpret_cast<unsigned char*>(sdy + (FUSE ? bp.maxrows * bp.PW * 64 : 0));
   const int lane = threadIdx.x & 63, wave = threadIdx.x >> 6, col = lane & 15, hg = lane >> 4;
   const int blocks_per_img = OH / ROWS_PER_WG, nblocks = N * blocks_per_img;
   const int row_elems = 3 * W, row_u2 = row_elems / 4;
@@ -191,6 +211,20 @@
   float dbacc[8];
 #pragma unroll
   for (int i = 0; i < 8; ++i) dbacc[i] = 0.f;
+  float fA[8], fB[8], fC[8];
+  if constexpr (FUSE) {
+#pragma unroll
+    for (int i = 0; i < 8; ++i)
+      bnpool_dx_factors(bp.ctx, bp.cdbg, bp.cdbg + 64, 64, (threadIdx.x & 7) * 8 + i, fA[i], fB[i], fC[i]);
+  }
+  float inv_ow = 0.f, inv_sh = 0.f, inv_sw = 0.f;
+  int shkw = 0;
+  if constexpr (FUSE) {
+    inv_ow = 1.0f / (float)OW;
+    inv_sh = 1.0f / (float)bp.sh;
+    inv_sw = 1.0f / (float)bp.sw;
+    shkw = bp.sh * bp.kw;
+  }
   uint2 pre[STAGE_SLOTS];
   for (int blk = blockIdx.x; blk < nblocks; blk += gridDim.x) {
     const int n = blk / blocks_per_img, oh0 = (blk - n * blocks_per_img) * ROWS_PER_WG;
@@ -204,6 +238,25 @@
       if (i < nchunks && ih >= 0 && ih < H)
         pre[q] = *reinterpret_cast<const uint2*>(x + ((long long)n * H + ih) * row_elems + 4 * j);
     }
+    int oh_lo = 0, oh_hi = -1;
+    uint4 pdy[POOL_SLOTS];
+    uint2 pam[POOL_SLOTS];
+    if constexpr (FUSE) {
+      oh_lo = bnpool_first_window(oh0 + bp.pt, bp.kh, bp.sh);
+      oh_hi = min((oh0 + ROWS_PER_WG - 1 + bp.pt) / bp.sh, bp.PH - 1);
+      const int nv = (oh_hi - oh_lo + 1) * bp.PW * 8;
+      const long long g0 = ((long long)n * bp.PH + oh_lo) * bp.PW * 64;
+#pragma unroll
+      for (int q = 0; q < POOL_SLOTS; ++q) {
+        const int i = threadIdx.x + q * 256;
+        pdy[q] = make_uint4(0u, 0u, 0u, 0u);
+        pam[q] = make_uint2(0u, 0u);
+        if (i < nv) {
+          pdy[q] = reinterpret_cast<const uint4*>(bp.dyp + g0)[i];
+          pam[q] = reinterpret_cast<const uint2*>(bp.am + g0)[i];
+        }
+      }
+    }
 #pragma unroll
     for (int q = 0; q < STAGE_SLOTS; ++q) {
       const int i = threadIdx.x + q * 256;
@@ -211,25 +264,72 @@
       if (i < nchunks) *reinterpret_cast<uint2*>(xin + rr * RS + 12 + 4 * j) = pre[q];
     }
     const long long m_base = ((long long)n * OH + oh0) * OW;
+    constexpr int PX_MUL = FUSE ? 2 : 1, PX_STEP = FUSE ? 1 : 32;
     auto load_dy = [&](int rnd, uint4* dst) {
 #pragma unroll
       for (int j = 0; j < 2; ++j)
-        dst[j] = *reinterpret_cast<const uint4*>(dy + (m_base + rnd * 64 + (threadIdx.x >> 3) + 32 * j) * 64 +
+        dst[j] = *reinterpret_cast<const uint4*>(dy + (m_base + rnd * 64 + (threadIdx.x >> 3) * PX_MUL + PX_STEP * j) * 64 +
                                                  (threadIdx.x & 7) * 8);
     };
     auto round = [&](int rnd, uint4* gr) {
       u16* dt = dyt + (rnd & 1) * 64 * OUT_LD;
 #pragma unroll
       for (int j = 0; j < 2; ++j) {
-        const int px = (threadIdx.x >> 3) + 32 * j, c8 = threadIdx.x & 7;
-        const u16* hv = reinterpret_cast<const u16*>(&gr[j]);
+        const int px = (threadIdx.x >> 3) * PX_MUL + PX_STEP * j, c8 = threadIdx.x & 7;
+        u16 hv[8];
+        if constexpr (FUSE) {
+          const int p = rnd * 64 + px, ohl = small_div(p, inv_ow), iw = p - ohl * OW;
+          const int hp = oh0 + ohl + bp.pt, wp = iw + bp.pl;
+          const int po0 = hp < bp.kh ? 0 : small_div(hp - bp.kh + bp.sh, inv_sh);
+          const int pw0 = wp < bp.kw ? 0 : small_div(wp - bp.kw + bp.sw, inv_sw);
+          const int po1 = min(small_div(hp, inv_sh), bp.PH - 1), pw1 = min(small_div(wp, inv_sw), bp.PW - 1);
+          const int base = __mul24(po0 - oh_lo, bp.PW) + pw0;
+          const int idx00 = __mul24(hp - __mul24(po0, bp.sh), bp.kw) + (wp - __mul24(pw0, bp.sw));
+          uint4 cg4[4];
+          uint2 ca[4];
+          unsigned me[4];
+#pragma unroll
+          for (int a = 0; a < 2; ++a)
+#pragma unroll
+            for (int b = 0; b < 2; ++b) {
+              const int q = a * 2 + b;
+              const bool ok = po0 + a <= po1 && pw0 + b <= pw1;
+              const int o = ok ? (base + a * bp.PW + b) * 64 + c8 * 8 : c8 * 8;
+              cg4[q] = *reinterpret_cast<const uint4*>(sdy + o);
+              ca[q] = *reinterpret_cast<const uint2*>(sam + o);
+              me[q] = ok ? 0x80u + (unsigned)(idx00 - a * shkw - b * bp.sw) : 0x100u;
+            }
+          float g[8];
+#pragma unroll
+          for (int i = 0; i < 8; ++i) g[i] = 0.f;
+#pragma unroll
+          for (int q = 0; q < 4; ++q) {
+            if (me[q] == 0x100u) continue;
+            const unsigned* gw = reinterpret_cast<const unsigned*>(&cg4[q]);
+#pragma unroll
+            for (int i = 0; i < 8; ++i) {
+              const unsigned ab = ((i < 4 ? ca[q].x : ca[q].y) >> (8 * (i & 3))) & 0xffu;
+              const float gv = __uint_as_float((i & 1) ? (gw[i >> 1] & 0xffff0000u) : (gw[i >> 1] << 16));
+              if (ab == me[q]) g[i] += gv;
+            }
+          }
+          const unsigned* yw = reinterpret_cast<const unsigned*>(&gr[j]);
+#pragma unroll
+          for (int i = 0; i < 8; ++i) {
+            const float yv = __uint_as_float((i & 1) ? (yw[i >> 1] & 0xffff0000u) : (yw[i >> 1] << 16));
+            hv[i] = f2bf(bnpool_dx_elem(fA[i], fB[i], fC[i], g[i], yv));
+          }
+        } else {
+#pragma unroll
+          for (int i = 0; i < 8; ++i) hv[i] = reinterpret_cast<const u16*>(&gr[j])[i];
+        }
 #pragma unroll
         for (int i = 0; i < 8; ++i) {
           dt[(c8 * 8 + i) * OUT_LD + (((px >> 3) ^ c8) << 3) + (px & 7)] = hv[i];
           dbacc[i] += bf2f(hv[i]);
         }
       }
-      if (rnd + 2 < rounds) load_dy(rnd + 2, gr);
+      if (rnd + LA < rounds) load_dy(rnd + LA, gr);
       __syncthreads();
 #pragma unroll
       for (int ch = 0; ch < 2; ++ch) {
@@ -258,12 +358,30 @@
         }
       }
     };
-    uint4 gA[2], gB[2];
+    uint4 gA[2], gB[2], gC[2];
     load_dy(0, gA);
     if (rounds > 1) load_dy(1, gB);
-    for (int rnd = 0; rnd < rounds; rnd += 2) {
-      round(rnd, gA);
-      if (rnd + 1 < rounds) round(rnd + 1, gB);
+    if constexpr (FUSE) {
+      if (rounds > 2) load_dy(2, gC);
+#pragma unroll
+      for (int q = 0; q < POOL_SLOTS; ++q) {
+        const int i = threadIdx.x + q * 256;
+        if (i < (oh_hi - oh_lo + 1) * bp.PW * 8) {
+          reinterpret_cast<uint4*>(sdy)[i] = pdy[q];
+          reinterpret_cast<uint2*>(sam)[i] = pam[q];
+        }
+      }
+      __syncthreads();
+      for (int rnd = 0; rnd < rounds; rnd += 3) {
+        round(rnd, gA);
+        if (rnd + 1 < rounds) round(rnd + 1, gB);
+        if (rnd + 2 < rounds) round(rnd + 2, gC);
+      }
+    } else {
+      for (int rnd = 0; rnd < rounds; rnd += 2) {
+        round(rnd, gA);
+        if (rnd + 1 < rounds) round(rnd + 1, gB);
+      }
     }
   }
   float* pw = part + (long long)blockIdx.x * 64 * 192;
@@ -321,7 +439,7 @@
   int dev = 0, ncu = 256;
   (void)hipGetDevice(&dev);
   (void)hipDeviceGetAttribute(&ncu, hipDeviceAttributeMultiprocessorCount, dev);
-  const long long G = (long long)kWrwWgPerCu * ncu;
+  const long long G = (long long)kWrwMaxGridPerCu * ncu;
   return G * (64 * 192 + 64);
 }
 
@@ -343,8 +461,61 @@
   const int G = nblocks < kWrwWgPerCu * ncu ? nblocks : kWrwWgPerCu * ncu;
   float* part = ws;
   float* part_db = ws + (long long)G * 64 * 192;
-  hipLaunchKernelGGL(stem_conv_wrw, dim3(G), dim3(256), lds, s, (const u16*)x, (const u16*)dy, part, part_db, N, H, W,
-                     OH, OW, RS);
+  hipLaunchKernelGGL(stem_conv_wrw<false>, dim3(G), dim3(256), lds, s, (const u16*)x, (const u16*)dy, part, part_db, N,
+                     H, W, OH, OW, RS, StemBnPool{});
+  hipLaunchKernelGGL(stem_wrw_reduce, dim3((64 * 147 + 64 + 15) / 16), dim3(256), 0, s, part, part_db, G, dW, db);
+  return (int)hipGetLastError();
+}
+
+DL4J_API int dl4j_stem_conv_wrw_bnpool(const void* x, const void* y, const void* dyp, const unsigned char* am,
+                                       const float* ctx, const float* cdbg, float* dW, float* db, float* ws, int N,
+                                       int H, int W, int OH, int OW, int PH, int PW, int kh, int kw, int sh, int sw,
+                                       int pt, int pl, hipStream_t s) {
+  if (N < 1 || OH % ROWS_PER_WG != 0 || OW % 16 != 0 || OH != (H - 1) / 2 + 1 || OW != (W - 1) / 2 + 1 ||
+      (3 * W) % 4 != 0 || (ROWS_PER_WG * OW) % 64 != 0)
+    return -1;
+  if (kh < 1 || kw < 1 || sh < 1 || sw < 1 || kh > 2 * sh || kw > 2 * sw || kh * kw > 127 || pt < 0 || pl < 0 ||
+      PH < 1 || PW < 1 || !y || !dyp || !am || !ctx || !cdbg)
+    return -1;
+  int RS = 12 + 3 * W;
+  const int need = 6 * (OW - 1) + 3 + 24 + 2;
+  if (RS < need) RS = need;
+  RS = (RS + 15) & ~15;
+  const int maxrows = (ROWS_PER_WG - 1 + kh - 1) / sh + 1;
+  if ((long long)maxrows * PW * 8 > POOL_SLOTS * 256) return -1;
+  const size_t lds = (size_t)IN_ROWS * RS * 2 + 2 * 64 * OUT_LD * 2 + 256 * 8 * 4 + (size_t)maxrows * PW * 64 * 3;
+  if (lds > 160 * 1024 / kWrwFusedWgPerCu || (IN_ROWS - 1) * (3 * W / 4) > STAGE_SLOTS * 256) return -1;
+  int dev = 0, ncu = 256;
+  (void)hipGetDevice(&dev);
+  (void)hipDeviceGetAttribute(&ncu, hipDeviceAttributeMultiprocessorCount, dev);
+  static bool lds_opt_in[64] = {};
+  if (dev < 0 || dev >= 64) return -1;
+  if (!lds_opt_in[dev]) {
+    if (hipFuncSetAttribute(reinterpret_cast<const void*>(stem_conv_wrw<true>),
+                            hipFuncAttributeMaxDynamicSharedMemorySize, 160 * 1024 / kWrwFusedWgPerCu) != hipSuccess) {
+      (void)hipGetLastError();
+      return -1;
+    }
+    lds_opt_in[dev] = true;
+  }
+  const int nblocks = N * (OH / ROWS_PER_WG);
+  static const int grid_per_cu = [] {
+    const char* e = getenv("DL4J_AMD_STEM_FUSED_GRID");
+    const int v = e ? atoi(e) : kWrwFusedGridPerCu;
+    return v < 1 ? 1 : (v > kWrwMaxGridPerCu ? kWrwMaxGridPerCu : v);
+  }();
+  const int G = nblocks < grid_per_cu * ncu ? nblocks : grid_per_cu * ncu;
+  float* part = ws;
+  float* part_db = ws + (long long)G * 64 * 192;
+  StemBnPool bp;
+  bp.dyp = (const u16*)dyp;
+  bp.am = am;
+  bp.ctx = ctx;
+  bp.cdbg = cdbg;
+  bp.PH = PH; bp.PW = PW; bp.kh = kh; bp.kw = kw; bp.sh = sh; bp.sw = sw; bp.pt = pt; bp.pl = pl;
+  bp.maxrows = maxrows;
+  hipLaunchKernelGGL(stem_conv_wrw<true>, dim3(G), dim3(256), lds, s, (const u16*)x, (const u16*)y, part, part_db, N, H,
+                     W, OH, OW, RS, bp);
   hipLaunchKernelGGL(stem_wrw_reduce, dim3((64 * 147 + 64 + 15) / 16), dim3(256), 0, s, part, part_db, G, dW, db);
   return (int)hipGetLastError();
 }
diff --git a/csrc/include/dl4j_amd.h b/csrc/include/dl4j_amd.h
--- a/csrc/include/dl4j_amd.h
+++ b/csrc/include/dl4j_amd.h
@@ -88,6 +88,7 @@
 int dl4j_bn_bwd_planes(int dtype, const void* x, const void* dy, void* dx, void* dres, const unsigned char* mask, long long M, int C, const float* ctx, float* dgamma, float* dbeta, int relu, const float* planes, long long P, float* ws, hipStream_t s);
 int dl4j_bn_pool_fwd(int dtype, const void* x, void* y, unsigned char* am, void* xh, int N, int H, int W, int C, int OH, int OW, int kh, int kw, int sh, int sw, int pt, int pl, const float* gamma, const float* beta, float gconst, float bconst, float* run_mean, float* run_var, float decay, float eps, int training, const float* tstats, long long P, int rpp, float* ws, float* ctx_out, hipStream_t s);
 int dl4j_bn_pool_bwd(int dtype, const void* x, const void* dy, const unsigned char* am, const void* xh, void* dx, int N, int H, int W, int C, int OH, int OW, int kh, int kw, int sh, int sw, int pt, int pl, const float* ctx, float* dgamma, float* dbeta, float* ws, hipStream_t s);
+int dl4j_bn_pool_bwd_stats(int dtype, const void* dy, const unsigned char* am, const void* xh, int N, int H, int W, int C, int OH, int OW, float* dgamma, float* dbeta, float* cdbg, float* ws, hipStream_t s);
 
 int dl4j_nonfinite_count(const void* segs, int nseg, void* seg_dev, unsigned long long* counts, long long max_n, hipStream_t s);
 
@@ -122,6 +123,7 @@
 int dl4j_stem_conv_fwd(const void* x, const void* wpk, void* y, float* tstats, int N, int H, int W, int OH, int OW, hipStream_t s);
 long long dl4j_stem_wrw_workspace_floats(int N, int OH);
 int dl4j_stem_conv_wrw(const void* x, const void* dy, float* dW, float* db, float* ws, int N, int H, int W, int OH, int OW, hipStream_t s);
+int dl4j_stem_conv_wrw_bnpool(const void* x, const void* y, const void* dyp, const unsigned char* am, const float* ctx, const float* cdbg, float* dW, float* db, float* ws, int N, int H, int W, int OH, int OW, int PH, int PW, int kh, int kw, int sh, int sw, int pt, int pl, hipStream_t s);
 int dl4j_stem_pack_weights(const void* w, void* pk, long long sk, long long sc, long long sr, long long ss, hipStream_t s);
 
 int dl4j_conv_wrw_set_tree(int fan);
diff --git a/deeplearning4j_amd/nn/graph/computation_graph.py b/deeplearning4j_amd/nn/graph/computation_graph.py
--- a/deeplearning4j_amd/nn/graph/computation_graph.py
+++ b/deeplearning4j_amd/nn/graph/computation_graph.py
@@ -194,6 +194,21 @@
             flows[name] = need or own
         for name, layer in self.layers_by_name.items():
             layer.need_input_grad = self._need_input_grad[name]
+        self._stem_bwd_fuse = []
+        for name, layer in self.layers_by_name.items():
+            if getattr(layer, "fuse_pool", None) is None:
+                continue
+            v, ins = self.conf.vertices[name], self.vertex_inputs[name]
+            if len(ins) != 1 or v.preProcessor is not None or ins[0] in self._passthrough:
+                continue
+            cn = ins[0]
+            cv = self.conf.vertices.get(cn)
+            if not (isinstance(cv, LayerVertex) and type(cv.layerConf) is ConvolutionLayer) or cn in self.outputs or \
+                    self.consumers.get(cn) != [name] or self._need_input_grad[cn] or \
+                    cv.layerConf.idropout is not None or \
+                    type(cv.layerConf.activation).__name__ != "ActivationIdentity":
+                continue
+            self._stem_bwd_fuse.append(name)
 
     def getLayers(self):
         return list(self.layers_by_name.values())
@@ -360,6 +375,14 @@
                 eps_acc[name] = e
 
         self._begin_backward()
+        if getattr(self, "_stem_bwd_fuse", None):
+            from ...ops import conv_stem
+            from ...optimize.listeners import TrainingListener
+            hooked = any(getattr(type(l), "onBackwardPass", None) is not TrainingListener.onBackwardPass or
+                         "onBackwardPass" in getattr(l, "__dict__", {}) for l in self.listeners)
+            defer = conv_stem.bwd_fuse_enabled() and not hooked and not _prof.ACTIVE and tbptt_back is None
+            for bn in self._stem_bwd_fuse:
+                self.layers_by_name[bn].defer_dx = defer
         for name in reversed(self.topo):
             v = self.conf.vertices[name]
             if name in self._passthrough:
diff --git a/deeplearning4j_amd/nn/layers/convolution.py b/deeplearning4j_amd/nn/layers/convolution.py
--- a/deeplearning4j_amd/nn/layers/convolution.py
+++ b/deeplearning4j_amd/nn/layers/convolution.py
@@ -1,3 +1,5 @@
+import os
+
 import torch
 import torch.nn.functional as F
 
@@ -89,7 +91,32 @@
         self._z = z
         return self.conf.activation.getActivation(z, training)
 
-    def backpropGradient(self, eps):
+    def _backprop_deferred(self, eps):
+        from ...ops import conv_stem
+        from ...ops.dispatch import use_native
+        s, pad4, d = self._geom_cache
+        W = self.W("W")
+        xt = _cl(self._xt.to(W.dtype))
+        if getattr(self, "need_input_grad", True) or type(self.conf.activation).__name__ != "ActivationIdentity" or \
+                os.environ.get("DL4J_AMD_KERNEL_STEM", "1") != "1" or not use_native(xt, "conv") or \
+                not conv_stem.supported(xt, W, None, s, pad4, d) or tuple(eps.shape[2:]) != tuple(self._z.shape[2:]):
+            return None
+        r = conv_stem.backward_weight(xt, eps, self.grads["W"], self.grads.get("b"), "b" in self.grads)
+        if r == "unsupported":
+            return None
+        dW, db = r
+        if dW is not None:
+            copy_grad_(self.grads["W"], dW)
+        if "b" in self.grads and db is not None:
+            copy_grad_(self.grads["b"], db)
+        return self.make_gradient(), None
+
+    def backpropGradient(self, eps):
+        if not torch.is_tensor(eps) and hasattr(eps, "materialize"):
+            r = self._backprop_deferred(eps)
+            if r is not None:
+                return r
+            eps = eps.materialize()
         delta = self.conf.activation.backprop(self._z, eps.to(self._z.dtype))
         s, pad4, d = self._geom_cache
         W = self.W("W")
diff --git a/deeplearning4j_amd/nn/layers/normalization.py b/deeplearning4j_amd/nn/layers/normalization.py
--- a/deeplearning4j_amd/nn/layers/normalization.py
+++ b/deeplearning4j_amd/nn/layers/normalization.py
@@ -79,7 +79,9 @@
             self._zero_stat_grads()
             return self.make_gradient(), self.backpropDropOut(eps)
         if getattr(self, "_pool_fused", False):
-            dx, dgamma, dbeta = ops.bn_pool_backward(eps, self._ctx, gg, gb)
+            defer = bool(getattr(self, "defer_dx", False)) and self.conf.idropout is None
+            self.defer_dx = False
+            dx, dgamma, dbeta = ops.bn_pool_backward(eps, self._ctx, gg, gb, defer_dx=defer)
             self.dresidual = None
         elif getattr(self, "_rbn_active", None) is not None:
             rbn = self._rbn_active
@@ -94,7 +96,7 @@
             if dbeta is not gb:
                 copy_grad_(gb, dbeta)
         self._zero_stat_grads()
-        return self.make_gradient(), self.backpropDropOut(dx)
+        return self.make_gradient(), (dx if not torch.is_tensor(dx) else self.backpropDropOut(dx))
 
     def _zero_stat_grads(self):
         if not getattr(self, "_stat_grads_zero", False):
diff --git a/deeplearning4j_amd/ops/conv_stem.py b/deeplearning4j_amd/ops/conv_stem.py
--- a/deeplearning4j_amd/ops/conv_stem.py
+++ b/deeplearning4j_amd/ops/conv_stem.py
@@ -1,3 +1,5 @@
+import os
+
 import torch
 
 from . import native
@@ -59,6 +61,13 @@
 _ws = {}
 
 
+FUSED_CALLS = [0]
+
+
+def bwd_fuse_enabled():
+    return os.environ.get("DL4J_AMD_STEM_BWD_FUSE", "1") == "1"
+
+
 def backward_weight(x, dy, gW=None, gb=None, need_db=False):
     N, _, H, W = x.shape
     OH, OW = dy.shape[2], dy.shape[3]
@@ -74,8 +83,23 @@
     if need_db:
         directb = gb is not None and gb.dtype == torch.float32 and gb.is_contiguous() and gb.numel() == 64
         db = gb.reshape(-1) if directb else torch.empty(64, dtype=torch.float32, device=x.device)
-    rc = lib.dl4j_stem_conv_wrw(_ptr(x), _ptr(dy), _ptr(dW), _ptr(db), _ptr(ws), N, H, W, OH, OW,
-                                _stream())
+    rc = -1
+    if isinstance(dy, native.DeferredPoolDx):
+        d = dy
+        if d.dtype == torch.bfloat16 and d.shape[1] == 64:
+            kh, kw, sh, sw, pt, pl = d.geometry
+            PH, PW = d.pooled_hw
+            rc = lib.dl4j_stem_conv_wrw_bnpool(_ptr(x), _ptr(d.y), _ptr(d.dyp), _ptr(d.am), _ptr(d.ctx), _ptr(d.cdbg),
+                                               _ptr(dW), _ptr(db), _ptr(ws), N, H, W, OH, OW, PH, PW, kh, kw, sh, sw,
+                                               pt, pl, _stream())
+        if rc == -1:
+            dy = d.materialize()
+        else:
+            native._check(rc, "stem_conv_wrw_bnpool")
+            FUSED_CALLS[0] += 1
+    if rc == -1:
+        rc = lib.dl4j_stem_conv_wrw(_ptr(x), _ptr(dy), _ptr(dW), _ptr(db), _ptr(ws), N, H, W, OH, OW,
+                                    _stream())
     if rc == -1:
         return "unsupported"
     native._check(rc, "stem_conv_wrw")
diff --git a/deeplearning4j_amd/ops/native.py b/deeplearning4j_amd/ops/native.py
--- a/deeplearning4j_amd/ops/native.py
+++ b/deeplearning4j_amd/ops/native.py
@@ -484,16 +484,49 @@
     return y, ("NATIVE_POOL", x, ctx, am, xh, (kh, kw, sh, sw, pt, pl), (OH, OW))
 
 
-def bn_pool_bwd(dy, ctx, dgamma_out=None, dbeta_out=None):
+class DeferredPoolDx:
+
+    def __init__(self, ctx, dyp, cdbg):
+        self.bn_ctx, self.dyp, self.cdbg = ctx, dyp, cdbg
+        self._dx = None
+
+    y = property(lambda self: self.bn_ctx[1])
+    ctx = property(lambda self: self.bn_ctx[2])
+    am = property(lambda self: self.bn_ctx[3])
+    geometry = property(lambda self: self.bn_ctx[5])
+    pooled_hw = property(lambda self: self.bn_ctx[6])
+    shape = property(lambda self: self.y.shape)
+    dtype = property(lambda self: self.y.dtype)
+    device = property(lambda self: self.y.device)
+
+    def dim(self):
+        return 4
+
+    def to(self, dtype):
+        return self if dtype == self.dtype else self.materialize().to(dtype)
+
+    def materialize(self):
+        if self._dx is None:
+            self._dx = bn_pool_bwd(self.dyp, self.bn_ctx)[0]
+        return self._dx
+
+
+def bn_pool_bwd(dy, ctx, dgamma_out=None, dbeta_out=None, defer_dx=False):
     _, x, c, am, xh, (kh, kw, sh, sw, pt, pl), (OH, OW) = ctx
     N, C, H, W = x.shape
     dy = _rows_like(dy, xh)
     lib = load()
-    dx = _ae(x.shape, x.dtype, x.device, channels_last=True)
+    dx = None if defer_dx else _ae(x.shape, x.dtype, x.device, channels_last=True)
     ok = lambda t: t is not None and t.dtype == torch.float32 and t.is_contiguous() and t.numel() == C
     dgamma = dgamma_out if ok(dgamma_out) else _ae((C,), torch.float32, x.device)
     dbeta = dbeta_out if ok(dbeta_out) else _ae((C,), torch.float32, x.device)
     ws = _ae((lib.dl4j_bn_workspace_floats(N * OH * OW, C),), torch.float32, x.device)
+    if defer_dx:
+        cdbg = _ae((2 * C,), torch.float32, x.device)
+        rc = lib.dl4j_bn_pool_bwd_stats(_dt16(x), _ptr(dy), _ptr(am), _ptr(xh), N, H, W, C, OH, OW, _ptr(dgamma),
+                                        _ptr(dbeta), _ptr(cdbg), _ptr(ws), _stream())
+        _check(rc, "bn_pool_bwd_stats")
+        return DeferredPoolDx(ctx, dy, cdbg), dgamma, dbeta
     rc = lib.dl4j_bn_pool_bwd(_dt16(x), _ptr(x), _ptr(dy), _ptr(am), _ptr(xh), _ptr(dx), N, H, W, C, OH, OW, kh, kw,
                               sh, sw, pt, pl, _ptr(c), _ptr(dgamma), _ptr(dbeta), _ptr(ws), _stream())
     _check(rc, "bn_pool_bwd")
diff --git a/deeplearning4j_amd/ops/norm.py b/deeplearning4j_amd/ops/norm.py
--- a/deeplearning4j_amd/ops/norm.py
+++ b/deeplearning4j_amd/ops/norm.py
@@ -90,10 +90,11 @@
     return y, ("COMPOSED", bctx, pctx, tuple(x.shape))
 
 
-def bn_pool_backward(dy, ctx, dgamma_out=None, dbeta_out=None):
+def bn_pool_backward(dy, ctx, dgamma_out=None, dbeta_out=None, defer_dx=False):
     if ctx[0] == "NATIVE_POOL":
         from . import native
-        return native.bn_pool_bwd(dy, ctx, dgamma_out, dbeta_out)
+        return native.bn_pool_bwd(dy, ctx, dgamma_out, dbeta_out,
+                                  defer_dx=defer_dx and ctx[1].dtype == torch.bfloat16 and ctx[1].shape[1] == 64)
     from .pool import pool2d_backward
     _, bctx, pctx, xshape = ctx
     d = pool2d_backward(dy, pctx)
```

Result: no change. 41990 images/sec (median of 6 runs) (+1.0%).
